# dmuley/sph-code

Measured on AMD Instinct MI355X. Metric: particle-steps/sec + achieved HBM GB/s, 10^6-particle 3D sphere, 1/2/4/8 GPUs, higher is better.
Workload: dtype f64

## Files before the change

### include/sphx.h

```cpp
#ifndef SPHX_H
#define SPHX_H

#include <stddef.h>
#include <stdint.h>

#ifdef __cplusplus
extern "C" {
#endif

#define SPHX_OK            0
#define SPHX_E_ARG        -1
#define SPHX_E_HIP        -2
#define SPHX_E_NOMEM      -3
#define SPHX_E_STATE      -4

#define SPHX_MAX_K        64
#define SPHX_MAX_SPECIES  32

typedef struct sphx_ctx sphx_ctx;

typedef struct sphx_constants {
    double k_B;
    double amu;
    double m_h;
    double m_0;
    double dt_0;
    double max_age;
    double pos_clamp;
} sphx_constants;

typedef struct sphx_stats {
    double ms_grid;
    double ms_search;
    double ms_prep;
    double ms_density;
    double ms_pi;
    double ms_visc;
    double ms_integrate;
    double ms_total;
    int64_t n;
    int64_t steps;
    int64_t candidates;
    int64_t retries;
    int64_t cells;
    int64_t refresh_steps;
    int64_t rebuild_steps;
    double  cell_size;
    double  ms_gravity;
    int64_t fallback_queries;
    double  ms_species;
    int64_t short_rows;
    int64_t detail_steps;
    int64_t far_queries;
    int64_t outlier_levels;
    int64_t bad_accel;
    int64_t bad_energy;
    int64_t bad_state;
    int64_t bad_h;
    int64_t search_steps;
} sphx_stats;

int         sphx_create(sphx_ctx** out, int device);
void        sphx_destroy(sphx_ctx* ctx);
const char* sphx_last_error(const sphx_ctx* ctx);
int         sphx_version(void);
const char* sphx_build_info(void);
const char* sphx_tunables(const sphx_ctx* ctx);
int sphx_selftest_scan(sphx_ctx* ctx, int n, unsigned seed, long long* mismatches, int* single_launch);
int sphx_selftest_mfma_cull(sphx_ctx* ctx, double E, int blocks, unsigned seed, double* max_err_over_E2,
                            double* wrong_signs, double* kappa);
int         sphx_host_alloc(void** out, size_t bytes);
int         sphx_host_free(void* p);
int         sphx_set_constants(sphx_ctx* ctx, const sphx_constants* c);
int         sphx_get_constants(const sphx_ctx* ctx, sphx_constants* c);
int         sphx_set_tuning(sphx_ctx* ctx, double rscale, double cell_factor);
int         sphx_set_timing_detail(sphx_ctx* ctx, int on);
int         sphx_set_incremental(sphx_ctx* ctx, int verlet, double rscale_build);

int sphx_neighbors(sphx_ctx* ctx, int64_t n, int k, const double* points, double dist,
                   double eps, int64_t* idx, double* dist_out, int64_t* nontriv, double* h);

int sphx_hydro_update(sphx_ctx* ctx, int64_t n, int k, int s, const int64_t* neighbor,
                      const double* points, const double* mass, const double* sizes,
                      const double* f_un, const double* particle_type, const double* T,
                      const double* mu_array, const double* gamma_array,
                      const double* velocities, int visc_mode,
                      double* hydro_accel, double* visc_accel, double* visc_heat,
                      double* rho, double* nden, double* f_un_nb, double* rho_dust);

int sphx_density(sphx_ctx* ctx, int64_t n, int k, const double* points, const double* mass,
                 const double* particle_type, const int64_t* neighbor, double d, double* out);
int sphx_dust_density(sphx_ctx* ctx, int64_t n, int k, const double* points, const double* mass,
                      const int64_t* neighbor, const double* particle_type, const double* sizes,
                      double* out);
int sphx_num_dens(sphx_ctx* ctx, int64_t n, int k, const double* mass, const double* points,
                  const double* mu_array, const int64_t* neighbor, double d, double* out);
int sphx_del_pressure(sphx_ctx* ctx, int64_t n, int k, const double* points, const double* mass,
                      const double* particle_type, const int64_t* neighbor,
                      const double* E_internal, const double* gamma_array, double d,
                      double* out );
int sphx_artificial_viscosity(sphx_ctx* ctx, int64_t n, int k, const int64_t* neighbor,
                              const double* points, const double* particle_type,
                              const double* sizes, const double* mass, const double* densities,
                              const double* velocities, const double* T,
                              const double* gamma_array, const double* mu_array, double d,
                              double* visc_accel , double* visc_heat );
int sphx_crossing_time(sphx_ctx* ctx, int64_t n, int k, const int64_t* neighbor,
                       const double* velocities, const double* sizes,
                       const double* particle_type, double* out );
int sphx_net_impulse(sphx_ctx* ctx, int64_t n, int k, const double* points, const double* mass,
                     const double* sizes, const double* velocities, const double* particle_type,
                     const int64_t* neighbor, const double* mean_grain_mass,
                     const double* mean_cross, double* accel_onto ,
                     double* accel_reaction );

int sphx_gravity_direct(sphx_ctx* ctx, int64_t n, const double* mass, const double* points,
                        const double* sizes, double softening, double G, double* accel);

int sphx_gravity_tree(sphx_ctx* ctx, int64_t n, const double* mass, const double* points,
                      const double* sizes, double softening, double G, int ws, int k_cells,
                      double* accel);

int sphx_agb_yields(sphx_ctx* ctx, int64_t n, const double* masses, const double* metallicities,
                    int nspl, const int32_t* ntx, const int32_t* nty, const double* tx,
                    const double* ty, const double* coeffs, const int32_t* mapto, double divisor,
                    int nspecies, const double* mu_specie, const double* composition,
                    double solar_mass, double* dust_out ,
                    double* gas_out );

int sphx_dt_rule(sphx_ctx* ctx, int64_t n, const double* ct, const int32_t* first, double* dt);
int sphx_clamp_arrays(sphx_ctx* ctx, int64_t n, double* points, double* velocities);
int sphx_leapfrog(sphx_ctx* ctx, int64_t n, double* points, double* velocities, double* total_accel,
                  const double* old_accel, double* E_internal, double* T, const double* mass,
                  const double* mu, const double* gamma, const double* ptype, const double* grav_accel,
                  const double* delp, const double* densities, const double* dust_densities,
                  const double* drag_on_gas, const double* drag_reaction, const double* av_accel,
                  const double* av_heat, double dt);

int sphx_state_upload(sphx_ctx* ctx, int64_t n, int s, const double* pos, const double* vel,
                      const double* mass, const double* ptype, const double* f_un,
                      const double* T, const double* mu, const double* gamma,
                      const double* E_internal, const double* accel_old);
int sphx_state_set_drag(sphx_ctx* ctx, const double* mean_grain_mass, const double* mean_cross);
int sphx_state_set_agb(sphx_ctx* ctx, int nspl, const int32_t* ntx, const int32_t* nty, const double* tx,
                       const double* ty, const double* coeffs, const int32_t* mapto, double divisor,
                       const double* mu_specie, double solar_mass);
int sphx_state_download_species(sphx_ctx* ctx, double* F, double* Z, double* agb_dust);
int sphx_state_set_loop_forms(sphx_ctx* ctx, int on, double d);
int sphx_set_clip_grad(sphx_ctx* ctx, int on);
int sphx_set_visc_mode(sphx_ctx* ctx, int mode);
int sphx_state_set_gravity(sphx_ctx* ctx, int mode, double G);
int sphx_set_gravity_order(sphx_ctx* ctx, int order);
int sphx_step(sphx_ctx* ctx, int nsteps, int k, double dist, int first, double fixed_dt);
int sphx_state_download(sphx_ctx* ctx, double* pos, double* vel, double* accel,
                        double* E_internal, double* T, double* sizes, double* rho,
                        double* nden, double* visc_heat, double* dt_last);
int sphx_state_download_pressure(sphx_ctx* ctx, double* pressure);
int sphx_arb_fields(sphx_ctx* ctx, int64_t n, const double* points, const double* mass,
                    const double* particle_type, const double* sizes, const double* T, const double* n_part,
                    const double* value, double d, int64_t m, const double* arb_points, double radius,
                    double* density, double* dust_density, double* temperature, double* dust_temperature,
                    double* photoionization, int64_t* count, int64_t* candidates, int64_t ball_id);
int sphx_arb_fields_list(sphx_ctx* ctx, int64_t n, const double* points, const double* mass,
                         const double* particle_type, const double* sizes, const double* T, const double* n_part,
                         const double* value, double d, int64_t m, const double* arb_points,
                         const int64_t* row_start, const int64_t* members, double* density, double* dust_density,
                         double* temperature, double* dust_temperature, double* photoionization, int64_t* count,
                         int64_t* candidates);
int sphx_state_sample(sphx_ctx* ctx, double d, const double* n_part, const double* value, int64_t m,
                      const double* arb_points, double radius, double* density, double* dust_density,
                      double* temperature, double* dust_temperature, double* photoionization, int64_t* count,
                      int64_t* candidates);
int sphx_arb_last_timing(sphx_ctx* ctx, double ms[4]);
int sphx_get_stats(sphx_ctx* ctx, sphx_stats* out);
int sphx_reset_stats(sphx_ctx* ctx);

int sphx_set_stream(sphx_ctx* ctx, void* hip_stream );
int sphx_reset_stream(sphx_ctx* ctx);
int sphx_sync(sphx_ctx* ctx);
int sphx_dev_set_mean_h(sphx_ctx* ctx, double mean_h);
int sphx_dev_search(sphx_ctx* ctx, int64_t n_total, int64_t n_owned, int k, const double* pos,
                    const double* hint, double rscale, double dist, double* h_out);
int sphx_dev_get_order(sphx_ctx* ctx, int64_t n_total, int32_t* out);
int sphx_dev_prep(sphx_ctx* ctx, const double* pos, const double* vel, const double* mass,
                  const double* h, const double* T, const double* mu, const double* gamma,
                  const double* ptype);
int sphx_dev_density(sphx_ctx* ctx, double* rho, double* rho_dust, double* nden, double* hydro_accel);
int sphx_dev_pi(sphx_ctx* ctx, const double* rho_complete, double* Pi, double* Bw, double* ct_out);
int sphx_dev_visc(sphx_ctx* ctx, const double* Bw_complete, const double* mass, double* visc_accel,
                  double* visc_heat);
int sphx_dev_visc_pairwise(sphx_ctx* ctx, const double* rho_complete, const double* mass, double* visc_accel,
                           double* visc_heat, double* ct_out);
int sphx_dev_clamp(sphx_ctx* ctx, int64_t n, double* pos, double* vel);
int sphx_dev_pack_rows(sphx_ctx* ctx, int64_t n, const int64_t* idx, int nf, const double* const* fields,
                       const int32_t* widths, double* rows);
int sphx_dev_regroup(sphx_ctx* ctx, int64_t n_sel, const int64_t* sel, int64_t n_rows, const double* rows,
                     int nf, const double* const* fields_in, const int32_t* widths,
                     double* const* fields_out);
int sphx_dev_need_map(sphx_ctx* ctx, int64_t n, const double* pos, const double* w, const double* g_lo,
                      double g_cs, int G, unsigned char* out);
int sphx_dev_integrate_auto(sphx_ctx* ctx, int64_t n_owned, double* pos, double* vel, double* accel_old,
                            double* E_internal, double* T, const double* mass, const double* mu,
                            const double* gamma, const double* ptype, const double* hydro_accel,
                            const double* visc_accel, const double* visc_heat, const double* red2,
                            int first, double fixed_dt, double* dt_out);
int sphx_dev_loop_prep(sphx_ctx* ctx, const double* pos, const double* vel, const double* mass, const double* T,
                       const double* mu, const double* gamma, const double* ptype, const double* E_internal, double d);
int sphx_dev_loop_pass1(sphx_ctx* ctx, const double* h_complete, double* rho, double* rho_dust, double* nden, double* delp);
int sphx_dev_loop_pass2(sphx_ctx* ctx, const double* rho_complete, double* visc_accel, double* visc_heat, double* ct_out);
int sphx_dev_loop_pass2_interior(sphx_ctx* ctx);
int sphx_dev_set_reach_cap(sphx_ctx* ctx, double cap);
int sphx_dev_select_blobs(sphx_ctx* ctx, int part);
int sphx_dev_blob_split_counts(sphx_ctx* ctx, int32_t counts[3]);
int sphx_dev_integrate_loop(sphx_ctx* ctx, int64_t n_owned, double* pos, double* vel, double* accel_old,
                            double* E_internal, double* T, const double* mass, const double* mu, const double* gamma,
                            const double* ptype, const double* delp, const double* rho, const double* av_accel,
                            const double* av_heat, const double* red2, int first, double fixed_dt, double dt,
                            double* dt_out);
int sphx_dev_drag(sphx_ctx* ctx, const double* mass, const double* ptype, const double* mean_grain_mass,
                  const double* mean_cross, double* drag_on, double* drag_reaction);
int sphx_dev_set_drag_terms(sphx_ctx* ctx, const double* drag_on, const double* drag_reaction, const double* rho,
                            const double* rho_dust);
int sphx_dev_set_agb(sphx_ctx* ctx, int nspecies, int nspl, const int32_t* ntx, const int32_t* nty, const double* tx,
                     const double* ty, const double* coeffs, const int32_t* mapto, double divisor,
                     const double* mu_specie, double solar_mass);
int sphx_dev_species(sphx_ctx* ctx, int nspecies, const double* f_un, const double* mass, double* F, double* Z,
                     double* agb_dust);
int sphx_dev_reach(sphx_ctx* ctx, int64_t n, const double* h, const double* vel, double halo_scale,
                   double skin_frac, double dt_last, double* w);
int sphx_dev_reach_dt(sphx_ctx* ctx, int64_t n, const double* h, const double* vel, double halo_scale,
                      double skin_frac, const double* dt_dev, double* w);
int sphx_dev_plan_mask(sphx_ctx* ctx, int64_t n, const double* pos, const double* g_lo, double g_cs, int G,
                       int world, int rank, const unsigned char* maps, unsigned char* mask, int64_t* counts);
int sphx_dev_step_scalars(sphx_ctx* ctx, int64_t n_owned, const double* h, const double* w_plan, double D,
                          double hclip, const double* ct, double* out4);
int sphx_dev_integrate(sphx_ctx* ctx, int64_t n_owned, double* pos, double* vel, double* accel_old,
                       double* E_internal, double* T, const double* mass, const double* mu,
                       const double* gamma, const double* ptype, const double* hydro_accel,
                       const double* visc_accel, const double* visc_heat, double dt);

#ifdef __cplusplus
}
#endif
#endif
```

### sph-code_amd/_lib.py

```python
import ctypes as C
import os
import threading
import weakref

import numpy as np

HERE = os.path.dirname(os.path.abspath(__file__))
LIB_PATH = os.environ.get("SPHX_LIB") or os.path.join(HERE, "libsphx.so")

c_double_p = C.POINTER(C.c_double)
c_int64_p = C.POINTER(C.c_int64)


class SphxConstants(C.Structure):
    _fields_ = [(n, C.c_double) for n in ("k_B", "amu", "m_h", "m_0", "dt_0", "max_age", "pos_clamp")]


class SphxStats(C.Structure):
    _fields_ = [(n, C.c_double) for n in ("ms_grid", "ms_search", "ms_prep", "ms_density", "ms_pi",
                                          "ms_visc", "ms_integrate", "ms_total")] + \
               [(n, C.c_int64) for n in ("n", "steps", "candidates", "retries", "cells", "refresh_steps",
                                         "rebuild_steps")] + \
               [("cell_size", C.c_double), ("ms_gravity", C.c_double), ("fallback_queries", C.c_int64),
                ("ms_species", C.c_double), ("short_rows", C.c_int64), ("detail_steps", C.c_int64), ("far_queries", C.c_int64),
                ("outlier_levels", C.c_int64), ("bad_accel", C.c_int64), ("bad_energy", C.c_int64), ("bad_state", C.c_int64),
                ("bad_h", C.c_int64), ("search_steps", C.c_int64)]

    def as_dict(self):
        return {n: getattr(self, n) for n, _ in self._fields_}


SPHX_E_STATE = -4
_P = C.c_void_p
_D = c_double_p
_I = c_int64_p
SIGNATURES = {
    "sphx_create": (C.c_int, [C.POINTER(_P), C.c_int]),
    "sphx_destroy": (None, [_P]),
    "sphx_last_error": (C.c_char_p, [_P]),
    "sphx_version": (C.c_int, []),
    "sphx_build_info": (C.c_char_p, []),
    "sphx_tunables": (C.c_char_p, [_P]),
    "sphx_selftest_scan": (C.c_int, [_P, C.c_int, C.c_uint, C.POINTER(C.c_longlong), C.POINTER(C.c_int)]),
    "sphx_selftest_mfma_cull": (C.c_int, [_P, C.c_double, C.c_int, C.c_uint, _D, _D, _D]),
    "sphx_host_alloc": (C.c_int, [C.POINTER(_P), C.c_size_t]),
    "sphx_host_free": (C.c_int, [_P]),
    "sphx_set_constants": (C.c_int, [_P, C.POINTER(SphxConstants)]),
    "sphx_get_constants": (C.c_int, [_P, C.POINTER(SphxConstants)]),
    "sphx_set_tuning": (C.c_int, [_P, C.c_double, C.c_double]),
    "sphx_set_incremental": (C.c_int, [_P, C.c_int, C.c_double]),
    "sphx_neighbors": (C.c_int, [_P, C.c_int64, C.c_int, _D, C.c_double, C.c_double, _I, _D, _I, _D]),
    "sphx_hydro_update": (C.c_int, [_P, C.c_int64, C.c_int, C.c_int, _I] + [_D] * 9 + [C.c_int] + [_D] * 7),
    "sphx_density": (C.c_int, [_P, C.c_int64, C.c_int, _D, _D, _D, _I, C.c_double, _D]),
    "sphx_dust_density": (C.c_int, [_P, C.c_int64, C.c_int, _D, _D, _I, _D, _D, _D]),
    "sphx_num_dens": (C.c_int, [_P, C.c_int64, C.c_int, _D, _D, _D, _I, C.c_double, _D]),
    "sphx_del_pressure": (C.c_int, [_P, C.c_int64, C.c_int, _D, _D, _D, _I, _D, _D, C.c_double, _D]),
    "sphx_artificial_viscosity": (C.c_int, [_P, C.c_int64, C.c_int, _I] + [_D] * 9 + [C.c_double, _D, _D]),
    "sphx_crossing_time": (C.c_int, [_P, C.c_int64, C.c_int, _I, _D, _D, _D, _D]),
    "sphx_net_impulse": (C.c_int, [_P, C.c_int64, C.c_int, _D, _D, _D, _D, _D, _I, _D, _D, _D, _D]),
    "sphx_agb_yields": (C.c_int, [_P, C.c_int64, _D, _D, C.c_int, C.POINTER(C.c_int32), C.POINTER(C.c_int32), _D, _D, _D,
                                  C.POINTER(C.c_int32), C.c_double, C.c_int, _D, _D, C.c_double, _D, _D]),
    "sphx_dt_rule": (C.c_int, [_P, C.c_int64, _D, C.POINTER(C.c_int32), _D]),
    "sphx_clamp_arrays": (C.c_int, [_P, C.c_int64, _D, _D]),
    "sphx_leapfrog": (C.c_int, [_P, C.c_int64] + [_D] * 18 + [C.c_double]),
    "sphx_state_upload": (C.c_int, [_P, C.c_int64, C.c_int] + [_D] * 10),
    "sphx_state_set_drag": (C.c_int, [_P, _D, _D]),
    "sphx_state_set_agb": (C.c_int, [_P, C.c_int, C.POINTER(C.c_int32), C.POINTER(C.c_int32), _D, _D, _D,
                                     C.POINTER(C.c_int32), C.c_double, _D, C.c_double]),
    "sphx_state_download_species": (C.c_int, [_P, _D, _D, _D]),
    "sphx_state_set_loop_forms": (C.c_int, [_P, C.c_int, C.c_double]),
    "sphx_set_clip_grad": (C.c_int, [_P, C.c_int]),
    "sphx_set_visc_mode": (C.c_int, [_P, C.c_int]),
    "sphx_state_set_gravity": (C.c_int, [_P, C.c_int, C.c_double]),
    "sphx_set_gravity_order": (C.c_int, [_P, C.c_int]),
    "sphx_gravity_direct": (C.c_int, [_P, C.c_int64, _D, _D, _D, C.c_double, C.c_double, _D]),
    "sphx_gravity_tree": (C.c_int, [_P, C.c_int64, _D, _D, _D, C.c_double, C.c_double, C.c_int, C.c_int, _D]),
    "sphx_step": (C.c_int, [_P, C.c_int, C.c_int, C.c_double, C.c_int, C.c_double]),
    "sphx_state_download": (C.c_int, [_P] + [_D] * 10),
    "sphx_state_download_pressure": (C.c_int, [_P, _D]),
    "sphx_arb_fields": (C.c_int, [_P, C.c_int64] + [_D] * 7 + [C.c_double, C.c_int64, _D, C.c_double] + [_D] * 5 + [_I, _I, C.c_int64]),
    "sphx_arb_last_timing": (C.c_int, [_P, _D]),
    "sphx_arb_fields_list": (C.c_int, [_P, C.c_int64] + [_D] * 7 + [C.c_double, C.c_int64, _D, _I, _I] + [_D] * 5 + [_I, _I]),
    "sphx_state_sample": (C.c_int, [_P, C.c_double, _D, _D, C.c_int64, _D, C.c_double] + [_D] * 5 + [_I, _I]),
    "sphx_get_stats": (C.c_int, [_P, C.POINTER(SphxStats)]),
    "sphx_reset_stats": (C.c_int, [_P]),
    "sphx_set_stream": (C.c_int, [_P, C.c_void_p]),
    "sphx_reset_stream": (C.c_int, [_P]),
    "sphx_sync": (C.c_int, [_P]),
    "sphx_dev_set_mean_h": (C.c_int, [_P, C.c_double]),
    "sphx_dev_search": (C.c_int, [_P, C.c_int64, C.c_int64, C.c_int, _P, _P, C.c_double, C.c_double, _P]),
    "sphx_dev_get_order": (C.c_int, [_P, C.c_int64, _P]),
    "sphx_dev_prep": (C.c_int, [_P] + [_P] * 8),
    "sphx_dev_density": (C.c_int, [_P] + [_P] * 4),
    "sphx_dev_pi": (C.c_int, [_P] + [_P] * 4),
    "sphx_dev_visc": (C.c_int, [_P] + [_P] * 4),
    "sphx_dev_visc_pairwise": (C.c_int, [_P] + [_P] * 5),
    "sphx_dev_clamp": (C.c_int, [_P, C.c_int64, _P, _P]),
    "sphx_dev_pack_rows": (C.c_int, [_P, C.c_int64, _P, C.c_int, C.POINTER(C.c_void_p), C.POINTER(C.c_int32), _P]),
    "sphx_dev_regroup": (C.c_int, [_P, C.c_int64, _P, C.c_int64, _P, C.c_int, C.POINTER(C.c_void_p),
                                   C.POINTER(C.c_int32), C.POINTER(C.c_void_p)]),
    "sphx_dev_need_map": (C.c_int, [_P, C.c_int64, _P, _P, C.POINTER(C.c_double), C.c_double, C.c_int, _P]),
    "sphx_dev_integrate_auto": (C.c_int, [_P, C.c_int64] + [_P] * 13 + [C.c_int, C.c_double, _P]),
    "sphx_dev_reach": (C.c_int, [_P, C.c_int64, _P, _P, C.c_double, C.c_double, C.c_double, _P]),
    "sphx_set_timing_detail": (C.c_int, [_P, C.c_int]),
    "sphx_dev_reach_dt": (C.c_int, [_P, C.c_int64, _P, _P, C.c_double, C.c_double, _P, _P]),
    "sphx_dev_plan_mask": (C.c_int, [_P, C.c_int64, _P, C.POINTER(C.c_double), C.c_double, C.c_int, C.c_int, C.c_int, _P, _P, _P]),
    "sphx_dev_step_scalars": (C.c_int, [_P, C.c_int64, _P, _P, C.c_double, C.c_double, _P, _P]),
    "sphx_dev_integrate": (C.c_int, [_P, C.c_int64] + [_P] * 12 + [C.c_double]),
    "sphx_dev_drag": (C.c_int, [_P] + [_P] * 6),
    "sphx_dev_set_drag_terms": (C.c_int, [_P] + [_P] * 4),
    "sphx_dev_set_agb": (C.c_int, [_P, C.c_int, C.c_int, C.POINTER(C.c_int32), C.POINTER(C.c_int32), _D, _D, _D,
                                   C.POINTER(C.c_int32), C.c_double, _D, C.c_double]),
    "sphx_dev_species": (C.c_int, [_P, C.c_int] + [_P] * 5),
    "sphx_dev_loop_prep": (C.c_int, [_P] + [_P] * 8 + [C.c_double]),
    "sphx_dev_loop_pass1": (C.c_int, [_P] + [_P] * 5),
    "sphx_dev_loop_pass2": (C.c_int, [_P] + [_P] * 4),
    "sphx_dev_loop_pass2_interior": (C.c_int, [_P]),
    "sphx_dev_set_reach_cap": (C.c_int, [_P, C.c_double]),
    "sphx_dev_select_blobs": (C.c_int, [_P, C.c_int]),
    "sphx_dev_blob_split_counts": (C.c_int, [_P, _P]),
    "sphx_dev_integrate_loop": (C.c_int, [_P, C.c_int64] + [_P] * 14 + [C.c_int, C.c_double, C.c_double, _P]),
}

_lib = None
_lock = threading.Lock()


def load_library():
    global _lib
    with _lock:
        if _lib is not None:
            return _lib
        if not os.path.exists(LIB_PATH):
            raise RuntimeError(
                "libsphx.so is not built (%s). Run `python -c 'import __graft_entry__ as g; g.build()'` "
                "or `python sph-code_amd/build.py`. There is no CPU fallback." % LIB_PATH)
        lib = C.CDLL(LIB_PATH)
        for name, (res, args) in SIGNATURES.items():
            fn = getattr(lib, name)
            fn.restype = res
            fn.argtypes = args
        _lib = lib
        return lib


def f64(a, shape=None):
    out = np.ascontiguousarray(a, dtype=np.float64)
    if shape is not None and out.shape != shape:
        raise ValueError("expected shape %s, got %s" % (shape, out.shape))
    return out


def i64(a, shape=None):
    out = np.ascontiguousarray(a, dtype=np.int64)
    if shape is not None and out.shape != shape:
        raise ValueError("expected shape %s, got %s" % (shape, out.shape))
    return out


class _PinnedPool:
    MIN_BYTES = 8 << 20
    KEEP_PER_SIZE = 3

    def __init__(self):
        self.free = {}
        self.lock = threading.Lock()

    def empty(self, shape, dtype):
        dtype = np.dtype(dtype)
        nbytes = int(np.prod(shape)) * dtype.itemsize
        if nbytes < self.MIN_BYTES:
            return np.empty(shape, dtype)
        with self.lock:
            lst = self.free.get(nbytes)
            ptr = lst.pop() if lst else None
        if ptr is None:
            lib = load_library()
            p = _P()
            if lib.sphx_host_alloc(C.byref(p), nbytes) != 0 or not p.value:
                return np.empty(shape, dtype)
            ptr = p.value
        buf = (C.c_byte * nbytes).from_address(ptr)
        weakref.finalize(buf, self._release, ptr, nbytes)
        return np.frombuffer(buf, dtype=dtype).reshape(shape)

    def _release(self, ptr, nbytes):
        with self.lock:
            lst = self.free.setdefault(nbytes, [])
            if len(lst) < self.KEEP_PER_SIZE:
                lst.append(ptr)
                return
        try:
            load_library().sphx_host_free(_P(ptr))
        except Exception:
            pass


pinned = _PinnedPool()


def dp(a):
    return None if a is None else a.ctypes.data_as(c_double_p)


def ip(a):
    return None if a is None else a.ctypes.data_as(c_int64_p)


class Context:

    def __init__(self, device=None):
        self.lib = load_library()
        if device is None:
            device = int(os.environ.get("LOCAL_RANK", "0"))
        self.device = device
        h = C.c_void_p()
        rc = self.lib.sphx_create(C.byref(h), device)
        if rc != 0 or not h:
            raise RuntimeError("sphx_create(device=%d) failed with %d: no usable MI355X/HIP device "
                               "(libsphx has no CPU path)" % (device, rc))
        self.h = h

    def close(self):
        if getattr(self, "h", None):
            self.lib.sphx_destroy(self.h)
            self.h = None

    def __del__(self):
        try:
            self.close()
        except Exception:
            pass

    def check(self, rc):
        if rc == 0:
            return
        msg = self.lib.sphx_last_error(self.h)
        msg = msg.decode() if msg else ""
        if rc == -1:
            raise ValueError("libsphx: " + msg)
        raise RuntimeError("libsphx error %d: %s" % (rc, msg))

    def constants(self):
        c = SphxConstants()
        self.check(self.lib.sphx_get_constants(self.h, C.byref(c)))
        return c

    def set_constants(self, **kw):
        c = self.constants()
        for k_, v in kw.items():
            setattr(c, k_, v)
        self.check(self.lib.sphx_set_constants(self.h, C.byref(c)))

    def set_tuning(self, rscale=0.0, cell_factor=0.0):
        self.check(self.lib.sphx_set_tuning(self.h, float(rscale), float(cell_factor)))

    def set_incremental(self, verlet=True, rscale_build=0.0):
        self.check(self.lib.sphx_set_incremental(self.h, 1 if verlet else 0, float(rscale_build)))

    def stats(self):
        s = SphxStats()
        self.check(self.lib.sphx_get_stats(self.h, C.byref(s)))
        return s.as_dict()

    def reset_stats(self):
        self.check(self.lib.sphx_reset_stats(self.h))

    def build_info(self):
        return {"library": self.lib.sphx_build_info().decode(), "tunables": self.lib.sphx_tunables(self.h).decode(),
                "lib_path": LIB_PATH}

    def set_timing_detail(self, on=True):
        self.check(self.lib.sphx_set_timing_detail(self.h, 1 if on else 0))


_default = None


def default_context():
    global _default
    if _default is None:
        _default = Context()
    return _default
```

### sph-code_amd/csrc/sphx_api.hip

```cpp
#include "sphx_internal.h"
#include <stdarg.h>
#include <stdlib.h>
#include <new>

int sphx_set_err(sphx_ctx* ctx, int code, const char* fmt, ...) {
    if (ctx) {
        va_list ap;
        va_start(ap, fmt);
        vsnprintf(ctx->err, sizeof(ctx->err), fmt, ap);
        va_end(ap);
    }
    return code;
}

void sphx_release(sphx_ctx* ctx, DevBuf& b) {
    for (size_t q = 0; q < ctx->allocs.size(); ++q)
        if (ctx->allocs[q] == b.p) { ctx->allocs[q] = ctx->allocs.back(); ctx->allocs.pop_back(); break; }
    if (b.p) (void)hipFree(b.p);
    b.p = nullptr;
    b.cap = 0;
}

int sphx_ensure(sphx_ctx* ctx, DevBuf& b, size_t bytes, hipStream_t in_use_on) {
    if (bytes == 0) bytes = 8;
    if (b.cap >= bytes) return SPHX_OK;
    if (b.p) {
        HIPCHK(hipStreamSynchronize(in_use_on));
        sphx_release(ctx, b);
    }
    size_t want = bytes + bytes / 8 + 256;
    hipError_t e = hipMalloc(&b.p, want);
    if (e != hipSuccess) {
        b.p = nullptr;
        return sphx_set_err(ctx, SPHX_E_NOMEM, "hipMalloc(%zu) failed: %s", want, hipGetErrorString(e));
    }
    b.cap = want;
    ctx->allocs.push_back(b.p);
    return SPHX_OK;
}

static void default_constants(sphx_constants* c) {
    c->k_B = 1.380649e-23;
    c->amu = 1.66053906892e-27;
    c->m_h = 1.0008 * c->amu;
    c->m_0 = 31.622776601683793 * 1.989e30;
    c->dt_0 = 60. * 60. * 24. * 365. * 250000.;
    c->max_age = 3e7 * 60. * 60. * 24. * 365.;
    c->pos_clamp = 1e11 * 149597870700.0;
}

extern "C" int sphx_version(void) { return 100; }

extern "C" const char* sphx_build_info(void) { return "gfx950 experiments=0"; }
extern "C" const char* sphx_tunables(const sphx_ctx* ctx) { return ctx ? ctx->tunables : ""; }

extern "C" int sphx_host_alloc(void** out, size_t bytes) {
    if (!out) return SPHX_E_ARG;
    *out = nullptr;
    if (bytes == 0) bytes = 8;
    if (hipHostMalloc(out, bytes, hipHostMallocDefault) != hipSuccess) {
        (void)hipGetLastError();
        *out = nullptr;
        return SPHX_E_NOMEM;
    }
    return SPHX_OK;
}
extern "C" int sphx_host_free(void* p) {
    if (p && hipHostFree(p) != hipSuccess) return SPHX_E_HIP;
    return SPHX_OK;
}

static hipError_t sphx_stream_create(hipStream_t* st, int side) {
    int least = 0, greatest = 0;
    if (hipDeviceGetStreamPriorityRange(&least, &greatest) != hipSuccess) return hipStreamCreateWithFlags(st, hipStreamNonBlocking);
    return hipStreamCreateWithPriority(st, hipStreamNonBlocking, side ? least : greatest);
}

extern "C" int sphx_create(sphx_ctx** out, int device) {
    if (!out) return SPHX_E_ARG;
    *out = nullptr;
    int count = 0;
    if (hipGetDeviceCount(&count) != hipSuccess || count <= 0 || device < 0 || device >= count) {
        fprintf(stderr, "sphx_create: no usable HIP device %d (found %d). libsphx has no CPU path.\n",
                device, count);
        return SPHX_E_HIP;
    }
    sphx_ctx* ctx = new (std::nothrow) sphx_ctx();
    if (!ctx) return SPHX_E_NOMEM;
    ctx->device = device;
    memset(&ctx->stats, 0, sizeof(ctx->stats));
    memset(&ctx->grid, 0, sizeof(ctx->grid));
    default_constants(&ctx->cst);
    auto env = [&](const char* name) -> const char* {
        const char* e = getenv(name);
        if (e) {
            const size_t used = strlen(ctx->tunables);
            snprintf(ctx->tunables + used, sizeof(ctx->tunables) - used, "%s%s=%s", used ? " " : "", name, e);
        }
        return e;
    };
    if (const char* e = env("SPHX_RSCALE")) { double v = atof(e); if (v >= 1.0) ctx->rscale = v; }
    if (const char* e = env("SPHX_CELL")) { double v = atof(e); if (v > 0.0) ctx->cell_factor = v; }
    if (const char* e = env("SPHX_RSCALE_BUILD")) { double v = atof(e); if (v >= 1.0) ctx->rscale_build = v; }
    if (const char* e = env("SPHX_VERLET")) ctx->use_verlet = atoi(e) != 0;
    if (const char* e = env("SPHX_BLOB")) ctx->use_blob = atoi(e) != 0;
    if (const char* e = env("SPHX_BLOB_CURVE")) ctx->blob_curve = atoi(e);
    if (const char* e = env("SPHX_KNN_GROUP")) ctx->use_group = atoi(e) != 0;
    if (const char* e = env("SPHX_HCLIP")) { double v = atof(e); if (v > 1.0) ctx->h_clip_factor = v; }
    if (const char* e = env("SPHX_TIMING_DETAIL")) ctx->timing_detail = atoi(e) != 0;
    if (const char* e = env("SPHX_MAX_CELLS")) { long long v = atoll(e); if (v > 0) ctx->max_cells = v; }
    if (const char* e = env("SPHX_CELL_FEEDBACK")) ctx->cell_feedback = atoi(e) != 0;
    if (const char* e = env("SPHX_CELL_FB_HI")) ctx->cell_fb_hi = atof(e);
    if (const char* e = env("SPHX_CELL_FB_LO")) ctx->cell_fb_lo = atof(e);
    if (const char* e = env("SPHX_DRAG_LDS")) ctx->drag_lds = atoi(e) != 0;
    if (const char* e = env("SPHX_BLOB_SPLIT")) ctx->blob_split_on = atoi(e) != 0;
    if (const char* e = env("SPHX_SPECIES_FUSED")) ctx->species_fused = atoi(e) != 0;
    if (const char* e = env("SPHX_SPECIES_LDS")) ctx->species_lds = atoi(e) != 0;
    if (const char* e = env("SPHX_HINT_DISTRUST")) ctx->distrust_mode = atoi(e);
    if (const char* e = env("SPHX_OUTLIER_LEVELS")) ctx->olev_mode = atoi(e);
    if (const char* e = env("SPHX_BOX_SIGMAS")) { double v = atof(e); if (v >= 1.0) ctx->box_sigmas = v; }
    if (const char* e = env("SPHX_GRAV_KERNEL")) ctx->grav_per_thread = atoi(e) == 0;
    if (const char* e = env("SPHX_GRAV_ORDER")) { int v = atoi(e); if (v == 1 || v == 2) ctx->grav_order = v; }
    if (const char* e = env("SPHX_GRAV_WS")) { int v = atoi(e); if (v >= 1 && v <= 4) ctx->grav_ws = v; }
    if (const char* e = env("SPHX_LDS")) ctx->use_lds = atoi(e) != 0;
    if (const char* e = env("SPHX_BLOB_SLOTS")) ctx->blob_slots = atoi(e);
    if (const char* e = env("SPHX_BLOB_WGS")) {
        int cus = 256;
        (void)hipDeviceGetAttribute(&cus, hipDeviceAttributeMultiprocessorCount, ctx->device);
        if (atoi(e) > 0) ctx->blob_grid = ((cus * atoi(e) + 7) / 8) * 8;
    }
    bool ok = hipSetDevice(device) == hipSuccess &&
              sphx_stream_create(&ctx->stream, 0) == hipSuccess &&
              hipHostMalloc(&ctx->pinned, 16384, hipHostMallocDefault) == hipSuccess;
    ctx->own_stream = ctx->stream;
    for (int i = 0; ok && i < 10; ++i) ok = hipEventCreate(&ctx->ev[i]) == hipSuccess;
    for (int r = 0; ok && r < 3; ++r)
        for (int i = 0; ok && i < 10; ++i) ok = hipEventCreate(&ctx->evring[r][i]) == hipSuccess;
    for (int r = 0; ok && r < 2; ++r)
        ok = hipEventCreateWithFlags(&ctx->lag_bev[r], hipEventDisableTiming) == hipSuccess &&
             hipEventCreateWithFlags(&ctx->lag_hev[r], hipEventDisableTiming) == hipSuccess;
    if (ok) ok = sphx_stream_create(&ctx->side_stream, 1) == hipSuccess &&
                 hipEventCreateWithFlags(&ctx->ev_join, hipEventDisableTiming) == hipSuccess &&
                 hipEventCreateWithFlags(&ctx->ev_perm, hipEventDisableTiming) == hipSuccess;
    if (ok) ok = sphx_ensure(ctx, ctx->scal, SC_NSLOTS * 8) == SPHX_OK &&
                 hipMemsetAsync(ctx->scal.p, 0, SC_NSLOTS * 8, ctx->stream) == hipSuccess &&
                 sphx_ensure(ctx, ctx->badc, (size_t)BADC_BUCKETS * BADC_STRIDE * sizeof(u64)) == SPHX_OK &&
                 hipMemsetAsync(ctx->badc.p, 0, (size_t)BADC_BUCKETS * BADC_STRIDE * sizeof(u64), ctx->stream) == hipSuccess;
    if (!ok) {
        fprintf(stderr, "sphx_create: HIP initialisation failed on device %d\n", device);
        delete ctx;
        return SPHX_E_HIP;
    }
    *out = ctx;
    return SPHX_OK;
}

extern "C" void sphx_destroy(sphx_ctx* ctx) {
    if (!ctx) return;
    (void)hipSetDevice(ctx->device);
    if (ctx->stream) (void)hipStreamSynchronize(ctx->stream);
    for (void* p : ctx->allocs) (void)hipFree(p);
    for (int i = 0; i < 10; ++i)
        if (ctx->ev[i]) (void)hipEventDestroy(ctx->ev[i]);
    for (int i = 0; i < 5; ++i)
        if (ctx->arb_ev[i]) (void)hipEventDestroy(ctx->arb_ev[i]);
    for (int r = 0; r < 3; ++r)
        for (int i = 0; i < 10; ++i)
            if (ctx->evring[r][i]) (void)hipEventDestroy(ctx->evring[r][i]);
    for (int r = 0; r < 2; ++r) {
        if (ctx->lag_bev[r]) (void)hipEventDestroy(ctx->lag_bev[r]);
        if (ctx->lag_hev[r]) (void)hipEventDestroy(ctx->lag_hev[r]);
    }
    if (ctx->pinned) (void)hipHostFree(ctx->pinned);
    if (ctx->olev_ev) (void)hipEventDestroy(ctx->olev_ev);
    if (ctx->ev_join) (void)hipEventDestroy(ctx->ev_join);
    if (ctx->ev_perm) (void)hipEventDestroy(ctx->ev_perm);
    if (ctx->side_stream) (void)hipStreamDestroy(ctx->side_stream);
    if (ctx->own_stream) (void)hipStreamDestroy(ctx->own_stream);
    delete ctx;
}

extern "C" const char* sphx_last_error(const sphx_ctx* ctx) { return ctx ? ctx->err : "null context"; }

extern "C" int sphx_set_constants(sphx_ctx* ctx, const sphx_constants* c) {
    if (!ctx || !c) return SPHX_E_ARG;
    ctx->cst = *c;
    return SPHX_OK;
}
extern "C" int sphx_set_tuning(sphx_ctx* ctx, double rscale, double cell_factor) {
    if (!ctx) return SPHX_E_ARG;
    if (rscale > 0.0) {
        if (rscale < 1.0) return sphx_set_err(ctx, SPHX_E_ARG, "rscale %g < 1", rscale);
        ctx->rscale = rscale;
    }
    if (cell_factor > 0.0) ctx->cell_factor = cell_factor;
    return SPHX_OK;
}
extern "C" int sphx_set_incremental(sphx_ctx* ctx, int verlet, double rscale_build) {
    if (!ctx) return SPHX_E_ARG;
    ctx->use_verlet = verlet != 0;
    if (!ctx->use_verlet) ctx->list_valid = false;
    if (rscale_build > 0.0) {
        if (rscale_build < 1.0) return sphx_set_err(ctx, SPHX_E_ARG, "rscale_build %g < 1", rscale_build);
        ctx->rscale_build = rscale_build;
    }
    return SPHX_OK;
}
extern "C" int sphx_get_constants(const sphx_ctx* ctx, sphx_constants* c) {
    if (!ctx || !c) return SPHX_E_ARG;
    *c = ctx->cst;
    return SPHX_OK;
}

static int upload(sphx_ctx* ctx, DevBuf& b, const void* host, size_t bytes) {
    SPHX_TRY(sphx_ensure(ctx, b, bytes));
    HIPCHK(hipMemcpyAsync(b.p, host, bytes, hipMemcpyHostToDevice, ctx->stream));
    return SPHX_OK;
}
static int download(sphx_ctx* ctx, void* host, const void* dev, size_t bytes) {
    if (!host) return SPHX_OK;
    HIPCHK(hipMemcpyAsync(host, dev, bytes, hipMemcpyDeviceToHost, ctx->stream));
    return SPHX_OK;
}

extern "C" int sphx_neighbors(sphx_ctx* ctx, int64_t n, int k, const double* points, double dist,
                              double eps, int64_t* idx, double* dist_out, int64_t* nontriv,
                              double* h) {
    (void)eps;
    if (!ctx) return SPHX_E_ARG;
    NEED(points);
    if (n < 1) return sphx_set_err(ctx, SPHX_E_ARG, "n=%lld < 1", (long long)n);
    if (k < 1 || k > SPHX_MAX_K) return sphx_set_err(ctx, SPHX_E_ARG, "N_NEIGH=%d not in 1..%d", k, SPHX_MAX_K);
    HIPCHK(hipSetDevice(ctx->device));
    ctx->map_perm = nullptr;
    ctx->qorder = nullptr;
    const size_t nb = (size_t)n * sizeof(double);
    SPHX_TRY(upload(ctx, ctx->in_a, points, 3 * nb));
    SPHX_TRY(sphx_ensure(ctx, ctx->in_b, nb));
    SPHX_TRY(sphx_ensure(ctx, ctx->in_c, nb));
    SPHX_TRY(sphx_ensure(ctx, ctx->in_d, nb));
    SPHX_TRY(sphx_ensure(ctx, ctx->in_e, nb));
    SPHX_TRY(sphx_ensure(ctx, ctx->in_f, nb));
    SPHX_TRY(sphx_ensure(ctx, ctx->in_g, nb));
    double *x = ctx->in_b.as<double>(), *y = ctx->in_c.as<double>(), *z = ctx->in_d.as<double>();
    double *xs = ctx->in_e.as<double>(), *ys = ctx->in_f.as<double>(), *zs = ctx->in_g.as<double>();
    SPHX_TRY(sphx_aos_to_soa3(ctx, n, ctx->in_a.as<double>(), x, y, z));
    ctx->clip_valid = false;
    SPHX_TRY(sphx_build_grid(ctx, n, k, x, y, z, 0.0));
    SPHX_TRY(sphx_gather3(ctx, n, ctx->perm.as<int>(), x, y, z, xs, ys, zs));
    SPHX_TRY(sphx_ensure(ctx, ctx->idx64, (size_t)n * k * sizeof(int64_t)));
    SPHX_TRY(sphx_ensure(ctx, ctx->dist_out, (size_t)n * k * sizeof(double)));
    SPHX_TRY(sphx_ensure(ctx, ctx->nontriv, (size_t)n * sizeof(int64_t)));
    SPHX_TRY(sphx_ensure(ctx, ctx->h_api, nb));
    KnnOut o;
    o.nbr = nullptr; o.h_sorted = nullptr;
    o.idx64 = ctx->idx64.as<int64_t>(); o.dist = ctx->dist_out.as<double>();
    o.nontriv = ctx->nontriv.as<int64_t>(); o.h_by_id = ctx->h_api.as<double>();
    KnnIn in;
    in.xs = xs; in.ys = ys; in.zs = zs;
    in.id = ctx->perm.as<int>();
    in.rbound = dist;
    SPHX_TRY(sphx_knn(ctx, n, k, in, o));
    SPHX_TRY(download(ctx, idx, o.idx64, (size_t)n * k * sizeof(int64_t)));
    SPHX_TRY(download(ctx, dist_out, o.dist, (size_t)n * k * sizeof(double)));
    SPHX_TRY(download(ctx, nontriv, o.nontriv, (size_t)n * sizeof(int64_t)));
    SPHX_TRY(download(ctx, h, o.h_by_id, nb));
    HIPCHK(hipStreamSynchronize(ctx->stream));
    return SPHX_OK;
}

extern "C" int sphx_hydro_update(sphx_ctx* ctx, int64_t n, int k, int s, const int64_t* neighbor,
                                 const double* points, const double* mass, const double* sizes,
                                 const double* f_un, const double* particle_type, const double* T,
                                 const double* mu_array, const double* gamma_array,
                                 const double* velocities, int visc_mode, double* hydro_accel,
                                 double* visc_accel, double* visc_heat, double* rho, double* nden,
                                 double* f_un_nb, double* rho_dust) {
    if (!ctx) return SPHX_E_ARG;
    NEED(points); NEED(mass); NEED(sizes); NEED(particle_type); NEED(T);
    NEED(mu_array); NEED(gamma_array); NEED(velocities);
    if (n < 1 || n > 0x7FFFFFF0ll) return sphx_set_err(ctx, SPHX_E_ARG, "n=%lld out of range", (long long)n);
    if (k < 1 || k > 4096) return sphx_set_err(ctx, SPHX_E_ARG, "k=%d out of range", k);
    if (visc_mode != 0 && visc_mode != 1)
// ... 651 lines not shown
```

### sph-code_amd/csrc/sphx_blob.h

```cpp
#pragma once
#include "sphx_internal.h"
#include "sphx_pair.h"

#ifndef BLOB_P
#define BLOB_P 128
#endif
#define BLOB_T (2 * BLOB_P)
#define LPP SPHX_SUM_PARTS
#define PASS_T (BLOB_P * LPP)
#ifndef BLOB_S
#define BLOB_S 960
#endif
#ifndef DEDUP_PRIO
#define DEDUP_PRIO 2
#endif
#ifndef BLOB_STAGE_PRIO
#define BLOB_STAGE_PRIO 1
#endif
#ifndef PASS_MINW
#define PASS_MINW 4
#endif
#define BLOB_PROBES 96
#define SLOT_NONE 0xFFFFu
#define SLOT_OVER 0xFFFEu
#define DD_BATCH 8

typedef unsigned short u16;

__device__ __forceinline__ unsigned slot_hash(int j) {
    return (unsigned)(((u64)((unsigned)j * 2654435761u) * (u64)BLOB_S) >> 32);
}

__device__ __forceinline__ Q4 lload4(const double2* img, int s, int c2) {
    const double2 lo = img[(2 * c2) * BLOB_S + s];
    const double2 hi = img[(2 * c2 + 1) * BLOB_S + s];
    return Q4{lo.x, lo.y, hi.x, hi.y};
}
__device__ __forceinline__ double sqrt_mid(double x) {
    const double y = __builtin_amdgcn_rsq(x);
    double g = x * y;
    double h = 0.5 * y;
    const double r = __builtin_fma(-h, g, 0.5);
    g = __builtin_fma(g, r, g);
    h = __builtin_fma(h, r, h);
    const double d0 = __builtin_fma(-g, g, x);
    g = __builtin_fma(d0, h, g);
    const double d1 = __builtin_fma(-g, g, x);
    g = __builtin_fma(d1, h, g);
    return x > 0.0 ? g : 0.0;
}
struct SqrtMid { __device__ __forceinline__ double operator()(double x) const { return sqrt_mid(x); } };

__device__ __forceinline__ double pair_swap(double v) {
    const long long b = __double_as_longlong(v);
    const int lo = __builtin_amdgcn_update_dpp(0, (int)b, 0xB1, 0xF, 0xF, true);
    const int hi = __builtin_amdgcn_update_dpp(0, (int)(b >> 32), 0xB1, 0xF, 0xF, true);
    return __longlong_as_double(((long long)hi << 32) | (unsigned)lo);
}
__device__ __forceinline__ double pair_swap2(double v) {
    const long long b = __double_as_longlong(v);
    const int lo = __builtin_amdgcn_update_dpp(0, (int)b, 0x4E, 0xF, 0xF, true);
    const int hi = __builtin_amdgcn_update_dpp(0, (int)(b >> 32), 0x4E, 0xF, 0xF, true);
    return __longlong_as_double(((long long)hi << 32) | (unsigned)lo);
}
__device__ __forceinline__ double group_total(double acc) {
    acc = acc + pair_swap(acc);
    if (LPP == 4) acc = acc + pair_swap2(acc);
    return acc;
}
__device__ __forceinline__ double group_max(double v) {
    v = fmax(v, pair_swap(v));
    if (LPP == 4) v = fmax(v, pair_swap2(v));
    return v;
}

#define NSTAGE ((BLOB_S + PASS_T - 1) / PASS_T)
#define NB (8 / LPP)
#define KPAD(k) ((((k) + 7) / 8) * 8)
#define IMG_BYTES(per_slot, k) ((size_t)BLOB_S * (per_slot) + (size_t)KPAD(k) * BLOB_P * sizeof(u16))

template <int NSIDE, class Rec>
__device__ __forceinline__ void stage(double2* img, double* side, u16* tile, const Rec* __restrict__ rec,
                                      const double* __restrict__ g0, int g0_stride,
                                      const double* __restrict__ g1, int g1_stride,
                                      const int* __restrict__ uq, const u16* __restrict__ slot16, int npad,
                                      int k, int b) {
    __builtin_amdgcn_s_setprio(BLOB_STAGE_PRIO);
    int ju[NSTAGE];
#pragma unroll
    for (int r = 0; r < NSTAGE; ++r) {
        const int s = threadIdx.x + r * PASS_T;
        ju[r] = (s < BLOB_S) ? uq[s] : -1;
    }
    const int pieces = KPAD(k) * (BLOB_P / 8);
    for (int q = threadIdx.x; q < pieces; q += PASS_T) {
        const int kk = q / (BLOB_P / 8), c = q % (BLOB_P / 8);
        uint4 v = make_uint4(0xFFFFFFFFu, 0xFFFFFFFFu, 0xFFFFFFFFu, 0xFFFFFFFFu);
        if (kk < k) v = *reinterpret_cast<const uint4*>(slot16 + (size_t)kk * npad + (size_t)b * BLOB_P + c * 8);
        *reinterpret_cast<uint4*>(tile + kk * BLOB_P + c * 8) = v;
    }
    double2 c[NSTAGE][4];
    double e0[NSTAGE], e1[NSTAGE];
#pragma unroll
    for (int r = 0; r < NSTAGE; ++r) {
        const int j = ju[r] < 0 ? 0 : ju[r];
        const double2* g = reinterpret_cast<const double2*>(&rec[j]);
        c[r][0] = g[0]; c[r][1] = g[1]; c[r][2] = g[2]; c[r][3] = g[3];
        e0[r] = (NSIDE > 0) ? g0[(size_t)j * g0_stride] : 0.0;
        e1[r] = (NSIDE > 1) ? g1[(size_t)j * g1_stride] : 0.0;
    }
#pragma unroll
    for (int r = 0; r < NSTAGE; ++r) {
        const int s = threadIdx.x + r * PASS_T;
        if (ju[r] >= 0) {
            if (NSIDE == 2) c[r][3].y = e0[r];
            img[0 * BLOB_S + s] = c[r][0]; img[1 * BLOB_S + s] = c[r][1];
            img[2 * BLOB_S + s] = c[r][2]; img[3 * BLOB_S + s] = c[r][3];
            if (NSIDE == 1) side[s] = e0[r];
            if (NSIDE == 2) side[s] = e1[r];
        }
    }
    __builtin_amdgcn_s_setprio(0);
}

__device__ __forceinline__ void load_slots(unsigned (&sl)[NB], const u16* tile, int m0, int half, int t) {
#pragma unroll
    for (int u = 0; u < NB; ++u) sl[u] = tile[(LPP * (m0 + u) + half) * BLOB_P + t];
}
__device__ __forceinline__ bool all_staged(const unsigned (&sl)[NB]) {
    unsigned worst = sl[0];
#pragma unroll
    for (int u = 1; u < NB; ++u) worst = worst > sl[u] ? worst : sl[u];
    return __ballot(worst >= SLOT_OVER) == 0ull;
}


struct BlobSel { const int* list; const int* cnt; int mode; };
__device__ __forceinline__ int blob_sel_count(const BlobSel& s, int nblk) {
    if (!s.list) return nblk;
    return (s.mode == 1) ? s.cnt[0] : (s.mode == 2) ? s.cnt[1] : s.cnt[0] + s.cnt[1];
}
__device__ __forceinline__ int blob_sel_at(const BlobSel& s, int bi, int count) {
    const int q = xcd_block(bi, count);
    return s.list ? s.list[q + (s.mode == 2 ? s.cnt[0] : 0)] : q;
}
BlobSel sphx_blob_sel(sphx_ctx* ctx, int part);

int sphx_blob_grid(sphx_ctx* ctx, int nblk);
int sphx_lds_opt_in(sphx_ctx* ctx, const void* kernel, size_t bytes);
```

### sph-code_amd/csrc/sphx_blob.hip

```cpp
#include "sphx_blob.h"
#include "sphx_wave.h"
#pragma clang fp contract(off)
#include <float.h>
#include <stdlib.h>
#include <stdio.h>

#define DD_TAB 2048
#define DD_PROBES 64
__device__ __forceinline__ unsigned dd_hash(int j) { return ((unsigned)j * 2654435761u) >> 21; }

__global__ __launch_bounds__(BLOB_T) void blob_dedup_kernel(int n, int npad, int k, int slots,
                                                            const int* __restrict__ nbr, u16* slot16,
                                                            int* uniq, const int* __restrict__ qorder,
                                                            const int* __restrict__ omap, int n_active,
                                                            unsigned char* bclass) {
    __builtin_amdgcn_s_setprio(DEDUP_PRIO);
    extern __shared__ u16 dd_tile[];
    __shared__ int key[DD_TAB];
    __shared__ u16 slot_of[DD_TAB];
    __shared__ int wave_tot[BLOB_T / 64];
    const int b = xcd_block(blockIdx.x, gridDim.x);
    const int t = threadIdx.x >> 1, half = threadIdx.x & 1;
    const int p = b * BLOB_P + t;
    for (int q = threadIdx.x; q < DD_TAB; q += BLOB_T) key[q] = -1;
// ... 11 lines not shown
            int jb[DD_BATCH];
#pragma unroll
            for (int u = 0; u < DD_BATCH; ++u) {
                jb[u] = jn[u];
                const int kk = 2 * (m0 + DD_BATCH + u) + half;
                jn[u] = (kk < k && live) ? nbr[(size_t)kk * npad + p] : -1;
            }
            unsigned hb[DD_BATCH];
            int eb[DD_BATCH];
#pragma unroll
            for (int u = 0; u < DD_BATCH; ++u) {
                hb[u] = dd_hash(jb[u] < 0 ? 0 : jb[u]);
                eb[u] = key[hb[u]];
            }
#pragma unroll
            for (int u = 0; u < DD_BATCH; ++u)
                if (jb[u] >= 0 && eb[u] == -1) {
                    const int old = atomicCAS(&key[hb[u]], -1, jb[u]);
                    eb[u] = (old == -1) ? jb[u] : old;
                }
#pragma unroll
            for (int u = 0; u < DD_BATCH; ++u) {
                const int kk = 2 * (m0 + u) + half;
                if (kk >= k) continue;
                const int j = jb[u];
                unsigned s = SLOT_NONE;
                if (j >= 0) {
                    unsigned h = hb[u];
                    s = SLOT_OVER;
                    if (eb[u] == j) {
                        s = h;
                    } else {
                        for (int probe = 1; probe < DD_PROBES; ++probe) {
                            h = (h + 1) & (DD_TAB - 1);
                            int e = key[h];
                            if (e == -1) {
                                e = atomicCAS(&key[h], -1, j);
                                if (e == -1) e = j;
                            }
                            if (e == j) { s = h; break; }
                        }
                    }
                }
                dd_tile[kk * BLOB_P + t] = (u16)s;
            }
        }
    }
    __syncthreads();
    constexpr int EPT = DD_TAB / BLOB_T;
    const int e0 = threadIdx.x * EPT;
    int cnt = 0;
#pragma unroll
    for (int q = 0; q < EPT; ++q) cnt += key[e0 + q] != -1;
    const int incl = wave_scan_incl(cnt);
    const int lane = threadIdx.x & 63, wv = threadIdx.x >> 6;
    if (lane == 63) wave_tot[wv] = incl;
    __syncthreads();
    int base = incl - cnt, total = 0;
#pragma unroll
    for (int w = 0; w < BLOB_T / 64; ++w) {
        const int tw = wave_tot[w];
        if (w < wv) base += tw;
        total += tw;
    }
    int* uq = uniq + (size_t)b * BLOB_S;
    int needs_ghost = 0;
#pragma unroll
    for (int q = 0; q < EPT; ++q) {
        const int j = key[e0 + q];
        if (j != -1) {
            slot_of[e0 + q] = (u16)(base < slots ? base : SLOT_OVER);
            if (base < slots) uq[base] = j;
            ++base;
            if (bclass && omap[j] >= n_active) needs_ghost = 1;
        }
    }
    for (int q = (total < slots ? total : slots) + threadIdx.x; q < BLOB_S; q += BLOB_T) uq[q] = -1;
    __syncthreads();
    const int pieces = k * (BLOB_P / 8);
    for (int q = threadIdx.x; q < pieces; q += BLOB_T) {
        u16* src = dd_tile + q * 8;
        const int kk = q / (BLOB_P / 8), c = q % (BLOB_P / 8);
        unsigned v[8];
#pragma unroll
        for (int u = 0; u < 8; ++u) {
            const unsigned e = src[u];
            v[u] = e < DD_TAB ? (unsigned)slot_of[e] : e;
            if (v[u] == SLOT_OVER) needs_ghost = 1;
        }
        if ((size_t)b * BLOB_P + c * 8 < (size_t)npad)
            *reinterpret_cast<uint4*>(slot16 + (size_t)kk * npad + (size_t)b * BLOB_P + c * 8) =
                make_uint4(v[0] | (v[1] << 16), v[2] | (v[3] << 16), v[4] | (v[5] << 16), v[6] | (v[7] << 16));
    }
    if (bclass) {
        const int owned_q = (half == 0 && p < n && omap[qorder[p]] < n_active) ? 1 : 0;
        const int any_owned = __syncthreads_or(owned_q);
        const int any_ghost = __syncthreads_or(needs_ghost);
        if (threadIdx.x == 0) bclass[b] = (unsigned char)(!any_owned ? 2 : (any_ghost ? 1 : 0));
    }
}

#define SPLIT_T 1024
__global__ __launch_bounds__(SPLIT_T) void blob_split_kernel(int nblk, const unsigned char* __restrict__ bclass, int* list,
                                                             int* cnt) {
    __shared__ int wsum[2][SPLIT_T / 64];
    const int per = (nblk + SPLIT_T - 1) / SPLIT_T;
    const int b0 = threadIdx.x * per, b1 = (b0 + per < nblk) ? b0 + per : nblk;
    int c0 = 0, c1 = 0;
    for (int b = b0; b < b1; ++b) { const int c = bclass[b]; c0 += c == 0; c1 += c == 1; }
    const int i0 = wave_scan_incl(c0), i1 = wave_scan_incl(c1);
    const int lane = threadIdx.x & 63, wv = threadIdx.x >> 6;
    if (lane == 63) { wsum[0][wv] = i0; wsum[1][wv] = i1; }
    __syncthreads();
    int o0 = i0 - c0, o1 = i1 - c1, t0 = 0, t1 = 0;
    for (int w = 0; w < SPLIT_T / 64; ++w) {
        if (w < wv) { o0 += wsum[0][w]; o1 += wsum[1][w]; }
        t0 += wsum[0][w]; t1 += wsum[1][w];
    }
    for (int b = b0; b < b1; ++b) {
        const int c = bclass[b];
        if (c == 0) list[o0++] = b;
        else if (c == 1) list[t0 + o1++] = b;
    }
    if (threadIdx.x == 0) { cnt[0] = t0; cnt[1] = t1; cnt[2] = nblk - t0 - t1; }
}

int sphx_blob_translate(sphx_ctx* ctx, int64_t n, int k) {
    const int64_t npad = sphx_pad64(n);
    const int nblk = (int)((npad + BLOB_P - 1) / BLOB_P);
    SPHX_TRY(sphx_ensure(ctx, ctx->slot16, (size_t)k * npad * sizeof(u16) + 512));
    SPHX_TRY(sphx_ensure(ctx, ctx->uniq, (size_t)nblk * BLOB_S * sizeof(int)));
    int slots = ctx->blob_slots;
    if (slots < 1) slots = 1;
    if (slots > BLOB_S) slots = BLOB_S;
    const bool split = ctx->map_perm != nullptr && ctx->blob_split_on;
    unsigned char* bclass = nullptr;
    ctx->blob_split_valid = false;
    if (split) {
        SPHX_TRY(sphx_ensure(ctx, ctx->blob_class, (size_t)nblk));
        SPHX_TRY(sphx_ensure(ctx, ctx->blob_split, ((size_t)nblk + 4) * sizeof(int)));
        bclass = ctx->blob_class.as<unsigned char>();
    }
    hipLaunchKernelGGL(blob_dedup_kernel, dim3(nblk), dim3(BLOB_T), (size_t)k * BLOB_P * sizeof(u16), ctx->stream, (int)n, (int)npad, k, slots,
                       ctx->nbr.as<int>(), ctx->slot16.as<u16>(), ctx->uniq.as<int>(), ctx->qorder, ctx->map_perm,
                       ctx->map_nactive, bclass);
    if (split) {
        int* list = ctx->blob_split.as<int>();
        hipLaunchKernelGGL(blob_split_kernel, dim3(1), dim3(SPLIT_T), 0, ctx->stream, nblk, bclass, list, list + (size_t)nblk);
        ctx->blob_split_valid = true;
        ctx->blob_split_nblk = nblk;
    }
    HIPCHK(hipGetLastError());
    ctx->blob_lists = true;
    return SPHX_OK;
}

template <bool FAST, bool CLIP>
__device__ __forceinline__ void density_batch(DensAcc& a, double (&wout)[NB], const unsigned (&sl)[NB], const double2* img,
                                              const RecA* __restrict__ rec, const int* __restrict__ nbr,
                                              size_t col0, size_t colstep, double xr, double yr, double zr,
                                              double hi2, double ci, double Ai) {
    Q4 q0b[NB], q1b[NB];
#pragma unroll
    for (int u = 0; u < NB; ++u) {
        if (FAST || sl[u] < SLOT_OVER) { q0b[u] = lload4(img, (int)sl[u], 0); q1b[u] = lload4(img, (int)sl[u], 1); }
        else if (sl[u] == SLOT_OVER) {
            const double* q = reinterpret_cast<const double*>(&rec[nbr[col0 + u * colstep]]);
            q0b[u] = gload4(q); q1b[u] = gload4(q + 4);
        } else { q0b[u] = Q4{xr, yr, zr, 0.0}; q1b[u] = Q4{0.0, 0.0, 0.0, 0.0}; }
    }
    if (FAST) __builtin_amdgcn_sched_barrier(0);
#pragma unroll
    for (int u = 0; u < NB; ++u) {
        wout[u] = 0.0;
        if (!FAST && sl[u] == SLOT_NONE) continue;
        wout[u] = density_term<SqrtMid>(a, q0b[u], q1b[u], xr, yr, zr, hi2, ci, Ai, CLIP);
    }
}

__global__ __launch_bounds__(PASS_T, PASS_MINW) void blob_density_kernel(int n, int npad, int k, int nblk,
                                                              const int* __restrict__ nbr,
                                                              const u16* __restrict__ slot16,
                                                              const int* __restrict__ uniq,
                                                              const int* __restrict__ qorder, int clip,
                                                              const int* __restrict__ omap, int n_active,
                                                              const RecA* __restrict__ rec, double* rho_s,
                                                              double* rho, double* rhod, double* nden, double* G,
                                                              double* ha, BlobSel sel) {
    extern __shared__ double2 img[];
    u16* tile = reinterpret_cast<u16*>(img + 4 * BLOB_S);
    const int t = threadIdx.x / LPP, half = threadIdx.x & (LPP - 1);
    const int nsel = blob_sel_count(sel, nblk);
    for (int bi = blockIdx.x; bi < nsel; bi += gridDim.x) {
        const int b = blob_sel_at(sel, bi, nsel);
        const int p = b * BLOB_P + t;
        const int i = (p < n) ? qorder[p] : 0;
        stage<0>(img, nullptr, tile, rec, nullptr, 0, nullptr, 0, uniq + (size_t)b * BLOB_S, slot16, npad, k, b);
        const double* self = reinterpret_cast<const double*>(&rec[i]);
        const Q4 s0 = gload4(self), s1 = gload4(self + 4);
        const int o = (p < n) ? (omap ? omap[i] : i) : 0x7FFFFFFF;
        __syncthreads();
        if (o < n_active) {
            double xr = s0.a, yr = s0.b, zr = s0.c;
            {
                const unsigned sl0 = tile[t];
                if (sl0 < SLOT_OVER) { const Q4 r = lload4(img, (int)sl0, 0); xr = r.a; yr = r.b; zr = r.c; }
                else if (sl0 == SLOT_OVER) { const int j0 = nbr[p]; xr = rec[j0].x; yr = rec[j0].y; zr = rec[j0].z; }
            }
            const double hi2 = s0.d, ci = -6.0 * s1.a, Ai = s1.c;
            DensAcc a{0.0, 0.0, 0.0, 0.0, 0.0, 0.0};
            const int nm = KPAD(k) / LPP;
            unsigned sl[NB];
            load_slots(sl, tile, 0, half, t);
            for (int m0 = 0; m0 < nm; m0 += NB) {
                unsigned cur[NB];
#pragma unroll
                for (int u = 0; u < NB; ++u) cur[u] = sl[u];
                if (m0 + NB < nm) load_slots(sl, tile, m0 + NB, half, t);
                const size_t col0 = (size_t)(LPP * m0 + half) * npad + p;
                const bool fast = all_staged(cur);
                double wo[NB];
                if (fast && !clip) density_batch<true, false>(a, wo, cur, img, rec, nbr, col0, LPP * (size_t)npad, xr, yr, zr, hi2, ci, Ai);
                else if (fast) density_batch<true, true>(a, wo, cur, img, rec, nbr, col0, LPP * (size_t)npad, xr, yr, zr, hi2, ci, Ai);
                else if (!clip) density_batch<false, false>(a, wo, cur, img, rec, nbr, col0, LPP * (size_t)npad, xr, yr, zr, hi2, ci, Ai);
                else density_batch<false, true>(a, wo, cur, img, rec, nbr, col0, LPP * (size_t)npad, xr, yr, zr, hi2, ci, Ai);
            }
            const double s_rho = group_total(a.rho), s_rd = group_total(a.rd), s_n = group_total(a.n);
            const double gx = group_total(a.gx), gy = group_total(a.gy), gz = group_total(a.gz);
            if (!half) {
                rho[o] = s_rho; rhod[o] = s_rd; nden[o] = s_n;
                rho_s[i] = s_rho;
                if (G) { G[3 * (size_t)o + 0] = -gx; G[3 * (size_t)o + 1] = -gy; G[3 * (size_t)o + 2] = -gz; }
                ha[3 * (size_t)o + 0] = -gx / s_rho;
                ha[3 * (size_t)o + 1] = -gy / s_rho;
                ha[3 * (size_t)o + 2] = -gz / s_rho;
            }
        }
        __syncthreads();
    }
}

template <bool FAST>
__device__ __forceinline__ void pi_batch(double& s_pi, double& maxrel, const unsigned (&sl)[NB], const double2* img,
                                         const double* lrho, const RecB* __restrict__ recb,
                                         const double* __restrict__ rho_s, const int* __restrict__ nbr, size_t col0,
                                         size_t colstep, const Q4& r0, const Q4& rv, double rho_i, double cs_i) {
    Q4 q0b[NB], qvb[NB];
    double rhob[NB];
#pragma unroll
    for (int u = 0; u < NB; ++u) {
        if (FAST || sl[u] < SLOT_OVER) {
            q0b[u] = lload4(img, (int)sl[u], 0); qvb[u] = lload4(img, (int)sl[u], 1);
            rhob[u] = lrho[sl[u]];
        } else if (sl[u] == SLOT_OVER) {
            const int jj = nbr[col0 + u * colstep];
            const double* qb = reinterpret_cast<const double*>(&recb[jj]);
            q0b[u] = gload4(qb); qvb[u] = gload4(qb + 4);
            rhob[u] = rho_s[jj];
        } else { q0b[u] = r0; qvb[u] = rv; rhob[u] = rho_i; }
    }
    if (FAST) __builtin_amdgcn_sched_barrier(0);
#pragma unroll
    for (int u = 0; u < NB; ++u) {
        if (!FAST && sl[u] == SLOT_NONE) continue;
        const PiPair t = pi_term<SqrtMid>(q0b[u], qvb[u], rhob[u], r0, rv, rho_i, cs_i);
        s_pi += t.pi;
        maxrel = fmax(maxrel, t.rel);
    }
}

__global__ __launch_bounds__(PASS_T, PASS_MINW) void blob_pi_kernel(int n, int npad, int k, int nblk,
                                                         const int* __restrict__ nbr,
                                                         const u16* __restrict__ slot16,
                                                         const int* __restrict__ uniq,
                                                         const int* __restrict__ qorder,
                                                         const int* __restrict__ omap, int n_active,
                                                         const RecB* __restrict__ recb,
                                                         const double* __restrict__ rho_s,
                                                         const RecSelf* __restrict__ selfr, RecBC* bc, double* Pi,
                                                         double* BwOut, u64* ct_bits, BlobSel sel) {
    extern __shared__ double2 img[];
    double* lrho = reinterpret_cast<double*>(img + 4 * BLOB_S);
    u16* tile = reinterpret_cast<u16*>(lrho + BLOB_S);
    const int t = threadIdx.x / LPP, half = threadIdx.x & (LPP - 1);
    u64 my_ct = SPHX_CT_NONE;
    const int nsel = blob_sel_count(sel, nblk);
    for (int bi = blockIdx.x; bi < nsel; bi += gridDim.x) {
        const int b = blob_sel_at(sel, bi, nsel);
        const int p = b * BLOB_P + t;
        const int i = (p < n) ? qorder[p] : 0;
        stage<1>(img, lrho, tile, recb, rho_s, 1, nullptr, 0, uniq + (size_t)b * BLOB_S, slot16, npad, k, b);
        const RecSelf sf = selfr[i];
        const double rho_i = rho_s[i];
        const double* selfq = reinterpret_cast<const double*>(&recb[i]);
        const Q4 self0 = gload4(selfq), selfv = gload4(selfq + 4);
        const int o = (p < n) ? (omap ? omap[i] : i) : 0x7FFFFFFF;
        __syncthreads();
        if (o < n_active) {
            Q4 r0 = self0, rv = selfv;
            {
                const unsigned sl0 = tile[t];
                if (sl0 < SLOT_OVER) { r0 = lload4(img, (int)sl0, 0); rv = lload4(img, (int)sl0, 1); }
                else if (sl0 == SLOT_OVER) {
                    const double* rq = reinterpret_cast<const double*>(&recb[nbr[p]]);
                    r0 = gload4(rq); rv = gload4(rq + 4);
                }
            }
            const double cs_i = sf.csi, ms_i = sf.mg, h_i = sf.h;
            double s_pi = 0.0, maxrel = 0.0;
            const int nm = KPAD(k) / LPP;
            unsigned sl[NB];
            load_slots(sl, tile, 0, half, t);
            for (int m0 = 0; m0 < nm; m0 += NB) {
                unsigned cur[NB];
#pragma unroll
                for (int u = 0; u < NB; ++u) cur[u] = sl[u];
                if (m0 + NB < nm) load_slots(sl, tile, m0 + NB, half, t);
                const size_t col0 = (size_t)(LPP * m0 + half) * npad + p;
                if (all_staged(cur))
                    pi_batch<true>(s_pi, maxrel, cur, img, lrho, recb, rho_s, nbr, col0, LPP * (size_t)npad, r0, rv, rho_i, cs_i);
                else
                    pi_batch<false>(s_pi, maxrel, cur, img, lrho, recb, rho_s, nbr, col0, LPP * (size_t)npad, r0, rv, rho_i, cs_i);
            }
            s_pi = group_total(s_pi);
            maxrel = group_max(maxrel);
            if (!half) {
                Pi[o] = s_pi;
                const double bw = fmax(ms_i, 0.0) * s_pi;
                bc[i].Bw = bw;
                if (BwOut) BwOut[o] = bw;
                if (ms_i > 0.0) {
                    const u64 cb = ct_vote_bits(h_i, maxrel);
                    my_ct = cb < my_ct ? cb : my_ct;
                }
            }
        }
        __syncthreads();
    }
    block_min_vote<PASS_T>(my_ct, ct_bits);
}

template <bool FAST, bool CLIP>
__device__ __forceinline__ void visc_batch(ViscAcc& a, const unsigned (&sl)[NB], const double2* img,
                                           const double* lc1, const RecB* __restrict__ recb,
                                           const RecBC* __restrict__ bc, const int* __restrict__ nbr, size_t col0,
                                           size_t colstep, const Q4& r0, const Q4& rv, double hi2, double ci,
                                           double Bi) {
    Q4 q0b[NB], qvb[NB];
    double c1b[NB];
#pragma unroll
    for (int u = 0; u < NB; ++u) {
        if (FAST || sl[u] < SLOT_OVER) {
            q0b[u] = lload4(img, (int)sl[u], 0); qvb[u] = lload4(img, (int)sl[u], 1);
            c1b[u] = lc1[sl[u]];
        } else if (sl[u] == SLOT_OVER) {
            const int jj = nbr[col0 + u * colstep];
            const double* qb = reinterpret_cast<const double*>(&recb[jj]);
            q0b[u] = gload4(qb); qvb[u] = gload4(qb + 4);
            const double2 tt = *reinterpret_cast<const double2*>(&bc[jj]);
            qvb[u].d = tt.x; c1b[u] = tt.y;
        } else { q0b[u] = r0; qvb[u] = rv; c1b[u] = 0.0; }
    }
    if (FAST) __builtin_amdgcn_sched_barrier(0);
#pragma unroll
    for (int u = 0; u < NB; ++u) {
        if (!FAST && sl[u] == SLOT_NONE) continue;
        visc_term<SqrtMid>(a, q0b[u], qvb[u], qvb[u].d, c1b[u], r0, rv, hi2, ci, Bi, CLIP);
    }
}

__global__ __launch_bounds__(PASS_T, PASS_MINW) void blob_visc_kernel(int n, int npad, int k, int nblk,
                                                           const int* __restrict__ nbr,
                                                           const u16* __restrict__ slot16,
                                                           const int* __restrict__ uniq,
                                                           const int* __restrict__ qorder, int clip,
                                                           const int* __restrict__ omap, int n_active,
                                                           const RecB* __restrict__ recb,
                                                           const RecBC* __restrict__ bc,
                                                           const double* __restrict__ m, double* va, double* vh,
                                                           BlobSel sel) {
    extern __shared__ double2 img[];
    double* lc1 = reinterpret_cast<double*>(img + 4 * BLOB_S);
    u16* tile = reinterpret_cast<u16*>(lc1 + BLOB_S);
    const int t = threadIdx.x / LPP, half = threadIdx.x & (LPP - 1);
    const double* bcd = reinterpret_cast<const double*>(bc);
    const int nsel = blob_sel_count(sel, nblk);
    for (int bi = blockIdx.x; bi < nsel; bi += gridDim.x) {
        const int b = blob_sel_at(sel, bi, nsel);
        const int p = b * BLOB_P + t;
        const int i = (p < n) ? qorder[p] : 0;
        stage<2>(img, lc1, tile, recb, bcd, 2, bcd + 1, 2, uniq + (size_t)b * BLOB_S, slot16, npad, k, b);
        const double2 bci = *reinterpret_cast<const double2*>(&bc[i]);
        const double* selfq = reinterpret_cast<const double*>(&recb[i]);
        const Q4 self0 = gload4(selfq), selfv = gload4(selfq + 4);
        const int o = (p < n) ? (omap ? omap[i] : i) : 0x7FFFFFFF;
        const double mi = (o < n_active) ? m[o] : 0.0;
        __syncthreads();
        if (o < n_active) {
            Q4 r0 = self0, rv = selfv;
            {
                const unsigned sl0 = tile[t];
                if (sl0 < SLOT_OVER) { r0 = lload4(img, (int)sl0, 0); rv = lload4(img, (int)sl0, 1); }
                else if (sl0 == SLOT_OVER) {
                    const double* rq = reinterpret_cast<const double*>(&recb[nbr[p]]);
                    r0 = gload4(rq); rv = gload4(rq + 4);
                }
            }
            const double hi2 = self0.d, ci = -6.0 * bci.y, Bi = bci.x;
            ViscAcc a{0.0, 0.0, 0.0, 0.0};
            const int nm = KPAD(k) / LPP;
            unsigned sl[NB];
            load_slots(sl, tile, 0, half, t);
            for (int m0 = 0; m0 < nm; m0 += NB) {
                unsigned cur[NB];
#pragma unroll
                for (int u = 0; u < NB; ++u) cur[u] = sl[u];
                if (m0 + NB < nm) load_slots(sl, tile, m0 + NB, half, t);
                const size_t col0 = (size_t)(LPP * m0 + half) * npad + p;
                const bool fast = all_staged(cur);
                if (fast && !clip) visc_batch<true, false>(a, cur, img, lc1, recb, bc, nbr, col0, LPP * (size_t)npad, r0, rv, hi2, ci, Bi);
                else if (fast) visc_batch<true, true>(a, cur, img, lc1, recb, bc, nbr, col0, LPP * (size_t)npad, r0, rv, hi2, ci, Bi);
                else if (!clip) visc_batch<false, false>(a, cur, img, lc1, recb, bc, nbr, col0, LPP * (size_t)npad, r0, rv, hi2, ci, Bi);
                else visc_batch<false, true>(a, cur, img, lc1, recb, bc, nbr, col0, LPP * (size_t)npad, r0, rv, hi2, ci, Bi);
            }
            const double ax = group_total(a.x), ay = group_total(a.y), az = group_total(a.z), heat = group_total(a.h);
            if (!half) {
                va[3 * (size_t)o + 0] = -ax; va[3 * (size_t)o + 1] = -ay; va[3 * (size_t)o + 2] = -az;
                vh[o] = heat * mi / 2.0;
            }
        }
        __syncthreads();
    }
}

template <bool FAST, bool CLIP>
__device__ __forceinline__ void visc_pw_batch(ViscAcc& a, double& maxrel, const unsigned (&sl)[NB], const double2* img,
                                              const double* lrho, const RecB* __restrict__ recb,
                                              const double* __restrict__ rho_s, const RecBC* __restrict__ bc,
                                              const int* __restrict__ nbr, size_t col0, size_t colstep, const Q4& r0,
                                              const Q4& rv, double rho_i, double cs_i, double hi2, double ci) {
    Q4 q0b[NB], qvb[NB];
    double rhob[NB], mcb[NB];
#pragma unroll
    for (int u = 0; u < NB; ++u) {
        if (FAST || sl[u] < SLOT_OVER) {
            q0b[u] = lload4(img, (int)sl[u], 0); qvb[u] = lload4(img, (int)sl[u], 1);
            rhob[u] = lrho[sl[u]];
            mcb[u] = bc[nbr[col0 + u * colstep]].Bw;
        } else if (sl[u] == SLOT_OVER) {
            const int jj = nbr[col0 + u * colstep];
            const double* qb = reinterpret_cast<const double*>(&recb[jj]);
            q0b[u] = gload4(qb); qvb[u] = gload4(qb + 4);
            rhob[u] = rho_s[jj]; mcb[u] = bc[jj].Bw;
        } else { q0b[u] = r0; qvb[u] = rv; rhob[u] = rho_i; mcb[u] = 0.0; }
    }
    if (FAST) __builtin_amdgcn_sched_barrier(0);
#pragma unroll
    for (int u = 0; u < NB; ++u) {
        if (!FAST && sl[u] == SLOT_NONE) continue;
        maxrel = fmax(maxrel, visc_pw_term<SqrtMid>(a, q0b[u], qvb[u], rhob[u], mcb[u], r0, rv, rho_i, cs_i, hi2, ci, CLIP));
    }
}

__global__ __launch_bounds__(PASS_T, PASS_MINW) void blob_visc_pw_kernel(int n, int npad, int k, int nblk,
                                                              const int* __restrict__ nbr,
                                                              const u16* __restrict__ slot16,
                                                              const int* __restrict__ uniq,
                                                              const int* __restrict__ qorder, int clip,
                                                              const int* __restrict__ omap, int n_active,
                                                              const RecB* __restrict__ recb,
                                                              const double* __restrict__ rho_s,
                                                              const RecBC* __restrict__ bc,
                                                              const RecSelf* __restrict__ selfr,
                                                              const double* __restrict__ m, double* va, double* vh,
                                                              u64* ct_bits, BlobSel sel) {
    extern __shared__ double2 img[];
    double* lrho = reinterpret_cast<double*>(img + 4 * BLOB_S);
    u16* tile = reinterpret_cast<u16*>(lrho + BLOB_S);
    const int t = threadIdx.x / LPP, half = threadIdx.x & (LPP - 1);
    u64 my_ct = SPHX_CT_NONE;
    const int nsel = blob_sel_count(sel, nblk);
    for (int bi = blockIdx.x; bi < nsel; bi += gridDim.x) {
        const int b = blob_sel_at(sel, bi, nsel);
        const int p = b * BLOB_P + t;
        const int i = (p < n) ? qorder[p] : 0;
        stage<1>(img, lrho, tile, recb, rho_s, 1, nullptr, 0, uniq + (size_t)b * BLOB_S, slot16, npad, k, b);
        const RecSelf sf = selfr[i];
        const double rho_i = rho_s[i], mci = bc[i].Bw;
        const double* selfq = reinterpret_cast<const double*>(&recb[i]);
        const Q4 self0 = gload4(selfq), selfv = gload4(selfq + 4);
        const int o = (p < n) ? (omap ? omap[i] : i) : 0x7FFFFFFF;
        const double mi = (o < n_active) ? m[o] : 0.0;
        __syncthreads();
        if (o < n_active) {
            Q4 r0 = self0, rv = selfv;
            {
                const unsigned sl0 = tile[t];
                if (sl0 < SLOT_OVER) { r0 = lload4(img, (int)sl0, 0); rv = lload4(img, (int)sl0, 1); }
                else if (sl0 == SLOT_OVER) {
                    const double* rq = reinterpret_cast<const double*>(&recb[nbr[p]]);
                    r0 = gload4(rq); rv = gload4(rq + 4);
                }
            }
            const double cs_i = sf.csi, h_i = sf.h, hi2 = self0.d, ci = -6.0 * mci;
            ViscAcc a{0.0, 0.0, 0.0, 0.0};
            double maxrel = 0.0;
            const int nm = KPAD(k) / LPP;
            unsigned sl[NB];
            load_slots(sl, tile, 0, half, t);
            for (int m0 = 0; m0 < nm; m0 += NB) {
                unsigned cur[NB];
#pragma unroll
                for (int u = 0; u < NB; ++u) cur[u] = sl[u];
                if (m0 + NB < nm) load_slots(sl, tile, m0 + NB, half, t);
                const size_t col0 = (size_t)(LPP * m0 + half) * npad + p;
                const bool fast = all_staged(cur);
                if (fast && !clip) visc_pw_batch<true, false>(a, maxrel, cur, img, lrho, recb, rho_s, bc, nbr, col0, LPP * (size_t)npad, r0, rv, rho_i, cs_i, hi2, ci);
                else if (fast) visc_pw_batch<true, true>(a, maxrel, cur, img, lrho, recb, rho_s, bc, nbr, col0, LPP * (size_t)npad, r0, rv, rho_i, cs_i, hi2, ci);
                else if (!clip) visc_pw_batch<false, false>(a, maxrel, cur, img, lrho, recb, rho_s, bc, nbr, col0, LPP * (size_t)npad, r0, rv, rho_i, cs_i, hi2, ci);
                else visc_pw_batch<false, true>(a, maxrel, cur, img, lrho, recb, rho_s, bc, nbr, col0, LPP * (size_t)npad, r0, rv, rho_i, cs_i, hi2, ci);
            }
            const double ax = group_total(a.x), ay = group_total(a.y), az = group_total(a.z), heat = group_total(a.h);
            maxrel = group_max(maxrel);
            if (!half) {
                va[3 * (size_t)o + 0] = -ax; va[3 * (size_t)o + 1] = -ay; va[3 * (size_t)o + 2] = -az;
                vh[o] = heat * mi / 2.0;
                if (sf.mg > 0.0) {
                    const u64 cb = ct_vote_bits(h_i, maxrel);
                    my_ct = cb < my_ct ? cb : my_ct;
                }
            }
        }
        __syncthreads();
    }
    block_min_vote<PASS_T>(my_ct, ct_bits);
}

template <int SPEC_MAXM>
__device__ __forceinline__ void species_sweeps(const double (&w)[SPEC_MAXM], double2* img, const u16* tile,
                                               const int* __restrict__ uq, const int* __restrict__ nbr, int n, int npad,
                                               int nm, int p, int i, int t, int half, bool live, int S,
                                               const double* __restrict__ fun, const int* __restrict__ row_of,
                                               const double* __restrict__ m, const AgbTable& agb, int agb_on, double* F,
                                               double* Zout, double* agb_out) {
    double tot[16];
#pragma unroll
    for (int hh = 0; hh < 2; ++hh) {
        __syncthreads();
        {
            int ju[NSTAGE];
#pragma unroll
            for (int r = 0; r < NSTAGE; ++r) {
                const int s = threadIdx.x + r * PASS_T;
                ju[r] = (s < BLOB_S) ? uq[s] : -1;
            }
            double2 c[NSTAGE][4];
#pragma unroll
            for (int r = 0; r < NSTAGE; ++r) {
                const int jr = ju[r] < 0 ? 0 : ju[r];
                const double2* g = reinterpret_cast<const double2*>(fun + (size_t)(row_of ? row_of[jr] : jr) * 16) + 4 * hh;
                c[r][0] = g[0]; c[r][1] = g[1]; c[r][2] = g[2]; c[r][3] = g[3];
            }
#pragma unroll
            for (int r = 0; r < NSTAGE; ++r) {
                const int s = threadIdx.x + r * PASS_T;
                if (ju[r] >= 0) {
                    img[0 * BLOB_S + s] = c[r][0]; img[1 * BLOB_S + s] = c[r][1];
                    img[2 * BLOB_S + s] = c[r][2]; img[3 * BLOB_S + s] = c[r][3];
                }
            }
        }
        __syncthreads();
        double acc[8];
#pragma unroll
        for (int q = 0; q < 8; ++q) acc[q] = 0.0;
#pragma unroll
        for (int mm = 0; mm < SPEC_MAXM; ++mm) {
            if (mm < nm) {
                const unsigned sl = tile[(LPP * mm + half) * BLOB_P + t];
                if (sl != SLOT_NONE && live) {
                    Q4 f0, f1;
                    if (sl < SLOT_OVER) { f0 = lload4(img, (int)sl, 0); f1 = lload4(img, (int)sl, 1); }
                    else {
                        const int jo = nbr[(size_t)(LPP * mm + half) * npad + p];
                        const double* q = fun + (size_t)(row_of ? row_of[jo] : jo) * 16 + 8 * hh;
                        f0 = gload4(q); f1 = gload4(q + 4);
                    }
                    const double wm = w[mm];
                    acc[0] += wm * f0.a; acc[1] += wm * f0.b; acc[2] += wm * f0.c; acc[3] += wm * f0.d;
                    acc[4] += wm * f1.a; acc[5] += wm * f1.b; acc[6] += wm * f1.c; acc[7] += wm * f1.d;
                }
            }
        }
#pragma unroll
        for (int q = 0; q < 8; ++q) tot[8 * hh + q] = group_total(acc[q]);
    }
    if (live && !half) {
#pragma unroll
        for (int q = 0; q < 16; ++q)
            if (q < S) F[(size_t)q * n + i] = tot[q];
    }
    if (live && agb_on) {
        const double Z = species_metallicity(agb, tot, S);
        if (!half) Zout[i] = Z;
        const double Mi = m[i];
        double* row = agb_out + (size_t)i * S;
        for (int q = half; q < S; q += LPP)
            if (!((agb.covered >> q) & 1u)) row[q] = 0.0;
        for (int o = half; o < agb.nspl; o += LPP) {
            double val;
            const int target = agb_one_spline(agb, o, Mi, Z, val);
            if (target >= 0) row[target] = val;
        }
    }
}

template <int SPEC_MAXM>
__global__ __launch_bounds__(PASS_T, PASS_MINW) void blob_density_species_kernel(int n, int npad, int k, int nblk,
        const int* __restrict__ nbr, const u16* __restrict__ slot16, const int* __restrict__ uniq,
        const int* __restrict__ qorder, int clip, const RecA* __restrict__ rec, double* rho_s, double* rho, double* rhod,
        double* nden, double* G, double* ha,
        int S, const double* __restrict__ fun, const int* __restrict__ row_of, const double* __restrict__ m, AgbTable agb,
        int agb_on, double* F, double* Zout, double* agb_out) {
    extern __shared__ double2 img[];
    u16* tile = reinterpret_cast<u16*>(img + 4 * BLOB_S);
    const int t = threadIdx.x / LPP, half = threadIdx.x & (LPP - 1);
    const int nm = KPAD(k) / LPP;
    for (int bi = blockIdx.x; bi < nblk; bi += gridDim.x) {
        const int b = xcd_block(bi, nblk);
        const int p = b * BLOB_P + t;
        const bool live = p < n;
        const int i = live ? qorder[p] : 0;
        const int* uq = uniq + (size_t)b * BLOB_S;
        stage<0>(img, nullptr, tile, rec, nullptr, 0, nullptr, 0, uq, slot16, npad, k, b);
        const double* self = reinterpret_cast<const double*>(&rec[i]);
        const Q4 s0 = gload4(self), s1 = gload4(self + 4);
        __syncthreads();
        double w[SPEC_MAXM];
#pragma unroll
        for (int mm = 0; mm < SPEC_MAXM; ++mm) w[mm] = 0.0;
        if (live) {
            double xr = s0.a, yr = s0.b, zr = s0.c;
            {
                const unsigned sl0 = tile[t];
                if (sl0 < SLOT_OVER) { const Q4 r = lload4(img, (int)sl0, 0); xr = r.a; yr = r.b; zr = r.c; }
                else if (sl0 == SLOT_OVER) { const int j0 = nbr[p]; xr = rec[j0].x; yr = rec[j0].y; zr = rec[j0].z; }
            }
            const double hi2 = s0.d, ci = -6.0 * s1.a, Ai = s1.c;
            DensAcc a{0.0, 0.0, 0.0, 0.0, 0.0, 0.0};
#pragma unroll
            for (int m0 = 0; m0 < SPEC_MAXM; m0 += NB) {
                if (m0 < nm) {
                    unsigned cur[NB];
                    load_slots(cur, tile, m0, half, t);
                    const size_t col0 = (size_t)(LPP * m0 + half) * npad + p;
                    const bool fast = all_staged(cur);
                    double wo[NB];
                    if (fast && !clip) density_batch<true, false>(a, wo, cur, img, rec, nbr, col0, LPP * (size_t)npad, xr, yr, zr, hi2, ci, Ai);
                    else if (fast) density_batch<true, true>(a, wo, cur, img, rec, nbr, col0, LPP * (size_t)npad, xr, yr, zr, hi2, ci, Ai);
                    else if (!clip) density_batch<false, false>(a, wo, cur, img, rec, nbr, col0, LPP * (size_t)npad, xr, yr, zr, hi2, ci, Ai);
                    else density_batch<false, true>(a, wo, cur, img, rec, nbr, col0, LPP * (size_t)npad, xr, yr, zr, hi2, ci, Ai);
#pragma unroll
                    for (int u = 0; u < NB; ++u) if (m0 + u < SPEC_MAXM) w[m0 + u] = wo[u];
                }
            }
            const double s_rho = group_total(a.rho), s_rd = group_total(a.rd), s_n = group_total(a.n);
            const double gx = group_total(a.gx), gy = group_total(a.gy), gz = group_total(a.gz);
            if (!half) {
                rho[i] = s_rho; rhod[i] = s_rd; nden[i] = s_n;
                rho_s[i] = s_rho;
                if (G) { G[3 * (size_t)i + 0] = -gx; G[3 * (size_t)i + 1] = -gy; G[3 * (size_t)i + 2] = -gz; }
                ha[3 * (size_t)i + 0] = -gx / s_rho;
                ha[3 * (size_t)i + 1] = -gy / s_rho;
                ha[3 * (size_t)i + 2] = -gz / s_rho;
            }
        }
        species_sweeps(w, img, tile, uq, nbr, n, npad, nm, p, i, t, half, live, S, fun, row_of, m, agb, agb_on, F, Zout, agb_out);
        __syncthreads();
    }
}


template <int SPEC_MAXM>
__global__ __launch_bounds__(PASS_T, PASS_MINW) void blob_species_kernel(int n, int npad, int k, int nblk,
                                                              const int* __restrict__ nbr,
                                                              const u16* __restrict__ slot16,
                                                              const int* __restrict__ uniq,
                                                              const int* __restrict__ qorder, int S,
                                                              const RecA* __restrict__ rec,
                                                              const double* __restrict__ fun,
                                                              const int* __restrict__ row_of,
                                                              const double* __restrict__ m, AgbTable agb, int agb_on,
                                                              double* F, double* Zout, double* agb_out) {
    extern __shared__ double2 img[];
    u16* tile = reinterpret_cast<u16*>(img + 4 * BLOB_S);
    const int t = threadIdx.x / LPP, half = threadIdx.x & (LPP - 1);
    const int nm = KPAD(k) / LPP;
    for (int bi = blockIdx.x; bi < nblk; bi += gridDim.x) {
        const int b = xcd_block(bi, nblk);
        const int p = b * BLOB_P + t;
        const bool live = p < n;
        const int i = live ? qorder[p] : 0;
        const int* uq = uniq + (size_t)b * BLOB_S;
        stage<0>(img, nullptr, tile, rec, nullptr, 0, nullptr, 0, uq, slot16, npad, k, b);
        __syncthreads();
        double w[SPEC_MAXM];
        {
            double xr, yr, zr;
            {
                const int j0 = live ? nbr[p] : 0;
                const unsigned sl0 = tile[t];
                if (sl0 < SLOT_OVER) { const Q4 r = lload4(img, (int)sl0, 0); xr = r.a; yr = r.b; zr = r.c; }
                else { const int jj = j0 < 0 ? i : j0; xr = rec[jj].x; yr = rec[jj].y; zr = rec[jj].z; }
            }
#pragma unroll
            for (int mm = 0; mm < SPEC_MAXM; ++mm) {
                w[mm] = 0.0;
                if (mm < nm) {
                    const unsigned sl = tile[(LPP * mm + half) * BLOB_P + t];
                    if (sl != SLOT_NONE && live) {
                        Q4 q0, q1;
                        if (sl < SLOT_OVER) { q0 = lload4(img, (int)sl, 0); q1 = lload4(img, (int)sl, 1); }
                        else {
                            const double* q = reinterpret_cast<const double*>(&rec[nbr[(size_t)(LPP * mm + half) * npad + p]]);
                            q0 = gload4(q); q1 = gload4(q + 4);
                        }
                        w[mm] = species_weight<SqrtMid>(q0, q1.a, q1.d, xr, yr, zr);
                    }
                }
            }
        }
        species_sweeps(w, img, tile, uq, nbr, n, npad, nm, p, i, t, half, live, S, fun, row_of, m, agb, agb_on, F, Zout, agb_out);
        __syncthreads();
    }
}

#define DRAG_XLDS (BLOB_S * (2 * sizeof(int) + 1))
template <bool FILL>
__global__ __launch_bounds__(PASS_T, PASS_MINW) void blob_drag_kernel(int n, int npad, int k, int nblk,
                                                           const int* __restrict__ nbr,
                                                           const u16* __restrict__ slot16,
                                                           const int* __restrict__ uniq,
                                                           const int* __restrict__ qorder,
                                                           const RecB* __restrict__ recb,
                                                           const double* __restrict__ m,
                                                           const double* __restrict__ ptype,
                                                           const double* __restrict__ mgm,
                                                           const double* __restrict__ mcs,
                                                           const int* __restrict__ id, double* onto, DragScatter sc) {
    extern __shared__ double2 img[];
    u16* tile = reinterpret_cast<u16*>(img + (FILL ? 4 * BLOB_S : 0));
    int* cntL = reinterpret_cast<int*>(tile + KPAD(k) * BLOB_P);
    int* baseL = cntL + BLOB_S;
    unsigned char* dust = reinterpret_cast<unsigned char*>(baseL + BLOB_S);
    const int t = threadIdx.x / LPP, part = threadIdx.x & (LPP - 1);
    const int nm = KPAD(k) / LPP;
    for (int bi = blockIdx.x; bi < nblk; bi += gridDim.x) {
        const int b = xcd_block(bi, nblk);
        const int p = b * BLOB_P + t;
        const bool live = p < n;
        const int i = live ? qorder[p] : 0;
        const int* uq = uniq + (size_t)b * BLOB_S;
        if (FILL) {
            stage<0>(img, nullptr, tile, recb, nullptr, 0, nullptr, 0, uq, slot16, npad, k, b);
        } else {
            const int pieces = KPAD(k) * (BLOB_P / 8);
            for (int q = threadIdx.x; q < pieces; q += PASS_T) {
                const int kk = q / (BLOB_P / 8), c = q % (BLOB_P / 8);
                uint4 v = make_uint4(0xFFFFFFFFu, 0xFFFFFFFFu, 0xFFFFFFFFu, 0xFFFFFFFFu);
                if (kk < k) v = *reinterpret_cast<const uint4*>(slot16 + (size_t)kk * npad + (size_t)b * BLOB_P + c * 8);
                *reinterpret_cast<uint4*>(tile + kk * BLOB_P + c * 8) = v;
            }
        }
        for (int s = threadIdx.x; s < BLOB_S; s += PASS_T) {
            const int j = uq[s];
            dust[s] = (j >= 0 && ptype[j] == 2.0) ? 1 : 0;
            cntL[s] = 0;
        }
        __syncthreads();
        if (live) {
            for (int m0 = 0; m0 < nm; ++m0) {
                const int kk = LPP * m0 + part;
                const unsigned sl = tile[kk * BLOB_P + t];
                if (sl < SLOT_OVER) {
                    if (dust[sl] && uq[sl] != i) atomicAdd(&cntL[sl], 1);
                } else if (sl == SLOT_OVER && !FILL) {
                    const int j = nbr[(size_t)kk * npad + p];
                    if (j != i && ptype[j] == 2.0) atomicAdd(&sc.cnt[j], 1);
                }
            }
        }
        __syncthreads();
        if (!FILL) {
            for (int s = threadIdx.x; s < BLOB_S; s += PASS_T)
                if (cntL[s]) atomicAdd(&sc.cnt[uq[s]], cntL[s]);
            __syncthreads();
            continue;
        }
        for (int s = threadIdx.x; s < BLOB_S; s += PASS_T) {
            const int c = cntL[s];
            if (c) {
                const int j = uq[s];
                baseL[s] = sc.start[j] + atomicSub(&sc.cnt[j], c) - c;
                cntL[s] = 0;
            }
        }
        const double* rq = reinterpret_cast<const double*>(&recb[i]);
        const Q4 r0 = gload4(rq), rv = gload4(rq + 4);
        __syncthreads();
        double ox = 0.0, oy = 0.0, oz = 0.0;
        if (live) {
            unsigned dm = 0;
            for (int m0 = 0; m0 < nm; ++m0) {
                const int kk = LPP * m0 + part;
                const unsigned sl = tile[kk * BLOB_P + t];
                bool d = false;
                if (sl < SLOT_OVER) d = dust[sl] != 0;
                else if (sl == SLOT_OVER) d = ptype[nbr[(size_t)kk * npad + p]] == 2.0;
                dm |= (d ? 1u : 0u) << m0;
            }
            while (dm) {
                const int m0 = __builtin_ctz(dm);
                dm &= dm - 1;
                const int kk = LPP * m0 + part;
                const unsigned sl = tile[kk * BLOB_P + t];
                int j;
                Q4 q0, qv;
                if (sl < SLOT_OVER) {
                    j = uq[sl];
                    q0 = lload4(img, (int)sl, 0); qv = lload4(img, (int)sl, 1);
                } else {
                    j = nbr[(size_t)kk * npad + p];
                    const double* qb = reinterpret_cast<const double*>(&recb[j]);
                    q0 = gload4(qb); qv = gload4(qb + 4);
                }
                const Vec3 f = drag_term(ox, oy, oz, q0, qv, r0, rv, j, m, mgm, mcs);
                if (j != i) {
                    const int slot = (sl < SLOT_OVER) ? baseL[sl] + atomicAdd(&cntL[sl], 1)
                                                      : sc.start[j] + atomicSub(&sc.cnt[j], 1) - 1;
                    sphx_drag_put(sc, slot, ((u64)(unsigned)id[i] << 8) | (u64)kk, -f.x, -f.y, -f.z);
                }
            }
        }
        const double tx = group_total(ox), ty = group_total(oy), tz = group_total(oz);
        if (live && part == 0) { onto[3 * (size_t)i] = tx; onto[3 * (size_t)i + 1] = ty; onto[3 * (size_t)i + 2] = tz; }
        __syncthreads();
    }
}

BlobSel sphx_blob_sel(sphx_ctx* ctx, int part) {
    if (!ctx->blob_split_valid) return BlobSel{nullptr, nullptr, 0};
    const int* list = ctx->blob_split.as<int>();
    return BlobSel{list, list + (size_t)ctx->blob_split_nblk, part == 0 ? 3 : part};
}

int sphx_blob_grid(sphx_ctx* ctx, int nblk) {
    if (ctx->blob_grid <= 0) {
        int cus = 256;
        (void)hipDeviceGetAttribute(&cus, hipDeviceAttributeMultiprocessorCount, ctx->device);
        ctx->blob_grid = ((cus * 2 + 7) / 8) * 8;
    }
    return nblk < ctx->blob_grid ? nblk : ctx->blob_grid;
}

int sphx_lds_opt_in(sphx_ctx* ctx, const void* kernel, size_t bytes) {
    for (int q = 0; q < ctx->n_lds_raised; ++q)
        if (ctx->lds_raised[q] == kernel) return SPHX_OK;
    if (ctx->n_lds_raised == SPHX_LDS_KERNELS)
        return sphx_set_err(ctx, SPHX_E_HIP, "sphx_lds_opt_in: more than %d kernels", SPHX_LDS_KERNELS);
    HIPCHK(hipFuncSetAttribute(kernel, hipFuncAttributeMaxDynamicSharedMemorySize, (int)bytes));
    ctx->lds_raised[ctx->n_lds_raised++] = kernel;
    return SPHX_OK;
}

template <class Kern, class... Rest>
static int blob_launch(sphx_ctx* ctx, Kern kern, int per_slot, size_t extra, int64_t n, int k, Rest... rest) {
    const int64_t npad = sphx_pad64(n);
    const int nblk = (int)((npad + BLOB_P - 1) / BLOB_P);
    SPHX_TRY(sphx_lds_opt_in(ctx, reinterpret_cast<const void*>(kern), IMG_BYTES(per_slot, SPHX_MAX_K) + extra));
    hipLaunchKernelGGL(kern, dim3(sphx_blob_grid(ctx, nblk)), dim3(PASS_T), IMG_BYTES(per_slot, k) + extra, ctx->stream, (int)n,
                       (int)npad, k, nblk, ctx->nbr.as<int>(), ctx->slot16.as<u16>(), ctx->uniq.as<int>(), ctx->qorder, rest...);
    HIPCHK(hipGetLastError());
    return SPHX_OK;
}
static int blob_n_active(const sphx_ctx* ctx, int64_t n) { return ctx->map_perm ? ctx->map_nactive : (int)n; }

int sphx_blob_density(sphx_ctx* ctx, int64_t n, int k, bool lean) {
    return blob_launch(ctx, blob_density_kernel, 64, 0, n, k, ctx->clip_grad, ctx->map_perm, blob_n_active(ctx, n),
                       ctx->rec1.as<RecA>(), ctx->rho_s.as<double>(), ctx->rho.as<double>(), ctx->rhod.as<double>(),
                       ctx->nden.as<double>(), lean ? nullptr : ctx->G.as<double>(), ctx->ha.as<double>(),
                       sphx_blob_sel(ctx, ctx->pass_part));
}

int sphx_blob_pi(sphx_ctx* ctx, int64_t n, int k, u64* ct_bits) {
    return blob_launch(ctx, blob_pi_kernel, 72, 0, n, k, ctx->map_perm, blob_n_active(ctx, n), ctx->recv.as<RecB>(),
                       ctx->rho_s.as<double>(), ctx->self_s.as<RecSelf>(), ctx->bc_s.as<RecBC>(), ctx->Pi.as<double>(),
                       ctx->map_perm ? ctx->Bw.as<double>() : nullptr, ct_bits, sphx_blob_sel(ctx, ctx->pass_part));
}

int sphx_blob_visc(sphx_ctx* ctx, int64_t n, int k, const double* m) {
    return blob_launch(ctx, blob_visc_kernel, 72, 0, n, k, ctx->clip_grad, ctx->map_perm, blob_n_active(ctx, n),
                       ctx->recv.as<RecB>(), ctx->bc_s.as<RecBC>(), m, ctx->va.as<double>(), ctx->vh.as<double>(),
                       sphx_blob_sel(ctx, ctx->pass_part));
}

int sphx_blob_visc_pw(sphx_ctx* ctx, int64_t n, int k, const double* m, u64* ct_bits) {
    return blob_launch(ctx, blob_visc_pw_kernel, 72, 0, n, k, ctx->clip_grad, ctx->map_perm, blob_n_active(ctx, n),
                       ctx->recv.as<RecB>(), ctx->rho_s.as<double>(), ctx->bc_s.as<RecBC>(), ctx->self_s.as<RecSelf>(), m,
                       ctx->va.as<double>(), ctx->vh.as<double>(), ct_bits, sphx_blob_sel(ctx, ctx->pass_part));
}

int sphx_blob_density_species(sphx_ctx* ctx, int64_t n, int k, bool lean, int S, const double* fun, const int* row_of,
                              const double* m_sorted, double* F, double* Z, double* agb, int agb_on) {
    const auto kern = (KPAD(k) / LPP <= 10) ? blob_density_species_kernel<10> : blob_density_species_kernel<16>;
    return blob_launch(ctx, kern, 64, 0, n, k, ctx->clip_grad, ctx->rec1.as<RecA>(), ctx->rho_s.as<double>(), ctx->rho.as<double>(),
                       ctx->rhod.as<double>(), ctx->nden.as<double>(), lean ? nullptr : ctx->G.as<double>(),
                       ctx->ha.as<double>(), S, fun, row_of, m_sorted, ctx->agb, agb_on, F, Z, agb);
}

int sphx_blob_species(sphx_ctx* ctx, int64_t n, int k, int S, const double* fun, const int* row_of, const double* m_sorted, double* F,
                      double* Z, double* agb, int agb_on) {
    const auto kern = (KPAD(k) / LPP <= 10) ? blob_species_kernel<10> : blob_species_kernel<16>;
    return blob_launch(ctx, kern, 64, 0, n, k, S, ctx->rec1.as<RecA>(), fun, row_of, m_sorted, ctx->agb, agb_on, F, Z, agb);
}

int sphx_blob_drag(sphx_ctx* ctx, int64_t n, int k, bool count_only, const double* m, const double* ptype, const double* mgm,
                   const double* mcs, const int* id, double* onto, const DragScatter& sc) {
    if (count_only)
        return blob_launch(ctx, blob_drag_kernel<false>, 0, DRAG_XLDS, n, k, nullptr, m, ptype, mgm, mcs, id, onto, sc);
    return blob_launch(ctx, blob_drag_kernel<true>, 64, DRAG_XLDS, n, k, ctx->recv.as<RecB>(), m, ptype, mgm, mcs, id, onto, sc);
}
```

### sph-code_amd/csrc/sphx_internal.h

```cpp
#pragma once
#include <hip/hip_runtime.h>
#include <stdint.h>
#include <stdio.h>
#include <string.h>
#include <math.h>
#include <float.h>
#include <vector>
#include "../../include/sphx.h"
#include "sphx_agb.h"

#define SPHX_WAVE 64
#define SPHX_W6_C 1.5666814710608448

typedef unsigned long long u64;
typedef unsigned int u32;

struct DevBuf {
    void* p = nullptr;
    size_t cap = 0;
    template <class T> T* as() const { return (T*)p; }
};

struct __attribute__((aligned(64))) RecA {
    double x, y, z;
    double h2;
    double c1;
    double ms;
    double A;
    double Nw;
};
struct __attribute__((aligned(64))) RecB {
    double x, y, z, h2;
    double vx, vy, vz;
    double cs;
};
struct __attribute__((aligned(16))) RecBC {
    double Bw;
    double c1;
};
struct __attribute__((aligned(32))) RecSelf {
    double csi;
    double h;
    double mg;
    double pad;
};

struct GridParams {
    double xmin, ymin, zmin;
    double cell, inv_cell;
    int nx, ny, nz;
    int ncells;
    float fnx1, fny1, fnz1;
};

#define OLEV_N 32
#define OLEV_MAX 20
#define OLEV_MIN_RC 8.0f
struct OutLevels {
    int L;
    double cx, cy, cz;
    double hmax;
    const int* start;
    const int* list;
};
__device__ __forceinline__ bool sphx_outside_box(const GridParams& g, double x, double y, double z) {
    const double tx = (x - g.xmin) * g.inv_cell, ty = (y - g.ymin) * g.inv_cell, tz = (z - g.zmin) * g.inv_cell;
    return tx < 0.0 || tx >= (double)g.nx || ty < 0.0 || ty >= (double)g.ny || tz < 0.0 || tz >= (double)g.nz;
}

struct BlobBits { int bx, by, bz; int hilbert; };
__device__ __forceinline__ unsigned hilbert_rank(unsigned x, unsigned y, unsigned z, int b) {
    unsigned X[3] = {x, y, z};
    const unsigned M = 1u << (b - 1);
    for (unsigned Q = M; Q > 1; Q >>= 1) {
        const unsigned P = Q - 1;
#pragma unroll
        for (int i = 0; i < 3; ++i) {
            if (X[i] & Q) X[0] ^= P;
            else { const unsigned t = (X[0] ^ X[i]) & P; X[0] ^= t; X[i] ^= t; }
        }
    }
    X[1] ^= X[0]; X[2] ^= X[1];
    unsigned t = 0;
    for (unsigned Q = M; Q > 1; Q >>= 1)
        if (X[2] & Q) t ^= Q - 1;
    X[0] ^= t; X[1] ^= t; X[2] ^= t;
    unsigned out = 0;
    for (int q = 0; q < b; ++q) {
        out |= ((X[2] >> q) & 1u) << (3 * q);
        out |= ((X[1] >> q) & 1u) << (3 * q + 1);
        out |= ((X[0] >> q) & 1u) << (3 * q + 2);
    }
    return out;
}
__device__ __forceinline__ unsigned blob_rank(int cx, int cy, int cz, BlobBits b) {
    if (b.hilbert) return hilbert_rank((unsigned)cx, (unsigned)cy, (unsigned)cz, b.hilbert);
    unsigned out = 0;
    int pos = 0;
    for (int q = 0; q < 11; ++q) {
        if (q < b.bx) out |= (unsigned)((cx >> q) & 1) << pos++;
        if (q < b.by) out |= (unsigned)((cy >> q) & 1) << pos++;
        if (q < b.bz) out |= (unsigned)((cz >> q) & 1) << pos++;
    }
    return out;
}

struct StateArrays {
    DevBuf x, y, z, vx, vy, vz, ax, ay, az;
    DevBuf m, T, mu, gam, E, hprev;
    DevBuf ptype;
    DevBuf id;
    DevBuf fun;
    DevBuf mgm, mcs;
};

#define SPHX_LDS_KERNELS 16

struct sphx_ctx {
    int device = 0;
    hipStream_t stream = nullptr;
    hipStream_t own_stream = nullptr;
    hipStream_t side_stream = nullptr;
    sphx_constants cst;
    char tunables[1024] = {0};
    double rscale = 1.08, cell_factor = 0.55;
    double rscale_build = 1.3;
    bool use_verlet = false;
    bool use_blob = true;
    int blob_curve = 0;
    bool use_group = true;
    bool use_lds = true;
    bool drag_lds = true;
    bool blob_split_on = true;
    bool species_lds = true;
    bool species_fused = true;
    int blob_grid = 0;
    int blob_slots = 1 << 20;
    int olev_mode = 2;
    int distrust_mode = 0;
    bool cell_feedback = true;
    double cell_fb_hi = 0.30, cell_fb_lo = 0.10;
    int64_t max_cells = 0;
    double box_sigmas = 3.0;
    double h_clip_factor = 8.0;
    double reach_cap = 0.0;
    bool timing_detail = false;
    int clip_grad = 0;
    int visc_mode = 0;
    bool drag = false;
    int loop_forms = 0;
    double loop_d = 0.0;
    int gravity = 0;
    double grav_G = 0.0;
    int grav_order = 2;
    bool grav_per_thread = false;
    int grav_ws = 1;
    bool agb_on = false;
    AgbTable agb;
    double dev_hmean = 0.0;

    char err[512] = {0};
    sphx_stats stats;
    int64_t n = 0, npad = 0;
    int k = 0, s = 0;
    int sp = 0;
    bool has_state = false;
    int64_t step_count = 0;
    double dt_last = 0.0;
    bool tprev_valid = false;
    bool ct_primed = false;
    bool recs_pw = false;
    bool nbr_api_valid = false;
    int64_t nbr_api_n = 0;
    int nbr_api_k = 0;
    bool list_valid = false;
    int64_t list_n = 0;
    int list_k = 0;
    const int* map_perm = nullptr;
    int map_nactive = 0;
    const int* qorder = nullptr;
    bool blob_lists = false;
    bool blob_split_valid = false;
    int blob_split_nblk = 0;
    int pass_part = 0;
    bool loop2_interior_done = false;
    bool dev_ev_pending = false;
    const double *dev_drag_on = nullptr, *dev_drag_re = nullptr, *dev_drag_rho = nullptr, *dev_drag_rhod = nullptr;
    GridParams grid;
    const double* tbox = nullptr;
    double tbox_h[6] = {0, 0, 0, 0, 0, 0};
    double clip_lo[3] = {0, 0, 0}, clip_hi[3] = {0, 0, 0};
    bool clip_valid = false;
    double h_clip = 0.0;
    double cell_scale = 1.0;
    bool cells_unsorted = false;
    bool blob_scatter_pending = false;
    BlobBits blob_scatter_bits;
    const int* blob_scatter_mstart = nullptr;
    bool bbox_ticket_zeroed = false;
    const void* cell_fill_zeroed = nullptr;
    const void* mcount_zeroed = nullptr;
    int mcount_zeroed_M = 0;
    const void* fcount_zeroed = nullptr;
    int64_t fcount_zeroed_n = 0;
    const void* ds_cnt_zeroed = nullptr;
    const void* olev_fill_zeroed = nullptr;
    unsigned lbs_epoch[2] = {0u, 0u};
    const void* lds_raised[SPHX_LDS_KERNELS] = {nullptr};
    int n_lds_raised = 0;
    OutLevels olev;
    bool olev_ev_valid = false;
    u64 farq_seen = 0;
    int64_t farq_last = 0;
    int64_t list_len_last = 0;
    bool knn_lag_valid = false;
    u64 knn_lag[10] = {0, 0, 0, 0, 0, 0, 0, 0, 0, 0};
    u64 densep_seen = 0;
    int64_t densep_last = 0;
    u64 crowded_seen = 0;
    int64_t crowded_last = 0;
    bool distrust = false;
    u64 badhint_seen = 0;
    bool ev_detail[3] = {false, false, false};
    int ev_has07[3] = {0, 0, 0};
    unsigned ev_pending = 0;
    hipEvent_t lag_balias[2] = {nullptr, nullptr}, lag_halias[2] = {nullptr, nullptr};
    bool lag_bvalid[2] = {false, false}, lag_hvalid[2] = {false, false};
    int64_t lag_bn[2] = {0, 0};
    int lag_bslot = 0, lag_hslot = 0;

    std::vector<void*> allocs;
    DevBuf rec1, recv;
    DevBuf rho_s, bc_s, self_s;
    DevBuf drag_on, drag_re;
    DevBuf need_pyr;
    DevBuf fun_id;
    DevBuf crowded;
    DevBuf loop_side;
    DevBuf ds_cnt, ds_start, ds_ent;
    DevBuf lrec_a, lrec_v;
    DevBuf grav, grav_sort, grav_tmp;
    DevBuf grav_pyr, grav_cell;
    DevBuf grav_quad;
    DevBuf list64, dref, pos0, pos4;
    DevBuf nbr;
    DevBuf porder, mcount, mstart;
    DevBuf agb_knots, Zmet, agb_dust;
    DevBuf fail_list;
    DevBuf olev_start, olev_fill, olev_list, olev_key;
    DevBuf lbs_state[2];
    DevBuf cell_rank;
    DevBuf tie_list;
    DevBuf slot16, uniq;
    DevBuf blob_class, blob_split;
    DevBuf rho, rhod, nden, G, Pi, Bw, va, vh, ha, F;
    DevBuf scal;
    DevBuf cell_of, cell_start, cell_fill, perm, inv, scan_tmp, bbox_tmp;
    DevBuf in_a, in_b, in_c, in_d, in_e, in_f, in_g, in_h, in_i, in_j, out_a, out_b, out_c;
    DevBuf idx64, dist_out, nontriv, h_api;
    DevBuf arb_rec, arb_wrec, arb_flag, arb_cmax, arb_q, arb_key, arb_tmp, arb_acc, arb_out, arb_red;
    DevBuf arb_pos, arb_cs, arb_perm;
    int64_t arb_ball_id = 0, arb_ball_n = 0, arb_ball_m = 0;
    GridParams arb_g;
    double arb_tb[6] = {0, 0, 0, 0, 0, 0};
    double arb_ms[4] = {0, 0, 0, 0};
    hipEvent_t arb_ev[5] = {nullptr, nullptr, nullptr, nullptr, nullptr};
    StateArrays st, alt;
    DevBuf badc;
    DevBuf scal_tmp;
    DevBuf hsum_tmp;
    hipEvent_t ev_join = nullptr;
    hipEvent_t ev_perm = nullptr;
    hipEvent_t olev_ev = nullptr;
    hipEvent_t ev[10] = {nullptr};
    hipEvent_t evring[3][10] = {{nullptr}};
    hipEvent_t lag_bev[2] = {nullptr, nullptr}, lag_hev[2] = {nullptr, nullptr};
    void* pinned = nullptr;
};

int sphx_set_err(sphx_ctx* ctx, int code, const char* fmt, ...);
int sphx_ensure(sphx_ctx* ctx, DevBuf& b, size_t bytes, hipStream_t in_use_on);
static inline int sphx_ensure(sphx_ctx* ctx, DevBuf& b, size_t bytes) { return sphx_ensure(ctx, b, bytes, ctx->stream); }
void sphx_release(sphx_ctx* ctx, DevBuf& b);

#define HIPCHK(expr)                                                                         \
    do {                                                                                     \
        hipError_t e_ = (expr);                                                              \
        if (e_ != hipSuccess)                                                                \
            return sphx_set_err(ctx, SPHX_E_HIP, "%s:%d %s -> %s", __FILE__, __LINE__,       \
                                #expr, hipGetErrorString(e_));                               \
    } while (0)
#define NEED(p)                                                                              \
    do {                                                                                     \
        if (!(p)) return sphx_set_err(ctx, SPHX_E_ARG, "%s: argument %s is NULL", __func__, #p); \
    } while (0)
#define SPHX_TRY(expr)                                                                       \
    do {                                                                                     \
        int r_ = (expr);                                                                     \
        if (r_ != SPHX_OK) return r_;                                                        \
    } while (0)

static inline int64_t sphx_pad64(int64_t n) { return (n + 63) & ~int64_t(63); }

__device__ __forceinline__ int xcd_block(int b, int nb) {
    const int q = nb >> 3, r = nb & 7, x = b & 7, s = b >> 3;
    return x * q + (x < r ? x : r) + s;
}

#ifndef SPHX_SUM_PARTS
#define SPHX_SUM_PARTS 4
#endif

#define LAG_OFF 1024

__device__ __forceinline__ double sphx_nan_to_num(double v) {
    if (v != v) return 0.0;
    if (v > DBL_MAX) return DBL_MAX;
    if (v < -DBL_MAX) return -DBL_MAX;
    return v;
}

#define SPHX_CT_NONE 0x7FF0000000000000ull
int sphx_prime_ct(sphx_ctx* ctx, u64* ct_bits);

enum {
    SC_CT_BITS = 0,
    SC_DT = 1,
    SC_CAND = 2,
    SC_RETRY = 3,
    SC_HSUM = 4,
    SC_DISP2 = 5,
    SC_NFAIL = 6,
    SC_HCNT = 7,
    SC_GRAV_EPS = 8,
    SC_NFAILQ = 9,
    SC_SHORT = 10,
    SC_FARQ = 11,
    SC_BADHINT = 12,
    SC_CROWDED = 13,
    SC_DENSEP = 14,
    SC_KGDBG = 16,
    SC_NSLOTS = 24
};

enum {
    BAD_ACCEL = 0,
    BAD_ENERGY = 1,
    BAD_STATE = 2,
    BAD_H = 3,
    BADC_BUCKETS = 64, BADC_STRIDE = 16
};
int sphx_badc_read(sphx_ctx* ctx);

int sphx_bbox(sphx_ctx* ctx, int64_t n, const double* x, const double* y, const double* z,
              double out_minmax[13], bool use_clip);
int sphx_median(sphx_ctx* ctx, int64_t n, const double* v, double* out_dev);
int sphx_gravity_launch(sphx_ctx* ctx, int64_t n, const double* x, const double* y, const double* z, int ps,
                        const double* m, const double* eps_dev, double eps, double G, const int* omap,
                        double* acc);
int sphx_gravity_tree_launch(sphx_ctx* ctx, int64_t n, const double* x, const double* y, const double* z,
                             const double* m, int ws, const double* eps_dev, double eps, double G, const int* omap,
                             double* acc);
int sphx_dev_collect(sphx_ctx* ctx);
int sphx_loop_step_sums(sphx_ctx* ctx, int64_t n, int k, double d);
int sphx_build_blob_order(sphx_ctx* ctx, int64_t n, bool defer_scatter = false);
static inline double sphx_cell_feedback(sphx_ctx* ctx, int64_t n) {
    if (ctx->cell_feedback && n > 0) {
        const double dense = (double)ctx->densep_last / (double)n;
        if (dense > ctx->cell_fb_hi) ctx->cell_scale = ctx->cell_scale * 0.97 > 0.35 ? ctx->cell_scale * 0.97 : 0.35;
        else if (dense < ctx->cell_fb_lo) ctx->cell_scale = ctx->cell_scale * 1.01 < 1.0 ? ctx->cell_scale * 1.01 : 1.0;
    }
    return ctx->cell_scale;
}
int sphx_blob_translate(sphx_ctx* ctx, int64_t n, int k);
int sphx_blob_density_species(sphx_ctx* ctx, int64_t n, int k, bool lean, int S, const double* fun, const int* row_of,
                              const double* m_sorted, double* F, double* Z, double* agb, int agb_on);
int sphx_blob_density(sphx_ctx* ctx, int64_t n, int k, bool lean);
int sphx_blob_pi(sphx_ctx* ctx, int64_t n, int k, u64* ct_bits);
int sphx_blob_visc(sphx_ctx* ctx, int64_t n, int k, const double* m);
int sphx_blob_visc_pw(sphx_ctx* ctx, int64_t n, int k, const double* m, u64* ct_bits);
int sphx_blob_species(sphx_ctx* ctx, int64_t n, int k, int S, const double* fun, const int* row_of, const double* m_sorted, double* F,
                      double* Z, double* agb, int agb_on);
struct GridBuildOpts {
    bool lagged = false;
    hipEvent_t alias_ev = nullptr;
    bool sort_cells_later = false;
    double* clamp_vel[3] = {nullptr, nullptr, nullptr};
};
int sphx_build_grid(sphx_ctx* ctx, int64_t n, int k, const double* x, const double* y, const double* z, double cell_hint,
                    const GridBuildOpts& opts = GridBuildOpts());
int sphx_excl_scan_int(sphx_ctx* ctx, const int* in, int* out, int n);
struct alignas(32) DragEntry { u64 key; double x, y, z; };
struct DragScatter { int* cnt; const int* start; DragEntry* ent; };
__device__ __forceinline__ void sphx_drag_put(const DragScatter& sc, int slot, u64 key, double x, double y, double z) {
    double2* q = reinterpret_cast<double2*>(sc.ent + slot);
    q[0] = make_double2(__longlong_as_double((long long)key), x);
    q[1] = make_double2(y, z);
}
int sphx_drag_scatter_plan(sphx_ctx* ctx, int64_t n, int k, const int* nbr, const double* ptype, const int* qorder, DragScatter* out,
                           bool blob = false);
int sphx_drag_scatter_reduce(sphx_ctx* ctx, int64_t n, const DragScatter& d, double* react);
int sphx_blob_drag(sphx_ctx* ctx, int64_t n, int k, bool count_only, const double* m, const double* ptype, const double* mgm,
                   const double* mcs, const int* id, double* onto, const DragScatter& sc);
int sphx_build_outlier_levels(sphx_ctx* ctx, int64_t n, const double* xs, const double* ys, const double* zs);
struct KnnIn {
    const double *xs, *ys, *zs;
// ... 57 lines not shown
```

### sph-code_amd/csrc/sphx_loopforms.hip

```cpp
#include "sphx_internal.h"
#include "sphx_pair.h"
#pragma clang fp contract(off)
#include <float.h>

#define PI64 201.06192982974676

__device__ __forceinline__ double pow9(double d) {
    double d2 = d * d, d4 = d2 * d2;
    return d4 * d4 * d;
}
__device__ __forceinline__ double weigh2(double r2, double m, double d, double m0, double d9) {
    const double a = m0 / m;
    const double q = pow(m / m0, 2.0 / 3.0) * (d * d) - r2;
    return m * 315.0 * (a * a * a) * (q * q * q) / (PI64 * d9);
}
__device__ __forceinline__ double weigh2_dust(double r2, double m, double ds) {
    const double q = ds * ds - r2;
    return m * 315.0 * (q * q * q) / (PI64 * pow9(ds));
}
__device__ __forceinline__ double grad_coef(double r2, double m, double d, double m0, double d9, double tk) {
    const double a = m0 / m;
    const double q = pow(m / m0, 2.0 / 3.0) * (d * d) - r2;
    double c = -315.0 * 6.0 * (a * a * a) / (PI64 * d9) * (q * q) * ((tk == 0.0) ? 1.0 : 0.0);
    return (q > 0.0) ? c : 0.0;
// ... 337 lines not shown
    RecP2 v;
    v.x = r.x; v.y = r.y; v.z = r.z;
    const double cs = sphx_nan_to_num(sqrt(a.gam[i] * a.kB * a.T[i] / (a.mu[i] * a.amu)));
    v.css = gas ? cs : -(cs + 1.0);
    v.vx = a.vx[i]; v.vy = a.vy[i]; v.vz = a.vz[i];
    v.rho = 0.0;
    a.p2[i] = v;
}

struct L1Acc { double rho, rd, n, gx, gy, gz; };
__device__ __forceinline__ void loop1_term(L1Acc& a, const Q4& q0, const Q4& q1, double gam_j, double dm, double dh,
                                           double xi, double yi, double zi, double Ei, bool gas_i, double d9) {
    const double dx = q0.a - xi, dy = q0.b - yi, dz = q0.c - zi;
    const double r2 = dx * dx + dy * dy + dz * dz;
    const double q = q0.d - r2;
    const double w = q1.a * (q * q * q) / (PI64 * d9);
    const bool gas_j = q1.c > 0.0;
    const double vr = w * (gas_j ? 1.0 : 0.0);
    if (vr > 0.0) a.rho += vr;
    const double vn = w / fabs(q1.c);
    if (vn > 0.0) a.n += vn;
    if (dm >= 0.0) {
        const double vd = weigh2_dust(r2, dm, dh);
        if (vd > 0.0) a.rd += vd;
    }
    if (gas_i) {
        double c = q1.b * (q * q) * (gas_j ? 1.0 : 0.0);
        c = (q > 0.0) ? c : 0.0;
        const double f = (q1.d + Ei) / gam_j;
        a.gx += 0.5 * sphx_nan_to_num(c * dx) * f;
        a.gy += 0.5 * sphx_nan_to_num(c * dy) * f;
        a.gz += 0.5 * sphx_nan_to_num(c * dz) * f;
    }
}
struct L2Acc { double ax, ay, az, heat; };
__device__ __forceinline__ double loop2_term(L2Acc& a, const Q4& q0, const Q4& qv, double m_j, const Q4& s0,
                                             const Q4& sv, double rho_i, double m_i, double hq_i, double g1_i) {
    const double dvx = qv.a - sv.a, dvy = qv.b - sv.b, dvz = qv.c - sv.c;
    const double rel = dvx * dvx + dvy * dvy + dvz * dvz;
    if (q0.d < 0.0) return rel;
    const double dx = q0.a - s0.a, dy = q0.b - s0.b, dz = q0.c - s0.c;
    const double r2 = dx * dx + dy * dy + dz * dz;
    double w = (dvx * dx + dvy * dy + dvz * dz) / sqrt_mid(r2);
    w = (w > 0.0) ? 0.0 : w;
    w = sphx_nan_to_num(w);
    const double vsig = q0.d + s0.d - 3.0 * w;
    const double rho_ij = (qv.d + rho_i) / 2.0;
    const double PI = -0.5 * vsig * w / rho_ij;
    const double q = hq_i - r2;
    double c = g1_i * (q * q) * 1.0;
    c = (q > 0.0) ? c : 0.0;
    const double gwx = sphx_nan_to_num(c * dx), gwy = sphx_nan_to_num(c * dy), gwz = sphx_nan_to_num(c * dz);
    const double mb = (m_j + m_i) / 2.0;
    a.ax += mb * PI * gwx; a.ay += mb * PI * gwy; a.az += mb * PI * gwz;
    a.heat += 0.5 * mb * PI * (dvx * gwx + dvy * gwy + dvz * gwz);
    return rel;
}

#define LNB 4
__global__ __launch_bounds__(256) void loop_pass1_kernel(int n, int npad, int k, double d9,
                                                         const int* __restrict__ nbr,
                                                         const RecP1* __restrict__ p1,
                                                         const double* __restrict__ gam,
                                                         const double* __restrict__ pt, const double* __restrict__ m,
                                                         const double* __restrict__ h,
                                                         const int* __restrict__ qorder, double* rho, double* rhod,
                                                         double* nden, double* G, RecP2* p2) {
    const int p = xcd_block(blockIdx.x, gridDim.x) * blockDim.x + threadIdx.x;
    if (p >= n) return;
    const int i = qorder ? qorder[p] : p;
    const double* sp = reinterpret_cast<const double*>(&p1[i]);
    const Q4 s0 = gload4(sp), s1 = gload4(sp + 4);
    const bool gas_i = s1.c > 0.0;
    L1Acc acc[SPHX_SUM_PARTS] = {};
    for (int kk0 = 0; kk0 < k; kk0 += LNB) {
        int jb[LNB];
        Q4 q0b[LNB], q1b[LNB];
        double gb[LNB];
#pragma unroll
        for (int u = 0; u < LNB; ++u) jb[u] = (kk0 + u < k) ? nbr[(size_t)(kk0 + u) * npad + p] : -1;
#pragma unroll
        for (int u = 0; u < LNB; ++u) {
            const int jj = jb[u] < 0 ? i : jb[u];
            const double* q = reinterpret_cast<const double*>(&p1[jj]);
            q0b[u] = gload4(q); q1b[u] = gload4(q + 4);
            gb[u] = gam[jj];
        }
#pragma unroll
        for (int u = 0; u < LNB; ++u) {
            if (jb[u] < 0) continue;
            double dm = -1.0, dh = 0.0;
            if (!(q1b[u].c > 0.0) && pt[jb[u]] == 2.0) { dm = m[jb[u]]; dh = h[jb[u]]; }
            loop1_term(acc[u & (SPHX_SUM_PARTS - 1)], q0b[u], q1b[u], gb[u], dm, dh, s0.a, s0.b, s0.c, s1.d, gas_i, d9);
        }
    }
    const double s_rho = parts_total(acc, &L1Acc::rho);
    rho[i] = s_rho; rhod[i] = parts_total(acc, &L1Acc::rd); nden[i] = parts_total(acc, &L1Acc::n);
    G[3 * (size_t)i] = parts_total(acc, &L1Acc::gx); G[3 * (size_t)i + 1] = parts_total(acc, &L1Acc::gy);
    G[3 * (size_t)i + 2] = parts_total(acc, &L1Acc::gz);
    p2[i].rho = s_rho;
}

__global__ __launch_bounds__(256) void loop_pass2_kernel(int n, int npad, int k, const int* __restrict__ nbr,
                                                         const RecP1* __restrict__ p1,
                                                         const RecP2* __restrict__ p2,
                                                         const double* __restrict__ m, const double* __restrict__ h,
                                                         const int* __restrict__ qorder, double* va, double* vh,
                                                         u64* ct_bits) {
    const int p = xcd_block(blockIdx.x, gridDim.x) * blockDim.x + threadIdx.x;
    u64 mine = SPHX_CT_NONE;
    if (p < n) {
        const int i = qorder ? qorder[p] : p;
        const double* sp = reinterpret_cast<const double*>(&p2[i]);
        const Q4 s0 = gload4(sp), sv = gload4(sp + 4);
        double ax = 0.0, ay = 0.0, az = 0.0, heat = 0.0;
        if (s0.d >= 0.0) {
            const double hq_i = p1[i].hq, g1_i = p1[i].g1, m_i = m[i];
            L2Acc acc[SPHX_SUM_PARTS] = {};
            double mx = 0.0;
            for (int kk0 = 0; kk0 < k; kk0 += LNB) {
                int jb[LNB];
                Q4 q0b[LNB], qvb[LNB];
                double mb[LNB];
#pragma unroll
                for (int u = 0; u < LNB; ++u) jb[u] = (kk0 + u < k) ? nbr[(size_t)(kk0 + u) * npad + p] : -1;
#pragma unroll
                for (int u = 0; u < LNB; ++u) {
                    const int jj = jb[u] < 0 ? i : jb[u];
                    const double* q = reinterpret_cast<const double*>(&p2[jj]);
                    q0b[u] = gload4(q); qvb[u] = gload4(q + 4);
                    mb[u] = m[jj];
                }
#pragma unroll
                for (int u = 0; u < LNB; ++u) {
                    if (jb[u] < 0) continue;
                    mx = fmax(mx, loop2_term(acc[u & (SPHX_SUM_PARTS - 1)], q0b[u], qvb[u], mb[u], s0, sv, sv.d, m_i, hq_i,
                                             g1_i));
                }
            }
            ax = parts_total(acc, &L2Acc::ax); ay = parts_total(acc, &L2Acc::ay); az = parts_total(acc, &L2Acc::az);
            heat = parts_total(acc, &L2Acc::heat);
            mine = ct_vote_bits(h[i], mx);
        }
        va[3 * (size_t)i] = ax; va[3 * (size_t)i + 1] = ay; va[3 * (size_t)i + 2] = az;
        vh[i] = heat;
    }
    block_min_vote<256>(mine, ct_bits);
}

__global__ __launch_bounds__(PASS_T, PASS_MINW) void blob_loop1_kernel(int n, int npad, int k, int nblk, double d9,
                                                                          const int* __restrict__ nbr,
                                                                          const u16* __restrict__ slot16,
                                                                          const int* __restrict__ uniq,
                                                                          const int* __restrict__ qorder,
                                                                          const RecP1* __restrict__ p1,
                                                                          const double* __restrict__ side, double* rho,
                                                                          double* rhod, double* nden, double* G,
                                                                          RecP2* p2, BlobSel sel) {
    extern __shared__ double2 img[];
    double* lgam = reinterpret_cast<double*>(img + 4 * BLOB_S);
    u16* tile = reinterpret_cast<u16*>(lgam + BLOB_S);
    const int t = threadIdx.x / LPP, part = threadIdx.x & (LPP - 1);
    const int nsel = blob_sel_count(sel, nblk);
    for (int bi = blockIdx.x; bi < nsel; bi += gridDim.x) {
        const int b = blob_sel_at(sel, bi, nsel);
        const int p = b * BLOB_P + t;
        const int i = (p < n) ? qorder[p] : 0;
        stage<1>(img, lgam, tile, p1, side, 1, nullptr, 0, uniq + (size_t)b * BLOB_S, slot16, npad, k, b);
        const double* sp = reinterpret_cast<const double*>(&p1[i]);
        const Q4 s0 = gload4(sp), s1 = gload4(sp + 4);
        __syncthreads();
        if (p < n) {
            const bool gas_i = s1.c > 0.0;
            L1Acc a{0.0, 0.0, 0.0, 0.0, 0.0, 0.0};
            const int nm = KPAD(k) / LPP;
            for (int m0 = 0; m0 < nm; m0 += NB) {
                unsigned sl[NB];
                load_slots(sl, tile, m0, part, t);
                Q4 q0b[NB], q1b[NB];
                double gb[NB];
                int jb[NB];
                if (all_staged(sl)) {
#pragma unroll
                    for (int u = 0; u < NB; ++u) {
                        q0b[u] = lload4(img, (int)sl[u], 0); q1b[u] = lload4(img, (int)sl[u], 1); gb[u] = lgam[sl[u]];
                        jb[u] = -1;
                    }
                } else {
#pragma unroll
                    for (int u = 0; u < NB; ++u) {
                        jb[u] = -1;
                        if (sl[u] < SLOT_OVER) {
                            q0b[u] = lload4(img, (int)sl[u], 0); q1b[u] = lload4(img, (int)sl[u], 1); gb[u] = lgam[sl[u]];
                        } else if (sl[u] == SLOT_OVER) {
                            jb[u] = nbr[(size_t)(LPP * (m0 + u) + part) * npad + p];
                            const double* q = reinterpret_cast<const double*>(&p1[jb[u]]);
                            q0b[u] = gload4(q); q1b[u] = gload4(q + 4); gb[u] = side[jb[u]];
                        } else { q0b[u] = s0; q1b[u] = s1; gb[u] = 1.0; }
                    }
                }
#pragma unroll
                for (int u = 0; u < NB; ++u) {
                    if (sl[u] == SLOT_NONE) continue;
                    double dm = -1.0, dh = 0.0;
                    if (!(q1b[u].c > 0.0) && gb[u] >= 0.0) { dm = gb[u]; dh = q1b[u].b; }
                    loop1_term(a, q0b[u], q1b[u], gb[u], dm, dh, s0.a, s0.b, s0.c, s1.d, gas_i, d9);
                }
            }
            const double s_rho = group_total(a.rho), s_rd = group_total(a.rd), s_n = group_total(a.n);
            const double gx = group_total(a.gx), gy = group_total(a.gy), gz = group_total(a.gz);
            if (part == 0) {
                rho[i] = s_rho; rhod[i] = s_rd; nden[i] = s_n;
                G[3 * (size_t)i] = gx; G[3 * (size_t)i + 1] = gy; G[3 * (size_t)i + 2] = gz;
                p2[i].rho = s_rho;
            }
        }
        __syncthreads();
    }
}

__global__ __launch_bounds__(PASS_T, PASS_MINW) void blob_loop2_kernel(int n, int npad, int k, int nblk,
                                                                          const int* __restrict__ nbr,
                                                                          const u16* __restrict__ slot16,
                                                                          const int* __restrict__ uniq,
                                                                          const int* __restrict__ qorder,
                                                                          const RecP1* __restrict__ p1,
                                                                          const RecP2* __restrict__ p2,
                                                                          const double* __restrict__ m,
                                                                          const double* __restrict__ h, double* va,
                                                                          double* vh, u64* ct_bits, BlobSel sel) {
    extern __shared__ double2 img[];
    double* lm = reinterpret_cast<double*>(img + 4 * BLOB_S);
    u16* tile = reinterpret_cast<u16*>(lm + BLOB_S);
    const int t = threadIdx.x / LPP, part = threadIdx.x & (LPP - 1);
    u64 mine = SPHX_CT_NONE;
    const int nsel = blob_sel_count(sel, nblk);
    for (int bi = blockIdx.x; bi < nsel; bi += gridDim.x) {
        const int b = blob_sel_at(sel, bi, nsel);
        const int p = b * BLOB_P + t;
        const int i = (p < n) ? qorder[p] : 0;
        stage<1>(img, lm, tile, p2, m, 1, nullptr, 0, uniq + (size_t)b * BLOB_S, slot16, npad, k, b);
        const double* sp = reinterpret_cast<const double*>(&p2[i]);
        const Q4 s0 = gload4(sp), sv = gload4(sp + 4);
        const double hq_i = p1[i].hq, g1_i = p1[i].g1, m_i = m[i], h_i = h[i];
        __syncthreads();
        if (p < n) {
            L2Acc a{0.0, 0.0, 0.0, 0.0};
            double mx = 0.0;
            if (s0.d >= 0.0) {
                const int nm = KPAD(k) / LPP;
                for (int m0 = 0; m0 < nm; m0 += NB) {
                    unsigned sl[NB];
                    load_slots(sl, tile, m0, part, t);
                    Q4 q0b[NB], qvb[NB];
                    double mb[NB];
                    if (all_staged(sl)) {
#pragma unroll
                        for (int u = 0; u < NB; ++u) {
                            q0b[u] = lload4(img, (int)sl[u], 0); qvb[u] = lload4(img, (int)sl[u], 1); mb[u] = lm[sl[u]];
                        }
                    } else {
#pragma unroll
                        for (int u = 0; u < NB; ++u) {
                            if (sl[u] < SLOT_OVER) {
                                q0b[u] = lload4(img, (int)sl[u], 0); qvb[u] = lload4(img, (int)sl[u], 1); mb[u] = lm[sl[u]];
                            } else if (sl[u] == SLOT_OVER) {
                                const int j = nbr[(size_t)(LPP * (m0 + u) + part) * npad + p];
                                const double* q = reinterpret_cast<const double*>(&p2[j]);
                                q0b[u] = gload4(q); qvb[u] = gload4(q + 4); mb[u] = m[j];
                            } else { q0b[u] = s0; qvb[u] = sv; mb[u] = m_i; }
                        }
                    }
#pragma unroll
                    for (int u = 0; u < NB; ++u) {
                        if (sl[u] == SLOT_NONE) continue;
                        mx = fmax(mx, loop2_term(a, q0b[u], qvb[u], mb[u], s0, sv, sv.d, m_i, hq_i, g1_i));
                    }
                }
            }
            const double ax = group_total(a.ax), ay = group_total(a.ay), az = group_total(a.az), heat = group_total(a.heat);
            mx = group_max(mx);
            if (part == 0) {
                va[3 * (size_t)i] = ax; va[3 * (size_t)i + 1] = ay; va[3 * (size_t)i + 2] = az;
                vh[i] = heat;
                if (s0.d >= 0.0) {
                    const u64 cb = ct_vote_bits(h_i, mx);
                    mine = cb < mine ? cb : mine;
                }
            }
        }
        __syncthreads();
    }
    block_min_vote<PASS_T>(mine, ct_bits);
}

static int loop_prep_launch(sphx_ctx* ctx, int64_t n, double d, StateArrays& st) {
    const size_t nb = (size_t)n * sizeof(double);
    DevBuf* outs[] = {&ctx->rho, &ctx->rhod, &ctx->nden, &ctx->vh};
    for (DevBuf* b : outs) SPHX_TRY(sphx_ensure(ctx, *b, nb));
    SPHX_TRY(sphx_ensure(ctx, ctx->G, 3 * nb));
    SPHX_TRY(sphx_ensure(ctx, ctx->va, 3 * nb));
    SPHX_TRY(sphx_ensure(ctx, ctx->lrec_a, (size_t)n * sizeof(RecP1)));
    SPHX_TRY(sphx_ensure(ctx, ctx->lrec_v, (size_t)n * sizeof(RecP2)));
    LoopPrepArgs p;
    p.n = (int)n;
    p.x = st.x.as<double>(); p.y = st.y.as<double>(); p.z = st.z.as<double>();
    p.vx = st.vx.as<double>(); p.vy = st.vy.as<double>(); p.vz = st.vz.as<double>();
    p.m = st.m.as<double>(); p.pt = st.ptype.as<double>();
    p.mu = st.mu.as<double>(); p.gam = st.gam.as<double>(); p.E = st.E.as<double>(); p.T = st.T.as<double>();
    p.d = d; p.m0 = ctx->cst.m_0; p.m_h = ctx->cst.m_h; p.kB = ctx->cst.k_B; p.amu = ctx->cst.amu;
    p.p1 = ctx->lrec_a.as<RecP1>(); p.p2 = ctx->lrec_v.as<RecP2>();
    hipLaunchKernelGGL(loop_prep_kernel, dim3((unsigned)((n + 255) / 256)), dim3(256), 0, ctx->stream, p);
    HIPCHK(hipGetLastError());
    return SPHX_OK;
}
__global__ __launch_bounds__(256) void loop_dust_side_kernel(int n, const double* __restrict__ pt, const double* __restrict__ m,
                                                             const double* __restrict__ h, const double* __restrict__ gam,
                                                             RecP1* p1, double* side) {
    const int i = blockIdx.x * blockDim.x + threadIdx.x;
    if (i >= n) return;
    const double t = pt[i];
    if (t == 0.0) { side[i] = gam[i]; return; }
    if (t == 2.0) { side[i] = m[i]; p1[i].g1 = h[i]; }
    else side[i] = -1.0;
}
static int loop_pass1_launch(sphx_ctx* ctx, int64_t n, int k, double d, StateArrays& st, const double* h) {
    const double d2 = d * d, d4 = d2 * d2, d9 = d4 * d4 * d;
    const int npad = (int)sphx_pad64(n);
    RecP1* p1 = ctx->lrec_a.as<RecP1>(); RecP2* p2 = ctx->lrec_v.as<RecP2>();
    if (ctx->qorder && ctx->blob_lists) {
        SPHX_TRY(sphx_lds_opt_in(ctx, reinterpret_cast<const void*>(blob_loop1_kernel), IMG_BYTES(72, SPHX_MAX_K)));
        const int nblk = (npad + BLOB_P - 1) / BLOB_P;
        const int g = sphx_blob_grid(ctx, nblk);
        SPHX_TRY(sphx_ensure(ctx, ctx->loop_side, (size_t)n * sizeof(double)));
        hipLaunchKernelGGL(loop_dust_side_kernel, dim3((unsigned)((n + 255) / 256)), dim3(256), 0, ctx->stream, (int)n,
                           st.ptype.as<double>(), st.m.as<double>(), h, st.gam.as<double>(), p1, ctx->loop_side.as<double>());
        hipLaunchKernelGGL(blob_loop1_kernel, dim3(g), dim3(PASS_T), IMG_BYTES(72, k), ctx->stream, (int)n, npad, k, nblk,
                           d9, ctx->nbr.as<int>(), ctx->slot16.as<u16>(), ctx->uniq.as<int>(), ctx->qorder, p1,
                           ctx->loop_side.as<double>(),
                           ctx->rho.as<double>(), ctx->rhod.as<double>(), ctx->nden.as<double>(), ctx->G.as<double>(), p2,
                           sphx_blob_sel(ctx, 0));
    } else {
        hipLaunchKernelGGL(loop_pass1_kernel, dim3((unsigned)((n + 255) / 256)), dim3(256), 0, ctx->stream, (int)n, npad, k, d9,
                           ctx->nbr.as<int>(), p1, st.gam.as<double>(), st.ptype.as<double>(), st.m.as<double>(),
                           h, ctx->qorder, ctx->rho.as<double>(), ctx->rhod.as<double>(),
                           ctx->nden.as<double>(), ctx->G.as<double>(), p2);
    }
    HIPCHK(hipGetLastError());
    return SPHX_OK;
}
static int loop_pass2_launch(sphx_ctx* ctx, int64_t n, int k, StateArrays& st, const double* h, u64* ct, int part = 0) {
    const int npad = (int)sphx_pad64(n);
    RecP1* p1 = ctx->lrec_a.as<RecP1>(); RecP2* p2 = ctx->lrec_v.as<RecP2>();
    if (ctx->qorder && ctx->blob_lists) {
        SPHX_TRY(sphx_lds_opt_in(ctx, reinterpret_cast<const void*>(blob_loop2_kernel), IMG_BYTES(72, SPHX_MAX_K)));
        const int nblk = (npad + BLOB_P - 1) / BLOB_P;
        const int g = sphx_blob_grid(ctx, nblk);
        hipLaunchKernelGGL(blob_loop2_kernel, dim3(g), dim3(PASS_T), IMG_BYTES(72, k), ctx->stream, (int)n, npad, k, nblk,
                           ctx->nbr.as<int>(), ctx->slot16.as<u16>(), ctx->uniq.as<int>(), ctx->qorder, p1, p2,
                           st.m.as<double>(), h, ctx->va.as<double>(), ctx->vh.as<double>(), ct, sphx_blob_sel(ctx, part));
    } else {
        hipLaunchKernelGGL(loop_pass2_kernel, dim3((unsigned)((n + 255) / 256)), dim3(256), 0, ctx->stream, (int)n, npad, k,
                           ctx->nbr.as<int>(), p1, p2, st.m.as<double>(), h, ctx->qorder, ctx->va.as<double>(),
                           ctx->vh.as<double>(), ct);
    }
    HIPCHK(hipGetLastError());
    return SPHX_OK;
}

int sphx_loop_step_sums(sphx_ctx* ctx, int64_t n, int k, double d) {
    StateArrays& st = ctx->st;
    SPHX_TRY(loop_prep_launch(ctx, n, d, st));
    u64* ct = ctx->scal.as<u64>() + SC_CT_BITS;
    if (!ctx->ct_primed) SPHX_TRY(sphx_prime_ct(ctx, ct));
    ctx->ct_primed = false;
    SPHX_TRY(loop_pass1_launch(ctx, n, k, d, st, st.hprev.as<double>()));
    SPHX_TRY(loop_pass2_launch(ctx, n, k, st, st.hprev.as<double>(), ct));
    return SPHX_OK;
}

struct DevGatherArgs {
    int n;
    const int* perm;
    const double *pos, *vel, *m, *T, *mu, *gam, *pt, *E;
    double *x, *y, *z, *vx, *vy, *vz, *sm, *sT, *smu, *sgam, *spt, *sE;
};
__global__ __launch_bounds__(256) void dev_gather_state_kernel(DevGatherArgs a) {
    const int s = blockIdx.x * blockDim.x + threadIdx.x;
    if (s >= a.n) return;
    const size_t c = (size_t)a.perm[s];
    a.x[s] = a.pos[3 * c]; a.y[s] = a.pos[3 * c + 1]; a.z[s] = a.pos[3 * c + 2];
    a.vx[s] = a.vel[3 * c]; a.vy[s] = a.vel[3 * c + 1]; a.vz[s] = a.vel[3 * c + 2];
    a.sm[s] = a.m[c]; a.sT[s] = a.T[c]; a.smu[s] = a.mu[c]; a.sgam[s] = a.gam[c]; a.spt[s] = a.pt[c]; a.sE[s] = a.E[c];
}
__global__ __launch_bounds__(256) void dev_to_sorted_kernel(int n, const int* perm, int n_active, int owned_only,
                                                            const double* src, double* dst) {
    const int s = blockIdx.x * blockDim.x + threadIdx.x;
    if (s >= n) return;
    const int c = perm[s];
    dst[s] = (owned_only && c >= n_active) ? 0.0 : src[c];
}
__global__ __launch_bounds__(256) void dev_rho_to_records_kernel(int n, const int* perm, const double* rho, RecP2* p2) {
    const int s = blockIdx.x * blockDim.x + threadIdx.x;
    if (s < n) p2[s].rho = rho[perm[s]];
}
__global__ __launch_bounds__(256) void dev_to_caller_kernel(int n, const int* perm, int n_active, int w,
                                                            const double* src, double* dst) {
    const int s = blockIdx.x * blockDim.x + threadIdx.x;
    if (s >= n) return;
    const int c = perm[s];
    if (c >= n_active) return;
    for (int q = 0; q < w; ++q) dst[(size_t)c * w + q] = src[(size_t)s * w + q];
}

extern "C" int sphx_dev_loop_prep(sphx_ctx* ctx, const double* pos, const double* vel, const double* mass,
                                  const double* T, const double* mu, const double* gamma, const double* ptype,
                                  const double* E_internal, double d) {
    if (!ctx) return SPHX_E_ARG;
    NEED(pos); NEED(vel); NEED(mass); NEED(T); NEED(mu); NEED(gamma); NEED(ptype); NEED(E_internal);
    if (!ctx->map_perm) return sphx_set_err(ctx, SPHX_E_STATE, "sphx_dev_loop_prep before sphx_dev_search");
    if (!(d > 0.0)) return sphx_set_err(ctx, SPHX_E_ARG, "sphx_dev_loop_prep: d must be positive");
    HIPCHK(hipSetDevice(ctx->device));
    const int64_t n = ctx->n;
    StateArrays& st = ctx->alt;
    DevBuf* bufs[] = {&st.x, &st.y, &st.z, &st.vx, &st.vy, &st.vz, &st.m, &st.T, &st.mu, &st.gam, &st.ptype, &st.E,
                      &st.hprev, &st.ax};
    for (DevBuf* b : bufs) SPHX_TRY(sphx_ensure(ctx, *b, (size_t)n * sizeof(double)));
    DevGatherArgs g;
    g.n = (int)n; g.perm = ctx->map_perm;
    g.pos = pos; g.vel = vel; g.m = mass; g.T = T; g.mu = mu; g.gam = gamma; g.pt = ptype; g.E = E_internal;
    g.x = st.x.as<double>(); g.y = st.y.as<double>(); g.z = st.z.as<double>();
    g.vx = st.vx.as<double>(); g.vy = st.vy.as<double>(); g.vz = st.vz.as<double>();
    g.sm = st.m.as<double>(); g.sT = st.T.as<double>(); g.smu = st.mu.as<double>(); g.sgam = st.gam.as<double>();
    g.spt = st.ptype.as<double>(); g.sE = st.E.as<double>();
    hipLaunchKernelGGL(dev_gather_state_kernel, dim3((unsigned)((n + 255) / 256)), dim3(256), 0, ctx->stream, g);
    HIPCHK(hipGetLastError());
    ctx->loop_d = d;
    return loop_prep_launch(ctx, n, d, st);
}

extern "C" int sphx_dev_loop_pass1(sphx_ctx* ctx, const double* h_complete, double* rho, double* rho_dust, double* nden,
                                   double* delp) {
    if (!ctx) return SPHX_E_ARG;
    NEED(h_complete);
    if (!ctx->map_perm || !(ctx->loop_d > 0.0)) return sphx_set_err(ctx, SPHX_E_STATE, "sphx_dev_loop_pass1 before sphx_dev_loop_prep");
    HIPCHK(hipSetDevice(ctx->device));
    const int64_t n = ctx->n;
    const unsigned grid = (unsigned)((n + 255) / 256);
    StateArrays& st = ctx->alt;
    hipLaunchKernelGGL(dev_to_sorted_kernel, dim3(grid), dim3(256), 0, ctx->stream, (int)n, ctx->map_perm, ctx->map_nactive, 0,
                       h_complete, st.hprev.as<double>());
    hipLaunchKernelGGL(dev_to_sorted_kernel, dim3(grid), dim3(256), 0, ctx->stream, (int)n, ctx->map_perm, ctx->map_nactive, 1,
                       h_complete, st.ax.as<double>());
    SPHX_TRY(loop_pass1_launch(ctx, n, ctx->k, ctx->loop_d, st, st.hprev.as<double>()));
    struct O { double* dst; const double* src; int w; } outs[] = {{rho, ctx->rho.as<double>(), 1}, {rho_dust, ctx->rhod.as<double>(), 1},
                                                                   {nden, ctx->nden.as<double>(), 1}, {delp, ctx->G.as<double>(), 3}};
    for (O& o : outs)
        if (o.dst)
            hipLaunchKernelGGL(dev_to_caller_kernel, dim3(grid), dim3(256), 0, ctx->stream, (int)n, ctx->map_perm,
                               ctx->map_nactive, o.w, o.src, o.dst);
    HIPCHK(hipGetLastError());
    return SPHX_OK;
}

extern "C" int sphx_dev_loop_pass2_interior(sphx_ctx* ctx) {
    if (!ctx) return SPHX_E_ARG;
    if (!ctx->map_perm || !(ctx->loop_d > 0.0))
        return sphx_set_err(ctx, SPHX_E_STATE, "sphx_dev_loop_pass2_interior before sphx_dev_loop_pass1");
    ctx->loop2_interior_done = false;
    if (!(ctx->qorder && ctx->blob_lists && ctx->blob_split_valid)) return 0;
    HIPCHK(hipSetDevice(ctx->device));
    u64* ct = ctx->scal.as<u64>() + SC_CT_BITS;
    SPHX_TRY(sphx_prime_ct(ctx, ct));
    ctx->ct_primed = false;
    SPHX_TRY(loop_pass2_launch(ctx, ctx->n, ctx->k, ctx->alt, ctx->alt.ax.as<double>(), ct, 1));
    ctx->loop2_interior_done = true;
    return 1;
}

extern "C" int sphx_dev_loop_pass2(sphx_ctx* ctx, const double* rho_complete, double* visc_accel, double* visc_heat,
                                   double* ct_out) {
    if (!ctx) return SPHX_E_ARG;
    NEED(rho_complete);
    if (!ctx->map_perm || !(ctx->loop_d > 0.0)) return sphx_set_err(ctx, SPHX_E_STATE, "sphx_dev_loop_pass2 before sphx_dev_loop_prep");
    HIPCHK(hipSetDevice(ctx->device));
    const int64_t n = ctx->n;
    const unsigned grid = (unsigned)((n + 255) / 256);
    StateArrays& st = ctx->alt;
    hipLaunchKernelGGL(dev_rho_to_records_kernel, dim3(grid), dim3(256), 0, ctx->stream, (int)n, ctx->map_perm, rho_complete,
                       ctx->lrec_v.as<RecP2>());
    u64* ct = ctx->scal.as<u64>() + SC_CT_BITS;
    const bool rest_only = ctx->loop2_interior_done;
    ctx->loop2_interior_done = false;
    if (!rest_only) SPHX_TRY(sphx_prime_ct(ctx, ct));
    ctx->ct_primed = false;
    SPHX_TRY(loop_pass2_launch(ctx, n, ctx->k, st, st.ax.as<double>(), ct, rest_only ? 2 : 0));
    if (visc_accel)
        hipLaunchKernelGGL(dev_to_caller_kernel, dim3(grid), dim3(256), 0, ctx->stream, (int)n, ctx->map_perm, ctx->map_nactive,
                           3, ctx->va.as<double>(), visc_accel);
    if (visc_heat)
        hipLaunchKernelGGL(dev_to_caller_kernel, dim3(grid), dim3(256), 0, ctx->stream, (int)n, ctx->map_perm, ctx->map_nactive,
                           1, ctx->vh.as<double>(), visc_heat);
    HIPCHK(hipGetLastError());
    if (ct_out)
        HIPCHK(hipMemcpyAsync(ct_out, ct, 8, hipMemcpyDeviceToDevice, ctx->stream));
    return SPHX_OK;
}
```

Before: 817.1 million.

## Drop LDS slot tile, load slot indices into registers, add per-pass stage caps

The blob passes stop staging the per-block u16 slot tile into LDS. Each thread now reads its neighbor slot indices straight from global memory, either into packed registers (density) or via a one-batch-ahead prefetch (loop passes). Staged-image capacity becomes a template and runtime parameter per pass (DENS_S/PI_S/VISC_S and a pass-slots cap), and workgroups-per-CU become per-kernel launch-bound knobs. The aim is to cut LDS footprint and raise occupancy, at the cost of more registers and global slot loads. A debug API for reporting distinct counts per block is also added.

```diff
diff --git a/include/sphx.h b/include/sphx.h
--- a/include/sphx.h
+++ b/include/sphx.h
@@ -174,6 +174,7 @@
 int sphx_arb_last_timing(sphx_ctx* ctx, double ms[4]);
 int sphx_get_stats(sphx_ctx* ctx, sphx_stats* out);
 int sphx_reset_stats(sphx_ctx* ctx);
+int sphx_blob_distinct_counts(sphx_ctx* ctx, int64_t cap, int32_t* counts, int64_t* nblk);
 
 int sphx_set_stream(sphx_ctx* ctx, void* hip_stream );
 int sphx_reset_stream(sphx_ctx* ctx);
diff --git a/sph-code_amd/_lib.py b/sph-code_amd/_lib.py
--- a/sph-code_amd/_lib.py
+++ b/sph-code_amd/_lib.py
@@ -84,6 +84,7 @@
     "sphx_state_sample": (C.c_int, [_P, C.c_double, _D, _D, C.c_int64, _D, C.c_double] + [_D] * 5 + [_I, _I]),
     "sphx_get_stats": (C.c_int, [_P, C.POINTER(SphxStats)]),
     "sphx_reset_stats": (C.c_int, [_P]),
+    "sphx_blob_distinct_counts": (C.c_int, [_P, C.c_int64, C.POINTER(C.c_int32), _I]),
     "sphx_set_stream": (C.c_int, [_P, C.c_void_p]),
     "sphx_reset_stream": (C.c_int, [_P]),
     "sphx_sync": (C.c_int, [_P]),
@@ -266,6 +267,14 @@
     def reset_stats(self):
         self.check(self.lib.sphx_reset_stats(self.h))
 
+    def blob_distinct_counts(self):
+        nblk = C.c_int64(0)
+        self.check(self.lib.sphx_blob_distinct_counts(self.h, 0, None, C.byref(nblk)))
+        out = np.zeros(nblk.value, np.int32)
+        self.check(self.lib.sphx_blob_distinct_counts(self.h, out.size, out.ctypes.data_as(C.POINTER(C.c_int32)),
+                                                      C.byref(nblk)))
+        return out
+
     def build_info(self):
         return {"library": self.lib.sphx_build_info().decode(), "tunables": self.lib.sphx_tunables(self.h).decode(),
                 "lib_path": LIB_PATH}
diff --git a/sph-code_amd/csrc/sphx_api.hip b/sph-code_amd/csrc/sphx_api.hip
--- a/sph-code_amd/csrc/sphx_api.hip
+++ b/sph-code_amd/csrc/sphx_api.hip
@@ -124,11 +124,8 @@
     if (const char* e = env("SPHX_GRAV_WS")) { int v = atoi(e); if (v >= 1 && v <= 4) ctx->grav_ws = v; }
     if (const char* e = env("SPHX_LDS")) ctx->use_lds = atoi(e) != 0;
     if (const char* e = env("SPHX_BLOB_SLOTS")) ctx->blob_slots = atoi(e);
-    if (const char* e = env("SPHX_BLOB_WGS")) {
-        int cus = 256;
-        (void)hipDeviceGetAttribute(&cus, hipDeviceAttributeMultiprocessorCount, ctx->device);
-        if (atoi(e) > 0) ctx->blob_grid = ((cus * atoi(e) + 7) / 8) * 8;
-    }
+    if (const char* e = env("SPHX_BLOB_PASS_SLOTS")) ctx->blob_pass_slots = atoi(e);
+    if (const char* e = env("SPHX_BLOB_WGS")) { if (atoi(e) > 0) ctx->blob_wgs = atoi(e); }
     bool ok = hipSetDevice(device) == hipSuccess &&
               sphx_stream_create(&ctx->stream, 0) == hipSuccess &&
               hipHostMalloc(&ctx->pinned, 16384, hipHostMallocDefault) == hipSuccess;
diff --git a/sph-code_amd/csrc/sphx_blob.h b/sph-code_amd/csrc/sphx_blob.h
--- a/sph-code_amd/csrc/sphx_blob.h
+++ b/sph-code_amd/csrc/sphx_blob.h
@@ -17,9 +17,26 @@
 #ifndef BLOB_STAGE_PRIO
 #define BLOB_STAGE_PRIO 1
 #endif
-#ifndef PASS_MINW
-#define PASS_MINW 4
-#endif
+#ifndef DENS_S
+#define DENS_S BLOB_S
+#endif
+#ifndef PI_S
+#define PI_S BLOB_S
+#endif
+#ifndef VISC_S
+#define VISC_S BLOB_S
+#endif
+#ifndef DENS_WGS
+#define DENS_WGS 2
+#endif
+#ifndef PI_WGS
+#define PI_WGS 2
+#endif
+#ifndef VISC_WGS
+#define VISC_WGS 2
+#endif
+#define PASS_MINW_OF(wgs) ((wgs) * PASS_T / 256)
+#define PASS_MINW PASS_MINW_OF(2)
 #define BLOB_PROBES 96
 #define SLOT_NONE 0xFFFFu
 #define SLOT_OVER 0xFFFEu
@@ -31,9 +48,10 @@
     return (unsigned)(((u64)((unsigned)j * 2654435761u) * (u64)BLOB_S) >> 32);
 }
 
+template <int CAP = BLOB_S>
 __device__ __forceinline__ Q4 lload4(const double2* img, int s, int c2) {
-    const double2 lo = img[(2 * c2) * BLOB_S + s];
-    const double2 hi = img[(2 * c2 + 1) * BLOB_S + s];
+    const double2 lo = img[(2 * c2) * CAP + s];
+    const double2 hi = img[(2 * c2 + 1) * CAP + s];
     return Q4{lo.x, lo.y, hi.x, hi.y};
 }
 __device__ __forceinline__ double sqrt_mid(double x) {
@@ -74,24 +92,97 @@
     return v;
 }
 
-#define NSTAGE ((BLOB_S + PASS_T - 1) / PASS_T)
+#define NSTAGE_OF(cap) (((cap) + PASS_T - 1) / PASS_T)
+#define NSTAGE NSTAGE_OF(BLOB_S)
 #define NB (8 / LPP)
 #define KPAD(k) ((((k) + 7) / 8) * 8)
-#define IMG_BYTES(per_slot, k) ((size_t)BLOB_S * (per_slot) + (size_t)KPAD(k) * BLOB_P * sizeof(u16))
-
-template <int NSIDE, class Rec>
-__device__ __forceinline__ void stage(double2* img, double* side, u16* tile, const Rec* __restrict__ rec,
+#define IMG_BYTES(cap, per_slot) ((size_t)(cap) * (per_slot))
+#define TILE_BYTES(k) ((size_t)KPAD(k) * BLOB_P * sizeof(u16))
+
+template <int NSIDE, int CAP, class Rec>
+__device__ __forceinline__ void stage(double2* img, double* side, const Rec* __restrict__ rec,
                                       const double* __restrict__ g0, int g0_stride,
                                       const double* __restrict__ g1, int g1_stride,
-                                      const int* __restrict__ uq, const u16* __restrict__ slot16, int npad,
-                                      int k, int b) {
+                                      const int* __restrict__ uq, int cap) {
     __builtin_amdgcn_s_setprio(BLOB_STAGE_PRIO);
-    int ju[NSTAGE];
-#pragma unroll
-    for (int r = 0; r < NSTAGE; ++r) {
+    constexpr int NS = NSTAGE_OF(CAP);
+    int ju[NS];
+#pragma unroll
+    for (int r = 0; r < NS; ++r) {
         const int s = threadIdx.x + r * PASS_T;
-        ju[r] = (s < BLOB_S) ? uq[s] : -1;
-    }
+        ju[r] = (s < cap) ? uq[s] : -1;
+    }
+    double2 c[NS][4];
+    double e0[NS], e1[NS];
+#pragma unroll
+    for (int r = 0; r < NS; ++r) {
+        const int j = ju[r] < 0 ? 0 : ju[r];
+        const double2* g = reinterpret_cast<const double2*>(&rec[j]);
+        c[r][0] = g[0]; c[r][1] = g[1]; c[r][2] = g[2]; c[r][3] = g[3];
+        e0[r] = (NSIDE > 0) ? g0[(size_t)j * g0_stride] : 0.0;
+        e1[r] = (NSIDE > 1) ? g1[(size_t)j * g1_stride] : 0.0;
+    }
+#pragma unroll
+    for (int r = 0; r < NS; ++r) {
+        const int s = threadIdx.x + r * PASS_T;
+        if (ju[r] >= 0) {
+            if (NSIDE == 2) c[r][3].y = e0[r];
+            img[0 * CAP + s] = c[r][0]; img[1 * CAP + s] = c[r][1];
+            img[2 * CAP + s] = c[r][2]; img[3 * CAP + s] = c[r][3];
+            if (NSIDE == 1) side[s] = e0[r];
+            if (NSIDE == 2) side[s] = e1[r];
+        }
+    }
+    __builtin_amdgcn_s_setprio(0);
+}
+
+#define MAXB (SPHX_MAX_K / 8)
+#define PKW (NB / 2)
+struct SlotRegs { unsigned pk[MAXB][PKW]; };
+__device__ __forceinline__ void load_slot_regs(SlotRegs& r, unsigned& ref, const u16* __restrict__ slot16, int npad, int k,
+                                               int p, int half, bool live) {
+    const unsigned lane = (unsigned)half * (unsigned)npad + (unsigned)p;
+    ref = live ? (unsigned)slot16[(unsigned)p] : SLOT_NONE;
+#pragma unroll
+    for (int bt = 0; bt < MAXB; ++bt) {
+#pragma unroll
+        for (int w = 0; w < PKW; ++w) {
+            const int r0 = LPP * (NB * bt + 2 * w), r1 = r0 + LPP;
+            const u16* row0 = slot16 + (size_t)r0 * npad;
+            const u16* row1 = slot16 + (size_t)r1 * npad;
+            unsigned lo = SLOT_NONE, hi = SLOT_NONE;
+            if (live && r0 + half < k) lo = row0[lane];
+            if (live && r1 + half < k) hi = row1[lane];
+            r.pk[bt][w] = lo | (hi << 16);
+        }
+    }
+}
+__device__ __forceinline__ void next_slots(unsigned (&sl)[NB], SlotRegs& r) {
+#pragma unroll
+    for (int w = 0; w < PKW; ++w) { sl[2 * w] = r.pk[0][w] & 0xFFFFu; sl[2 * w + 1] = r.pk[0][w] >> 16; }
+#pragma unroll
+    for (int bt = 0; bt + 1 < MAXB; ++bt) {
+#pragma unroll
+        for (int w = 0; w < PKW; ++w) r.pk[bt][w] = r.pk[bt + 1][w];
+    }
+}
+__device__ __forceinline__ unsigned slot_lane(int npad, int p, int half) { return (unsigned)half * (unsigned)npad + (unsigned)p; }
+__device__ __forceinline__ void load_batch_slots(unsigned (&sl)[NB], const u16* __restrict__ slot16, int npad, int k, int m0,
+                                                 unsigned lane, int half, bool live) {
+#pragma unroll
+    for (int u = 0; u < NB; ++u) {
+        const int r = LPP * (m0 + u);
+        sl[u] = (live && r + half < k) ? (unsigned)(slot16 + (size_t)r * npad)[lane] : SLOT_NONE;
+    }
+}
+__device__ __forceinline__ bool all_staged(const unsigned (&sl)[NB], unsigned cap) {
+    unsigned worst = sl[0];
+#pragma unroll
+    for (int u = 1; u < NB; ++u) worst = worst > sl[u] ? worst : sl[u];
+    return __ballot(worst >= cap) == 0ull;
+}
+
+__device__ __forceinline__ void stage_tile(u16* tile, const u16* __restrict__ slot16, int npad, int k, int b) {
     const int pieces = KPAD(k) * (BLOB_P / 8);
     for (int q = threadIdx.x; q < pieces; q += PASS_T) {
         const int kk = q / (BLOB_P / 8), c = q % (BLOB_P / 8);
@@ -99,39 +190,10 @@
         if (kk < k) v = *reinterpret_cast<const uint4*>(slot16 + (size_t)kk * npad + (size_t)b * BLOB_P + c * 8);
         *reinterpret_cast<uint4*>(tile + kk * BLOB_P + c * 8) = v;
     }
-    double2 c[NSTAGE][4];
-    double e0[NSTAGE], e1[NSTAGE];
-#pragma unroll
-    for (int r = 0; r < NSTAGE; ++r) {
-        const int j = ju[r] < 0 ? 0 : ju[r];
-        const double2* g = reinterpret_cast<const double2*>(&rec[j]);
-        c[r][0] = g[0]; c[r][1] = g[1]; c[r][2] = g[2]; c[r][3] = g[3];
-        e0[r] = (NSIDE > 0) ? g0[(size_t)j * g0_stride] : 0.0;
-        e1[r] = (NSIDE > 1) ? g1[(size_t)j * g1_stride] : 0.0;
-    }
-#pragma unroll
-    for (int r = 0; r < NSTAGE; ++r) {
-        const int s = threadIdx.x + r * PASS_T;
-        if (ju[r] >= 0) {
-            if (NSIDE == 2) c[r][3].y = e0[r];
-            img[0 * BLOB_S + s] = c[r][0]; img[1 * BLOB_S + s] = c[r][1];
-            img[2 * BLOB_S + s] = c[r][2]; img[3 * BLOB_S + s] = c[r][3];
-            if (NSIDE == 1) side[s] = e0[r];
-            if (NSIDE == 2) side[s] = e1[r];
-        }
-    }
-    __builtin_amdgcn_s_setprio(0);
-}
-
+}
 __device__ __forceinline__ void load_slots(unsigned (&sl)[NB], const u16* tile, int m0, int half, int t) {
 #pragma unroll
     for (int u = 0; u < NB; ++u) sl[u] = tile[(LPP * (m0 + u) + half) * BLOB_P + t];
-}
-__device__ __forceinline__ bool all_staged(const unsigned (&sl)[NB]) {
-    unsigned worst = sl[0];
-#pragma unroll
-    for (int u = 1; u < NB; ++u) worst = worst > sl[u] ? worst : sl[u];
-    return __ballot(worst >= SLOT_OVER) == 0ull;
 }
 
 
@@ -146,5 +208,9 @@
 }
 BlobSel sphx_blob_sel(sphx_ctx* ctx, int part);
 
-int sphx_blob_grid(sphx_ctx* ctx, int nblk);
+int sphx_blob_grid(sphx_ctx* ctx, int nblk, int wgs);
+static inline int sphx_pass_slots(const sphx_ctx* ctx, int cap) {
+    const int q = ctx->blob_pass_slots < 1 ? 1 : ctx->blob_pass_slots;
+    return q < cap ? q : cap;
+}
 int sphx_lds_opt_in(sphx_ctx* ctx, const void* kernel, size_t bytes);
diff --git a/sph-code_amd/csrc/sphx_blob.hip b/sph-code_amd/csrc/sphx_blob.hip
--- a/sph-code_amd/csrc/sphx_blob.hip
+++ b/sph-code_amd/csrc/sphx_blob.hip
@@ -187,19 +187,43 @@
     }
     HIPCHK(hipGetLastError());
     ctx->blob_lists = true;
+    ctx->blob_nblk = nblk;
     return SPHX_OK;
 }
 
-template <bool FAST, bool CLIP>
-__device__ __forceinline__ void density_batch(DensAcc& a, double (&wout)[NB], const unsigned (&sl)[NB], const double2* img,
+extern "C" int sphx_blob_distinct_counts(sphx_ctx* ctx, int64_t cap, int32_t* counts, int64_t* nblk_out) {
+    if (!ctx || !nblk_out || (cap > 0 && !counts)) return SPHX_E_ARG;
+    if (!ctx->blob_lists || ctx->blob_nblk < 1)
+        return sphx_set_err(ctx, SPHX_E_STATE, "sphx_blob_distinct_counts: no slot lists (LDS passes off, or no search yet)");
+    const int64_t nblk = ctx->blob_nblk;
+    *nblk_out = nblk;
+    const int64_t m = cap < nblk ? cap : nblk;
+    if (m < 1) return SPHX_OK;
+    int* host = (int*)malloc((size_t)m * BLOB_S * sizeof(int));
+    if (!host) return sphx_set_err(ctx, SPHX_E_NOMEM, "sphx_blob_distinct_counts: out of host memory");
+    HIPCHK(hipSetDevice(ctx->device));
+    hipError_t e = hipMemcpyAsync(host, ctx->uniq.as<int>(), (size_t)m * BLOB_S * sizeof(int), hipMemcpyDeviceToHost, ctx->stream);
+    if (e == hipSuccess) e = hipStreamSynchronize(ctx->stream);
+    if (e != hipSuccess) { free(host); HIPCHK(e); }
+    for (int64_t b = 0; b < m; ++b) {
+        int c = 0;
+        while (c < BLOB_S && host[b * BLOB_S + c] >= 0) ++c;
+        counts[b] = c;
+    }
+    free(host);
+    return SPHX_OK;
+}
+
+template <bool FAST, bool CLIP, int CAP>
+__device__ __forceinline__ void density_batch(DensAcc& a, double (&wout)[NB], const unsigned (&sl)[NB], unsigned cap, const double2* img,
                                               const RecA* __restrict__ rec, const int* __restrict__ nbr,
                                               size_t col0, size_t colstep, double xr, double yr, double zr,
                                               double hi2, double ci, double Ai) {
     Q4 q0b[NB], q1b[NB];
 #pragma unroll
     for (int u = 0; u < NB; ++u) {
-        if (FAST || sl[u] < SLOT_OVER) { q0b[u] = lload4(img, (int)sl[u], 0); q1b[u] = lload4(img, (int)sl[u], 1); }
-        else if (sl[u] == SLOT_OVER) {
+        if (FAST || sl[u] < cap) { q0b[u] = lload4<CAP>(img, (int)sl[u], 0); q1b[u] = lload4<CAP>(img, (int)sl[u], 1); }
+        else if (sl[u] != SLOT_NONE) {
             const double* q = reinterpret_cast<const double*>(&rec[nbr[col0 + u * colstep]]);
             q0b[u] = gload4(q); q1b[u] = gload4(q + 4);
         } else { q0b[u] = Q4{xr, yr, zr, 0.0}; q1b[u] = Q4{0.0, 0.0, 0.0, 0.0}; }
@@ -213,52 +237,48 @@
     }
 }
 
-__global__ __launch_bounds__(PASS_T, PASS_MINW) void blob_density_kernel(int n, int npad, int k, int nblk,
+__global__ __launch_bounds__(PASS_T, PASS_MINW_OF(DENS_WGS)) void blob_density_kernel(int n, int npad, int k, int nblk,
                                                               const int* __restrict__ nbr,
                                                               const u16* __restrict__ slot16,
                                                               const int* __restrict__ uniq,
-                                                              const int* __restrict__ qorder, int clip,
+                                                              const int* __restrict__ qorder, int cap, int clip,
                                                               const int* __restrict__ omap, int n_active,
                                                               const RecA* __restrict__ rec, double* rho_s,
                                                               double* rho, double* rhod, double* nden, double* G,
                                                               double* ha, BlobSel sel) {
     extern __shared__ double2 img[];
-    u16* tile = reinterpret_cast<u16*>(img + 4 * BLOB_S);
     const int t = threadIdx.x / LPP, half = threadIdx.x & (LPP - 1);
+    const unsigned ucap = (unsigned)cap;
     const int nsel = blob_sel_count(sel, nblk);
     for (int bi = blockIdx.x; bi < nsel; bi += gridDim.x) {
         const int b = blob_sel_at(sel, bi, nsel);
         const int p = b * BLOB_P + t;
         const int i = (p < n) ? qorder[p] : 0;
-        stage<0>(img, nullptr, tile, rec, nullptr, 0, nullptr, 0, uniq + (size_t)b * BLOB_S, slot16, npad, k, b);
+        SlotRegs sr;
+        unsigned sl0;
+        load_slot_regs(sr, sl0, slot16, npad, k, p, half, p < n);
+        stage<0, DENS_S>(img, nullptr, rec, nullptr, 0, nullptr, 0, uniq + (size_t)b * BLOB_S, cap);
         const double* self = reinterpret_cast<const double*>(&rec[i]);
         const Q4 s0 = gload4(self), s1 = gload4(self + 4);
         const int o = (p < n) ? (omap ? omap[i] : i) : 0x7FFFFFFF;
         __syncthreads();
         if (o < n_active) {
             double xr = s0.a, yr = s0.b, zr = s0.c;
-            {
-                const unsigned sl0 = tile[t];
-                if (sl0 < SLOT_OVER) { const Q4 r = lload4(img, (int)sl0, 0); xr = r.a; yr = r.b; zr = r.c; }
-                else if (sl0 == SLOT_OVER) { const int j0 = nbr[p]; xr = rec[j0].x; yr = rec[j0].y; zr = rec[j0].z; }
-            }
+            if (sl0 < ucap) { const Q4 r = lload4<DENS_S>(img, (int)sl0, 0); xr = r.a; yr = r.b; zr = r.c; }
+            else if (sl0 != SLOT_NONE) { const int j0 = nbr[p]; xr = rec[j0].x; yr = rec[j0].y; zr = rec[j0].z; }
             const double hi2 = s0.d, ci = -6.0 * s1.a, Ai = s1.c;
             DensAcc a{0.0, 0.0, 0.0, 0.0, 0.0, 0.0};
             const int nm = KPAD(k) / LPP;
-            unsigned sl[NB];
-            load_slots(sl, tile, 0, half, t);
             for (int m0 = 0; m0 < nm; m0 += NB) {
                 unsigned cur[NB];
-#pragma unroll
-                for (int u = 0; u < NB; ++u) cur[u] = sl[u];
-                if (m0 + NB < nm) load_slots(sl, tile, m0 + NB, half, t);
+                next_slots(cur, sr);
                 const size_t col0 = (size_t)(LPP * m0 + half) * npad + p;
-                const bool fast = all_staged(cur);
+                const bool fast = all_staged(cur, ucap);
                 double wo[NB];
-                if (fast && !clip) density_batch<true, false>(a, wo, cur, img, rec, nbr, col0, LPP * (size_t)npad, xr, yr, zr, hi2, ci, Ai);
-                else if (fast) density_batch<true, true>(a, wo, cur, img, rec, nbr, col0, LPP * (size_t)npad, xr, yr, zr, hi2, ci, Ai);
-                else if (!clip) density_batch<false, false>(a, wo, cur, img, rec, nbr, col0, LPP * (size_t)npad, xr, yr, zr, hi2, ci, Ai);
-                else density_batch<false, true>(a, wo, cur, img, rec, nbr, col0, LPP * (size_t)npad, xr, yr, zr, hi2, ci, Ai);
+                if (fast && !clip) density_batch<true, false, DENS_S>(a, wo, cur, ucap, img, rec, nbr, col0, LPP * (size_t)npad, xr, yr, zr, hi2, ci, Ai);
+                else if (fast) density_batch<true, true, DENS_S>(a, wo, cur, ucap, img, rec, nbr, col0, LPP * (size_t)npad, xr, yr, zr, hi2, ci, Ai);
+                else if (!clip) density_batch<false, false, DENS_S>(a, wo, cur, ucap, img, rec, nbr, col0, LPP * (size_t)npad, xr, yr, zr, hi2, ci, Ai);
+                else density_batch<false, true, DENS_S>(a, wo, cur, ucap, img, rec, nbr, col0, LPP * (size_t)npad, xr, yr, zr, hi2, ci, Ai);
             }
             const double s_rho = group_total(a.rho), s_rd = group_total(a.rd), s_n = group_total(a.n);
             const double gx = group_total(a.gx), gy = group_total(a.gy), gz = group_total(a.gz);
@@ -275,8 +295,8 @@
     }
 }
 
-template <bool FAST>
-__device__ __forceinline__ void pi_batch(double& s_pi, double& maxrel, const unsigned (&sl)[NB], const double2* img,
+template <bool FAST, int CAP>
+__device__ __forceinline__ void pi_batch(double& s_pi, double& maxrel, const unsigned (&sl)[NB], unsigned cap, const double2* img,
                                          const double* lrho, const RecB* __restrict__ recb,
                                          const double* __restrict__ rho_s, const int* __restrict__ nbr, size_t col0,
                                          size_t colstep, const Q4& r0, const Q4& rv, double rho_i, double cs_i) {
@@ -284,10 +304,10 @@
     double rhob[NB];
 #pragma unroll
     for (int u = 0; u < NB; ++u) {
-        if (FAST || sl[u] < SLOT_OVER) {
-            q0b[u] = lload4(img, (int)sl[u], 0); qvb[u] = lload4(img, (int)sl[u], 1);
+        if (FAST || sl[u] < cap) {
+            q0b[u] = lload4<CAP>(img, (int)sl[u], 0); qvb[u] = lload4<CAP>(img, (int)sl[u], 1);
             rhob[u] = lrho[sl[u]];
-        } else if (sl[u] == SLOT_OVER) {
+        } else if (sl[u] != SLOT_NONE) {
             const int jj = nbr[col0 + u * colstep];
             const double* qb = reinterpret_cast<const double*>(&recb[jj]);
             q0b[u] = gload4(qb); qvb[u] = gload4(qb + 4);
@@ -304,27 +324,30 @@
     }
 }
 
-__global__ __launch_bounds__(PASS_T, PASS_MINW) void blob_pi_kernel(int n, int npad, int k, int nblk,
+__global__ __launch_bounds__(PASS_T, PASS_MINW_OF(PI_WGS)) void blob_pi_kernel(int n, int npad, int k, int nblk,
                                                          const int* __restrict__ nbr,
                                                          const u16* __restrict__ slot16,
                                                          const int* __restrict__ uniq,
-                                                         const int* __restrict__ qorder,
+                                                         const int* __restrict__ qorder, int cap,
                                                          const int* __restrict__ omap, int n_active,
                                                          const RecB* __restrict__ recb,
                                                          const double* __restrict__ rho_s,
                                                          const RecSelf* __restrict__ selfr, RecBC* bc, double* Pi,
                                                          double* BwOut, u64* ct_bits, BlobSel sel) {
     extern __shared__ double2 img[];
-    double* lrho = reinterpret_cast<double*>(img + 4 * BLOB_S);
-    u16* tile = reinterpret_cast<u16*>(lrho + BLOB_S);
+    double* lrho = reinterpret_cast<double*>(img + 4 * PI_S);
     const int t = threadIdx.x / LPP, half = threadIdx.x & (LPP - 1);
+    const unsigned ucap = (unsigned)cap;
     u64 my_ct = SPHX_CT_NONE;
     const int nsel = blob_sel_count(sel, nblk);
     for (int bi = blockIdx.x; bi < nsel; bi += gridDim.x) {
         const int b = blob_sel_at(sel, bi, nsel);
         const int p = b * BLOB_P + t;
         const int i = (p < n) ? qorder[p] : 0;
-        stage<1>(img, lrho, tile, recb, rho_s, 1, nullptr, 0, uniq + (size_t)b * BLOB_S, slot16, npad, k, b);
+        SlotRegs sr;
+        unsigned sl0;
+        load_slot_regs(sr, sl0, slot16, npad, k, p, half, p < n);
+        stage<1, PI_S>(img, lrho, recb, rho_s, 1, nullptr, 0, uniq + (size_t)b * BLOB_S, cap);
         const RecSelf sf = selfr[i];
         const double rho_i = rho_s[i];
         const double* selfq = reinterpret_cast<const double*>(&recb[i]);
@@ -333,29 +356,22 @@
         __syncthreads();
         if (o < n_active) {
             Q4 r0 = self0, rv = selfv;
-            {
-                const unsigned sl0 = tile[t];
-                if (sl0 < SLOT_OVER) { r0 = lload4(img, (int)sl0, 0); rv = lload4(img, (int)sl0, 1); }
-                else if (sl0 == SLOT_OVER) {
-                    const double* rq = reinterpret_cast<const double*>(&recb[nbr[p]]);
-                    r0 = gload4(rq); rv = gload4(rq + 4);
-                }
+            if (sl0 < ucap) { r0 = lload4<PI_S>(img, (int)sl0, 0); rv = lload4<PI_S>(img, (int)sl0, 1); }
+            else if (sl0 != SLOT_NONE) {
+                const double* rq = reinterpret_cast<const double*>(&recb[nbr[p]]);
+                r0 = gload4(rq); rv = gload4(rq + 4);
             }
             const double cs_i = sf.csi, ms_i = sf.mg, h_i = sf.h;
             double s_pi = 0.0, maxrel = 0.0;
             const int nm = KPAD(k) / LPP;
-            unsigned sl[NB];
-            load_slots(sl, tile, 0, half, t);
             for (int m0 = 0; m0 < nm; m0 += NB) {
                 unsigned cur[NB];
-#pragma unroll
-                for (int u = 0; u < NB; ++u) cur[u] = sl[u];
-                if (m0 + NB < nm) load_slots(sl, tile, m0 + NB, half, t);
+                next_slots(cur, sr);
                 const size_t col0 = (size_t)(LPP * m0 + half) * npad + p;
-                if (all_staged(cur))
-                    pi_batch<true>(s_pi, maxrel, cur, img, lrho, recb, rho_s, nbr, col0, LPP * (size_t)npad, r0, rv, rho_i, cs_i);
+                if (all_staged(cur, ucap))
+                    pi_batch<true, PI_S>(s_pi, maxrel, cur, ucap, img, lrho, recb, rho_s, nbr, col0, LPP * (size_t)npad, r0, rv, rho_i, cs_i);
                 else
-                    pi_batch<false>(s_pi, maxrel, cur, img, lrho, recb, rho_s, nbr, col0, LPP * (size_t)npad, r0, rv, rho_i, cs_i);
+                    pi_batch<false, PI_S>(s_pi, maxrel, cur, ucap, img, lrho, recb, rho_s, nbr, col0, LPP * (size_t)npad, r0, rv, rho_i, cs_i);
             }
             s_pi = group_total(s_pi);
             maxrel = group_max(maxrel);
@@ -375,8 +391,8 @@
     block_min_vote<PASS_T>(my_ct, ct_bits);
 }
 
-template <bool FAST, bool CLIP>
-__device__ __forceinline__ void visc_batch(ViscAcc& a, const unsigned (&sl)[NB], const double2* img,
+template <bool FAST, bool CLIP, int CAP>
+__device__ __forceinline__ void visc_batch(ViscAcc& a, const unsigned (&sl)[NB], unsigned cap, const double2* img,
                                            const double* lc1, const RecB* __restrict__ recb,
                                            const RecBC* __restrict__ bc, const int* __restrict__ nbr, size_t col0,
                                            size_t colstep, const Q4& r0, const Q4& rv, double hi2, double ci,
@@ -385,10 +401,10 @@
     double c1b[NB];
 #pragma unroll
     for (int u = 0; u < NB; ++u) {
-        if (FAST || sl[u] < SLOT_OVER) {
-            q0b[u] = lload4(img, (int)sl[u], 0); qvb[u] = lload4(img, (int)sl[u], 1);
+        if (FAST || sl[u] < cap) {
+            q0b[u] = lload4<CAP>(img, (int)sl[u], 0); qvb[u] = lload4<CAP>(img, (int)sl[u], 1);
             c1b[u] = lc1[sl[u]];
-        } else if (sl[u] == SLOT_OVER) {
+        } else if (sl[u] != SLOT_NONE) {
             const int jj = nbr[col0 + u * colstep];
             const double* qb = reinterpret_cast<const double*>(&recb[jj]);
             q0b[u] = gload4(qb); qvb[u] = gload4(qb + 4);
@@ -404,27 +420,30 @@
     }
 }
 
-__global__ __launch_bounds__(PASS_T, PASS_MINW) void blob_visc_kernel(int n, int npad, int k, int nblk,
+__global__ __launch_bounds__(PASS_T, PASS_MINW_OF(VISC_WGS)) void blob_visc_kernel(int n, int npad, int k, int nblk,
                                                            const int* __restrict__ nbr,
                                                            const u16* __restrict__ slot16,
                                                            const int* __restrict__ uniq,
-                                                           const int* __restrict__ qorder, int clip,
+                                                           const int* __restrict__ qorder, int cap, int clip,
                                                            const int* __restrict__ omap, int n_active,
                                                            const RecB* __restrict__ recb,
                                                            const RecBC* __restrict__ bc,
                                                            const double* __restrict__ m, double* va, double* vh,
                                                            BlobSel sel) {
     extern __shared__ double2 img[];
-    double* lc1 = reinterpret_cast<double*>(img + 4 * BLOB_S);
-    u16* tile = reinterpret_cast<u16*>(lc1 + BLOB_S);
+    double* lc1 = reinterpret_cast<double*>(img + 4 * VISC_S);
     const int t = threadIdx.x / LPP, half = threadIdx.x & (LPP - 1);
+    const unsigned ucap = (unsigned)cap;
     const double* bcd = reinterpret_cast<const double*>(bc);
     const int nsel = blob_sel_count(sel, nblk);
     for (int bi = blockIdx.x; bi < nsel; bi += gridDim.x) {
         const int b = blob_sel_at(sel, bi, nsel);
         const int p = b * BLOB_P + t;
         const int i = (p < n) ? qorder[p] : 0;
-        stage<2>(img, lc1, tile, recb, bcd, 2, bcd + 1, 2, uniq + (size_t)b * BLOB_S, slot16, npad, k, b);
+        SlotRegs sr;
+        unsigned sl0;
+        load_slot_regs(sr, sl0, slot16, npad, k, p, half, p < n);
+        stage<2, VISC_S>(img, lc1, recb, bcd, 2, bcd + 1, 2, uniq + (size_t)b * BLOB_S, cap);
         const double2 bci = *reinterpret_cast<const double2*>(&bc[i]);
         const double* selfq = reinterpret_cast<const double*>(&recb[i]);
         const Q4 self0 = gload4(selfq), selfv = gload4(selfq + 4);
@@ -433,30 +452,23 @@
         __syncthreads();
         if (o < n_active) {
             Q4 r0 = self0, rv = selfv;
-            {
-                const unsigned sl0 = tile[t];
-                if (sl0 < SLOT_OVER) { r0 = lload4(img, (int)sl0, 0); rv = lload4(img, (int)sl0, 1); }
-                else if (sl0 == SLOT_OVER) {
-                    const double* rq = reinterpret_cast<const double*>(&recb[nbr[p]]);
-                    r0 = gload4(rq); rv = gload4(rq + 4);
-                }
+            if (sl0 < ucap) { r0 = lload4<VISC_S>(img, (int)sl0, 0); rv = lload4<VISC_S>(img, (int)sl0, 1); }
+            else if (sl0 != SLOT_NONE) {
+                const double* rq = reinterpret_cast<const double*>(&recb[nbr[p]]);
+                r0 = gload4(rq); rv = gload4(rq + 4);
             }
             const double hi2 = self0.d, ci = -6.0 * bci.y, Bi = bci.x;
             ViscAcc a{0.0, 0.0, 0.0, 0.0};
             const int nm = KPAD(k) / LPP;
-            unsigned sl[NB];
-            load_slots(sl, tile, 0, half, t);
             for (int m0 = 0; m0 < nm; m0 += NB) {
                 unsigned cur[NB];
-#pragma unroll
-                for (int u = 0; u < NB; ++u) cur[u] = sl[u];
-                if (m0 + NB < nm) load_slots(sl, tile, m0 + NB, half, t);
+                next_slots(cur, sr);
                 const size_t col0 = (size_t)(LPP * m0 + half) * npad + p;
-                const bool fast = all_staged(cur);
-                if (fast && !clip) visc_batch<true, false>(a, cur, img, lc1, recb, bc, nbr, col0, LPP * (size_t)npad, r0, rv, hi2, ci, Bi);
-                else if (fast) visc_batch<true, true>(a, cur, img, lc1, recb, bc, nbr, col0, LPP * (size_t)npad, r0, rv, hi2, ci, Bi);
-                else if (!clip) visc_batch<false, false>(a, cur, img, lc1, recb, bc, nbr, col0, LPP * (size_t)npad, r0, rv, hi2, ci, Bi);
-                else visc_batch<false, true>(a, cur, img, lc1, recb, bc, nbr, col0, LPP * (size_t)npad, r0, rv, hi2, ci, Bi);
+                const bool fast = all_staged(cur, ucap);
+                if (fast && !clip) visc_batch<true, false, VISC_S>(a, cur, ucap, img, lc1, recb, bc, nbr, col0, LPP * (size_t)npad, r0, rv, hi2, ci, Bi);
+                else if (fast) visc_batch<true, true, VISC_S>(a, cur, ucap, img, lc1, recb, bc, nbr, col0, LPP * (size_t)npad, r0, rv, hi2, ci, Bi);
+                else if (!clip) visc_batch<false, false, VISC_S>(a, cur, ucap, img, lc1, recb, bc, nbr, col0, LPP * (size_t)npad, r0, rv, hi2, ci, Bi);
+                else visc_batch<false, true, VISC_S>(a, cur, ucap, img, lc1, recb, bc, nbr, col0, LPP * (size_t)npad, r0, rv, hi2, ci, Bi);
             }
             const double ax = group_total(a.x), ay = group_total(a.y), az = group_total(a.z), heat = group_total(a.h);
             if (!half) {
@@ -468,8 +480,8 @@
     }
 }
 
-template <bool FAST, bool CLIP>
-__device__ __forceinline__ void visc_pw_batch(ViscAcc& a, double& maxrel, const unsigned (&sl)[NB], const double2* img,
+template <bool FAST, bool CLIP, int CAP>
+__device__ __forceinline__ void visc_pw_batch(ViscAcc& a, double& maxrel, const unsigned (&sl)[NB], unsigned cap, const double2* img,
                                               const double* lrho, const RecB* __restrict__ recb,
                                               const double* __restrict__ rho_s, const RecBC* __restrict__ bc,
                                               const int* __restrict__ nbr, size_t col0, size_t colstep, const Q4& r0,
@@ -478,11 +490,11 @@
     double rhob[NB], mcb[NB];
 #pragma unroll
     for (int u = 0; u < NB; ++u) {
-        if (FAST || sl[u] < SLOT_OVER) {
-            q0b[u] = lload4(img, (int)sl[u], 0); qvb[u] = lload4(img, (int)sl[u], 1);
+        if (FAST || sl[u] < cap) {
+            q0b[u] = lload4<CAP>(img, (int)sl[u], 0); qvb[u] = lload4<CAP>(img, (int)sl[u], 1);
             rhob[u] = lrho[sl[u]];
             mcb[u] = bc[nbr[col0 + u * colstep]].Bw;
-        } else if (sl[u] == SLOT_OVER) {
+        } else if (sl[u] != SLOT_NONE) {
             const int jj = nbr[col0 + u * colstep];
             const double* qb = reinterpret_cast<const double*>(&recb[jj]);
             q0b[u] = gload4(qb); qvb[u] = gload4(qb + 4);
@@ -501,7 +513,7 @@
                                                               const int* __restrict__ nbr,
                                                               const u16* __restrict__ slot16,
                                                               const int* __restrict__ uniq,
-                                                              const int* __restrict__ qorder, int clip,
+                                                              const int* __restrict__ qorder, int cap, int clip,
                                                               const int* __restrict__ omap, int n_active,
                                                               const RecB* __restrict__ recb,
                                                               const double* __restrict__ rho_s,
@@ -511,15 +523,16 @@
                                                               u64* ct_bits, BlobSel sel) {
     extern __shared__ double2 img[];
     double* lrho = reinterpret_cast<double*>(img + 4 * BLOB_S);
-    u16* tile = reinterpret_cast<u16*>(lrho + BLOB_S);
     const int t = threadIdx.x / LPP, half = threadIdx.x & (LPP - 1);
+    const unsigned ucap = (unsigned)cap;
     u64 my_ct = SPHX_CT_NONE;
     const int nsel = blob_sel_count(sel, nblk);
     for (int bi = blockIdx.x; bi < nsel; bi += gridDim.x) {
         const int b = blob_sel_at(sel, bi, nsel);
         const int p = b * BLOB_P + t;
         const int i = (p < n) ? qorder[p] : 0;
-        stage<1>(img, lrho, tile, recb, rho_s, 1, nullptr, 0, uniq + (size_t)b * BLOB_S, slot16, npad, k, b);
+        const unsigned sl0 = (p < n) ? (unsigned)slot16[(unsigned)p] : SLOT_NONE;
+        stage<1, BLOB_S>(img, lrho, recb, rho_s, 1, nullptr, 0, uniq + (size_t)b * BLOB_S, cap);
         const RecSelf sf = selfr[i];
         const double rho_i = rho_s[i], mci = bc[i].Bw;
         const double* selfq = reinterpret_cast<const double*>(&recb[i]);
@@ -529,31 +542,29 @@
         __syncthreads();
         if (o < n_active) {
             Q4 r0 = self0, rv = selfv;
-            {
-                const unsigned sl0 = tile[t];
-                if (sl0 < SLOT_OVER) { r0 = lload4(img, (int)sl0, 0); rv = lload4(img, (int)sl0, 1); }
-                else if (sl0 == SLOT_OVER) {
-                    const double* rq = reinterpret_cast<const double*>(&recb[nbr[p]]);
-                    r0 = gload4(rq); rv = gload4(rq + 4);
-                }
+            if (sl0 < ucap) { r0 = lload4<BLOB_S>(img, (int)sl0, 0); rv = lload4<BLOB_S>(img, (int)sl0, 1); }
+            else if (sl0 != SLOT_NONE) {
+                const double* rq = reinterpret_cast<const double*>(&recb[nbr[p]]);
+                r0 = gload4(rq); rv = gload4(rq + 4);
             }
             const double cs_i = sf.csi, h_i = sf.h, hi2 = self0.d, ci = -6.0 * mci;
             ViscAcc a{0.0, 0.0, 0.0, 0.0};
             double maxrel = 0.0;
             const int nm = KPAD(k) / LPP;
-            unsigned sl[NB];
-            load_slots(sl, tile, 0, half, t);
+            const unsigned lane = slot_lane(npad, p, half);
+            unsigned nx[NB];
+            load_batch_slots(nx, slot16, npad, k, 0, lane, half, true);
             for (int m0 = 0; m0 < nm; m0 += NB) {
                 unsigned cur[NB];
 #pragma unroll
-                for (int u = 0; u < NB; ++u) cur[u] = sl[u];
-                if (m0 + NB < nm) load_slots(sl, tile, m0 + NB, half, t);
+                for (int u = 0; u < NB; ++u) cur[u] = nx[u];
+                if (m0 + NB < nm) load_batch_slots(nx, slot16, npad, k, m0 + NB, lane, half, true);
                 const size_t col0 = (size_t)(LPP * m0 + half) * npad + p;
-                const bool fast = all_staged(cur);
-                if (fast && !clip) visc_pw_batch<true, false>(a, maxrel, cur, img, lrho, recb, rho_s, bc, nbr, col0, LPP * (size_t)npad, r0, rv, rho_i, cs_i, hi2, ci);
-                else if (fast) visc_pw_batch<true, true>(a, maxrel, cur, img, lrho, recb, rho_s, bc, nbr, col0, LPP * (size_t)npad, r0, rv, rho_i, cs_i, hi2, ci);
-                else if (!clip) visc_pw_batch<false, false>(a, maxrel, cur, img, lrho, recb, rho_s, bc, nbr, col0, LPP * (size_t)npad, r0, rv, rho_i, cs_i, hi2, ci);
-                else visc_pw_batch<false, true>(a, maxrel, cur, img, lrho, recb, rho_s, bc, nbr, col0, LPP * (size_t)npad, r0, rv, rho_i, cs_i, hi2, ci);
+                const bool fast = all_staged(cur, ucap);
+                if (fast && !clip) visc_pw_batch<true, false, BLOB_S>(a, maxrel, cur, ucap, img, lrho, recb, rho_s, bc, nbr, col0, LPP * (size_t)npad, r0, rv, rho_i, cs_i, hi2, ci);
+                else if (fast) visc_pw_batch<true, true, BLOB_S>(a, maxrel, cur, ucap, img, lrho, recb, rho_s, bc, nbr, col0, LPP * (size_t)npad, r0, rv, rho_i, cs_i, hi2, ci);
+                else if (!clip) visc_pw_batch<false, false, BLOB_S>(a, maxrel, cur, ucap, img, lrho, recb, rho_s, bc, nbr, col0, LPP * (size_t)npad, r0, rv, rho_i, cs_i, hi2, ci);
+                else visc_pw_batch<false, true, BLOB_S>(a, maxrel, cur, ucap, img, lrho, recb, rho_s, bc, nbr, col0, LPP * (size_t)npad, r0, rv, rho_i, cs_i, hi2, ci);
             }
             const double ax = group_total(a.x), ay = group_total(a.y), az = group_total(a.z), heat = group_total(a.h);
             maxrel = group_max(maxrel);
@@ -667,7 +678,8 @@
         const bool live = p < n;
         const int i = live ? qorder[p] : 0;
         const int* uq = uniq + (size_t)b * BLOB_S;
-        stage<0>(img, nullptr, tile, rec, nullptr, 0, nullptr, 0, uq, slot16, npad, k, b);
+        stage<0, BLOB_S>(img, nullptr, rec, nullptr, 0, nullptr, 0, uq, BLOB_S);
+        stage_tile(tile, slot16, npad, k, b);
         const double* self = reinterpret_cast<const double*>(&rec[i]);
         const Q4 s0 = gload4(self), s1 = gload4(self + 4);
         __syncthreads();
@@ -689,12 +701,12 @@
                     unsigned cur[NB];
                     load_slots(cur, tile, m0, half, t);
                     const size_t col0 = (size_t)(LPP * m0 + half) * npad + p;
-                    const bool fast = all_staged(cur);
+                    const bool fast = all_staged(cur, SLOT_OVER);
                     double wo[NB];
-                    if (fast && !clip) density_batch<true, false>(a, wo, cur, img, rec, nbr, col0, LPP * (size_t)npad, xr, yr, zr, hi2, ci, Ai);
-                    else if (fast) density_batch<true, true>(a, wo, cur, img, rec, nbr, col0, LPP * (size_t)npad, xr, yr, zr, hi2, ci, Ai);
-                    else if (!clip) density_batch<false, false>(a, wo, cur, img, rec, nbr, col0, LPP * (size_t)npad, xr, yr, zr, hi2, ci, Ai);
-                    else density_batch<false, true>(a, wo, cur, img, rec, nbr, col0, LPP * (size_t)npad, xr, yr, zr, hi2, ci, Ai);
+                    if (fast && !clip) density_batch<true, false, BLOB_S>(a, wo, cur, SLOT_OVER, img, rec, nbr, col0, LPP * (size_t)npad, xr, yr, zr, hi2, ci, Ai);
+                    else if (fast) density_batch<true, true, BLOB_S>(a, wo, cur, SLOT_OVER, img, rec, nbr, col0, LPP * (size_t)npad, xr, yr, zr, hi2, ci, Ai);
+                    else if (!clip) density_batch<false, false, BLOB_S>(a, wo, cur, SLOT_OVER, img, rec, nbr, col0, LPP * (size_t)npad, xr, yr, zr, hi2, ci, Ai);
+                    else density_batch<false, true, BLOB_S>(a, wo, cur, SLOT_OVER, img, rec, nbr, col0, LPP * (size_t)npad, xr, yr, zr, hi2, ci, Ai);
 #pragma unroll
                     for (int u = 0; u < NB; ++u) if (m0 + u < SPEC_MAXM) w[m0 + u] = wo[u];
                 }
@@ -737,7 +749,8 @@
         const bool live = p < n;
         const int i = live ? qorder[p] : 0;
         const int* uq = uniq + (size_t)b * BLOB_S;
-        stage<0>(img, nullptr, tile, rec, nullptr, 0, nullptr, 0, uq, slot16, npad, k, b);
+        stage<0, BLOB_S>(img, nullptr, rec, nullptr, 0, nullptr, 0, uq, BLOB_S);
+        stage_tile(tile, slot16, npad, k, b);
         __syncthreads();
         double w[SPEC_MAXM];
         {
@@ -797,15 +810,10 @@
         const int i = live ? qorder[p] : 0;
         const int* uq = uniq + (size_t)b * BLOB_S;
         if (FILL) {
-            stage<0>(img, nullptr, tile, recb, nullptr, 0, nullptr, 0, uq, slot16, npad, k, b);
+            stage<0, BLOB_S>(img, nullptr, recb, nullptr, 0, nullptr, 0, uq, BLOB_S);
+            stage_tile(tile, slot16, npad, k, b);
         } else {
-            const int pieces = KPAD(k) * (BLOB_P / 8);
-            for (int q = threadIdx.x; q < pieces; q += PASS_T) {
-                const int kk = q / (BLOB_P / 8), c = q % (BLOB_P / 8);
-                uint4 v = make_uint4(0xFFFFFFFFu, 0xFFFFFFFFu, 0xFFFFFFFFu, 0xFFFFFFFFu);
-                if (kk < k) v = *reinterpret_cast<const uint4*>(slot16 + (size_t)kk * npad + (size_t)b * BLOB_P + c * 8);
-                *reinterpret_cast<uint4*>(tile + kk * BLOB_P + c * 8) = v;
-            }
+            stage_tile(tile, slot16, npad, k, b);
         }
         for (int s = threadIdx.x; s < BLOB_S; s += PASS_T) {
             const int j = uq[s];
@@ -889,13 +897,14 @@
     return BlobSel{list, list + (size_t)ctx->blob_split_nblk, part == 0 ? 3 : part};
 }
 
-int sphx_blob_grid(sphx_ctx* ctx, int nblk) {
-    if (ctx->blob_grid <= 0) {
+int sphx_blob_grid(sphx_ctx* ctx, int nblk, int wgs) {
+    if (ctx->blob_cus <= 0) {
         int cus = 256;
         (void)hipDeviceGetAttribute(&cus, hipDeviceAttributeMultiprocessorCount, ctx->device);
-        ctx->blob_grid = ((cus * 2 + 7) / 8) * 8;
-    }
-    return nblk < ctx->blob_grid ? nblk : ctx->blob_grid;
+        ctx->blob_cus = cus;
+    }
+    const int grid = ((ctx->blob_cus * (ctx->blob_wgs > 0 ? ctx->blob_wgs : wgs) + 7) / 8) * 8;
+    return nblk < grid ? nblk : grid;
 }
 
 int sphx_lds_opt_in(sphx_ctx* ctx, const void* kernel, size_t bytes) {
@@ -909,11 +918,11 @@
 }
 
 template <class Kern, class... Rest>
-static int blob_launch(sphx_ctx* ctx, Kern kern, int per_slot, size_t extra, int64_t n, int k, Rest... rest) {
+static int blob_launch(sphx_ctx* ctx, Kern kern, int wgs, size_t lds, size_t lds_max, int64_t n, int k, Rest... rest) {
     const int64_t npad = sphx_pad64(n);
     const int nblk = (int)((npad + BLOB_P - 1) / BLOB_P);
-    SPHX_TRY(sphx_lds_opt_in(ctx, reinterpret_cast<const void*>(kern), IMG_BYTES(per_slot, SPHX_MAX_K) + extra));
-    hipLaunchKernelGGL(kern, dim3(sphx_blob_grid(ctx, nblk)), dim3(PASS_T), IMG_BYTES(per_slot, k) + extra, ctx->stream, (int)n,
+    SPHX_TRY(sphx_lds_opt_in(ctx, reinterpret_cast<const void*>(kern), lds_max));
+    hipLaunchKernelGGL(kern, dim3(sphx_blob_grid(ctx, nblk, wgs)), dim3(PASS_T), lds, ctx->stream, (int)n,
                        (int)npad, k, nblk, ctx->nbr.as<int>(), ctx->slot16.as<u16>(), ctx->uniq.as<int>(), ctx->qorder, rest...);
     HIPCHK(hipGetLastError());
     return SPHX_OK;
@@ -921,26 +930,26 @@
 static int blob_n_active(const sphx_ctx* ctx, int64_t n) { return ctx->map_perm ? ctx->map_nactive : (int)n; }
 
 int sphx_blob_density(sphx_ctx* ctx, int64_t n, int k, bool lean) {
-    return blob_launch(ctx, blob_density_kernel, 64, 0, n, k, ctx->clip_grad, ctx->map_perm, blob_n_active(ctx, n),
+    return blob_launch(ctx, blob_density_kernel, DENS_WGS, IMG_BYTES(DENS_S, 64), IMG_BYTES(DENS_S, 64), n, k, sphx_pass_slots(ctx, DENS_S), ctx->clip_grad, ctx->map_perm, blob_n_active(ctx, n),
                        ctx->rec1.as<RecA>(), ctx->rho_s.as<double>(), ctx->rho.as<double>(), ctx->rhod.as<double>(),
                        ctx->nden.as<double>(), lean ? nullptr : ctx->G.as<double>(), ctx->ha.as<double>(),
                        sphx_blob_sel(ctx, ctx->pass_part));
 }
 
 int sphx_blob_pi(sphx_ctx* ctx, int64_t n, int k, u64* ct_bits) {
-    return blob_launch(ctx, blob_pi_kernel, 72, 0, n, k, ctx->map_perm, blob_n_active(ctx, n), ctx->recv.as<RecB>(),
+    return blob_launch(ctx, blob_pi_kernel, PI_WGS, IMG_BYTES(PI_S, 72), IMG_BYTES(PI_S, 72), n, k, sphx_pass_slots(ctx, PI_S), ctx->map_perm, blob_n_active(ctx, n), ctx->recv.as<RecB>(),
                        ctx->rho_s.as<double>(), ctx->self_s.as<RecSelf>(), ctx->bc_s.as<RecBC>(), ctx->Pi.as<double>(),
                        ctx->map_perm ? ctx->Bw.as<double>() : nullptr, ct_bits, sphx_blob_sel(ctx, ctx->pass_part));
 }
 
 int sphx_blob_visc(sphx_ctx* ctx, int64_t n, int k, const double* m) {
-    return blob_launch(ctx, blob_visc_kernel, 72, 0, n, k, ctx->clip_grad, ctx->map_perm, blob_n_active(ctx, n),
+    return blob_launch(ctx, blob_visc_kernel, VISC_WGS, IMG_BYTES(VISC_S, 72), IMG_BYTES(VISC_S, 72), n, k, sphx_pass_slots(ctx, VISC_S), ctx->clip_grad, ctx->map_perm, blob_n_active(ctx, n),
                        ctx->recv.as<RecB>(), ctx->bc_s.as<RecBC>(), m, ctx->va.as<double>(), ctx->vh.as<double>(),
                        sphx_blob_sel(ctx, ctx->pass_part));
 }
 
 int sphx_blob_visc_pw(sphx_ctx* ctx, int64_t n, int k, const double* m, u64* ct_bits) {
-    return blob_launch(ctx, blob_visc_pw_kernel, 72, 0, n, k, ctx->clip_grad, ctx->map_perm, blob_n_active(ctx, n),
+    return blob_launch(ctx, blob_visc_pw_kernel, 2, IMG_BYTES(BLOB_S, 72), IMG_BYTES(BLOB_S, 72), n, k, sphx_pass_slots(ctx, BLOB_S), ctx->clip_grad, ctx->map_perm, blob_n_active(ctx, n),
                        ctx->recv.as<RecB>(), ctx->rho_s.as<double>(), ctx->bc_s.as<RecBC>(), ctx->self_s.as<RecSelf>(), m,
                        ctx->va.as<double>(), ctx->vh.as<double>(), ct_bits, sphx_blob_sel(ctx, ctx->pass_part));
 }
@@ -948,7 +957,7 @@
 int sphx_blob_density_species(sphx_ctx* ctx, int64_t n, int k, bool lean, int S, const double* fun, const int* row_of,
                               const double* m_sorted, double* F, double* Z, double* agb, int agb_on) {
     const auto kern = (KPAD(k) / LPP <= 10) ? blob_density_species_kernel<10> : blob_density_species_kernel<16>;
-    return blob_launch(ctx, kern, 64, 0, n, k, ctx->clip_grad, ctx->rec1.as<RecA>(), ctx->rho_s.as<double>(), ctx->rho.as<double>(),
+    return blob_launch(ctx, kern, 2, IMG_BYTES(BLOB_S, 64) + TILE_BYTES(k), IMG_BYTES(BLOB_S, 64) + TILE_BYTES(SPHX_MAX_K), n, k, ctx->clip_grad, ctx->rec1.as<RecA>(), ctx->rho_s.as<double>(), ctx->rho.as<double>(),
                        ctx->rhod.as<double>(), ctx->nden.as<double>(), lean ? nullptr : ctx->G.as<double>(),
                        ctx->ha.as<double>(), S, fun, row_of, m_sorted, ctx->agb, agb_on, F, Z, agb);
 }
@@ -956,12 +965,12 @@
 int sphx_blob_species(sphx_ctx* ctx, int64_t n, int k, int S, const double* fun, const int* row_of, const double* m_sorted, double* F,
                       double* Z, double* agb, int agb_on) {
     const auto kern = (KPAD(k) / LPP <= 10) ? blob_species_kernel<10> : blob_species_kernel<16>;
-    return blob_launch(ctx, kern, 64, 0, n, k, S, ctx->rec1.as<RecA>(), fun, row_of, m_sorted, ctx->agb, agb_on, F, Z, agb);
+    return blob_launch(ctx, kern, 2, IMG_BYTES(BLOB_S, 64) + TILE_BYTES(k), IMG_BYTES(BLOB_S, 64) + TILE_BYTES(SPHX_MAX_K), n, k, S, ctx->rec1.as<RecA>(), fun, row_of, m_sorted, ctx->agb, agb_on, F, Z, agb);
 }
 
 int sphx_blob_drag(sphx_ctx* ctx, int64_t n, int k, bool count_only, const double* m, const double* ptype, const double* mgm,
                    const double* mcs, const int* id, double* onto, const DragScatter& sc) {
     if (count_only)
-        return blob_launch(ctx, blob_drag_kernel<false>, 0, DRAG_XLDS, n, k, nullptr, m, ptype, mgm, mcs, id, onto, sc);
-    return blob_launch(ctx, blob_drag_kernel<true>, 64, DRAG_XLDS, n, k, ctx->recv.as<RecB>(), m, ptype, mgm, mcs, id, onto, sc);
-}
+        return blob_launch(ctx, blob_drag_kernel<false>, 2, TILE_BYTES(k) + DRAG_XLDS, TILE_BYTES(SPHX_MAX_K) + DRAG_XLDS, n, k, nullptr, m, ptype, mgm, mcs, id, onto, sc);
+    return blob_launch(ctx, blob_drag_kernel<true>, 2, IMG_BYTES(BLOB_S, 64) + TILE_BYTES(k) + DRAG_XLDS, IMG_BYTES(BLOB_S, 64) + TILE_BYTES(SPHX_MAX_K) + DRAG_XLDS, n, k, ctx->recv.as<RecB>(), m, ptype, mgm, mcs, id, onto, sc);
+}
diff --git a/sph-code_amd/csrc/sphx_internal.h b/sph-code_amd/csrc/sphx_internal.h
--- a/sph-code_amd/csrc/sphx_internal.h
+++ b/sph-code_amd/csrc/sphx_internal.h
@@ -134,8 +134,10 @@
     bool blob_split_on = true;
     bool species_lds = true;
     bool species_fused = true;
-    int blob_grid = 0;
+    int blob_cus = 0;
+    int blob_wgs = 0;
     int blob_slots = 1 << 20;
+    int blob_pass_slots = 1 << 20;
     int olev_mode = 2;
     int distrust_mode = 0;
     bool cell_feedback = true;
@@ -252,6 +254,7 @@
     DevBuf cell_rank;
     DevBuf tie_list;
     DevBuf slot16, uniq;
+    int blob_nblk = 0;
     DevBuf blob_class, blob_split;
     DevBuf rho, rhod, nden, G, Pi, Bw, va, vh, ha, F;
     DevBuf scal;
diff --git a/sph-code_amd/csrc/sphx_loopforms.hip b/sph-code_amd/csrc/sphx_loopforms.hip
--- a/sph-code_amd/csrc/sphx_loopforms.hip
+++ b/sph-code_amd/csrc/sphx_loopforms.hip
@@ -513,21 +513,21 @@
                                                                           const int* __restrict__ nbr,
                                                                           const u16* __restrict__ slot16,
                                                                           const int* __restrict__ uniq,
-                                                                          const int* __restrict__ qorder,
+                                                                          const int* __restrict__ qorder, int cap,
                                                                           const RecP1* __restrict__ p1,
                                                                           const double* __restrict__ side, double* rho,
                                                                           double* rhod, double* nden, double* G,
                                                                           RecP2* p2, BlobSel sel) {
     extern __shared__ double2 img[];
     double* lgam = reinterpret_cast<double*>(img + 4 * BLOB_S);
-    u16* tile = reinterpret_cast<u16*>(lgam + BLOB_S);
     const int t = threadIdx.x / LPP, part = threadIdx.x & (LPP - 1);
+    const unsigned ucap = (unsigned)cap;
     const int nsel = blob_sel_count(sel, nblk);
     for (int bi = blockIdx.x; bi < nsel; bi += gridDim.x) {
         const int b = blob_sel_at(sel, bi, nsel);
         const int p = b * BLOB_P + t;
         const int i = (p < n) ? qorder[p] : 0;
-        stage<1>(img, lgam, tile, p1, side, 1, nullptr, 0, uniq + (size_t)b * BLOB_S, slot16, npad, k, b);
+        stage<1, BLOB_S>(img, lgam, p1, side, 1, nullptr, 0, uniq + (size_t)b * BLOB_S, cap);
         const double* sp = reinterpret_cast<const double*>(&p1[i]);
         const Q4 s0 = gload4(sp), s1 = gload4(sp + 4);
         __syncthreads();
@@ -535,13 +535,18 @@
             const bool gas_i = s1.c > 0.0;
             L1Acc a{0.0, 0.0, 0.0, 0.0, 0.0, 0.0};
             const int nm = KPAD(k) / LPP;
+            const unsigned lane = slot_lane(npad, p, part);
+            unsigned nx[NB];
+            load_batch_slots(nx, slot16, npad, k, 0, lane, part, true);
             for (int m0 = 0; m0 < nm; m0 += NB) {
                 unsigned sl[NB];
-                load_slots(sl, tile, m0, part, t);
+#pragma unroll
+                for (int u = 0; u < NB; ++u) sl[u] = nx[u];
+                if (m0 + NB < nm) load_batch_slots(nx, slot16, npad, k, m0 + NB, lane, part, true);
                 Q4 q0b[NB], q1b[NB];
                 double gb[NB];
                 int jb[NB];
-                if (all_staged(sl)) {
+                if (all_staged(sl, ucap)) {
 #pragma unroll
                     for (int u = 0; u < NB; ++u) {
                         q0b[u] = lload4(img, (int)sl[u], 0); q1b[u] = lload4(img, (int)sl[u], 1); gb[u] = lgam[sl[u]];
@@ -551,9 +556,9 @@
 #pragma unroll
                     for (int u = 0; u < NB; ++u) {
                         jb[u] = -1;
-                        if (sl[u] < SLOT_OVER) {
+                        if (sl[u] < ucap) {
                             q0b[u] = lload4(img, (int)sl[u], 0); q1b[u] = lload4(img, (int)sl[u], 1); gb[u] = lgam[sl[u]];
-                        } else if (sl[u] == SLOT_OVER) {
+                        } else if (sl[u] != SLOT_NONE) {
                             jb[u] = nbr[(size_t)(LPP * (m0 + u) + part) * npad + p];
                             const double* q = reinterpret_cast<const double*>(&p1[jb[u]]);
                             q0b[u] = gload4(q); q1b[u] = gload4(q + 4); gb[u] = side[jb[u]];
@@ -584,7 +589,7 @@
                                                                           const int* __restrict__ nbr,
                                                                           const u16* __restrict__ slot16,
                                                                           const int* __restrict__ uniq,
-                                                                          const int* __restrict__ qorder,
+                                                                          const int* __restrict__ qorder, int cap,
                                                                           const RecP1* __restrict__ p1,
                                                                           const RecP2* __restrict__ p2,
                                                                           const double* __restrict__ m,
@@ -592,15 +597,15 @@
                                                                           double* vh, u64* ct_bits, BlobSel sel) {
     extern __shared__ double2 img[];
     double* lm = reinterpret_cast<double*>(img + 4 * BLOB_S);
-    u16* tile = reinterpret_cast<u16*>(lm + BLOB_S);
     const int t = threadIdx.x / LPP, part = threadIdx.x & (LPP - 1);
+    const unsigned ucap = (unsigned)cap;
     u64 mine = SPHX_CT_NONE;
     const int nsel = blob_sel_count(sel, nblk);
     for (int bi = blockIdx.x; bi < nsel; bi += gridDim.x) {
         const int b = blob_sel_at(sel, bi, nsel);
         const int p = b * BLOB_P + t;
         const int i = (p < n) ? qorder[p] : 0;
-        stage<1>(img, lm, tile, p2, m, 1, nullptr, 0, uniq + (size_t)b * BLOB_S, slot16, npad, k, b);
+        stage<1, BLOB_S>(img, lm, p2, m, 1, nullptr, 0, uniq + (size_t)b * BLOB_S, cap);
         const double* sp = reinterpret_cast<const double*>(&p2[i]);
         const Q4 s0 = gload4(sp), sv = gload4(sp + 4);
         const double hq_i = p1[i].hq, g1_i = p1[i].g1, m_i = m[i], h_i = h[i];
@@ -610,12 +615,17 @@
             double mx = 0.0;
             if (s0.d >= 0.0) {
                 const int nm = KPAD(k) / LPP;
+                const unsigned lane = slot_lane(npad, p, part);
+                unsigned nx[NB];
+                load_batch_slots(nx, slot16, npad, k, 0, lane, part, true);
                 for (int m0 = 0; m0 < nm; m0 += NB) {
                     unsigned sl[NB];
-                    load_slots(sl, tile, m0, part, t);
+#pragma unroll
+                    for (int u = 0; u < NB; ++u) sl[u] = nx[u];
+                    if (m0 + NB < nm) load_batch_slots(nx, slot16, npad, k, m0 + NB, lane, part, true);
                     Q4 q0b[NB], qvb[NB];
                     double mb[NB];
-                    if (all_staged(sl)) {
+                    if (all_staged(sl, ucap)) {
 #pragma unroll
                         for (int u = 0; u < NB; ++u) {
                             q0b[u] = lload4(img, (int)sl[u], 0); qvb[u] = lload4(img, (int)sl[u], 1); mb[u] = lm[sl[u]];
@@ -623,9 +633,9 @@
                     } else {
 #pragma unroll
                         for (int u = 0; u < NB; ++u) {
-                            if (sl[u] < SLOT_OVER) {
+                            if (sl[u] < ucap) {
                                 q0b[u] = lload4(img, (int)sl[u], 0); qvb[u] = lload4(img, (int)sl[u], 1); mb[u] = lm[sl[u]];
-                            } else if (sl[u] == SLOT_OVER) {
+                            } else if (sl[u] != SLOT_NONE) {
                                 const int j = nbr[(size_t)(LPP * (m0 + u) + part) * npad + p];
                                 const double* q = reinterpret_cast<const double*>(&p2[j]);
                                 q0b[u] = gload4(q); qvb[u] = gload4(q + 4); mb[u] = m[j];
@@ -690,14 +700,14 @@
     const int npad = (int)sphx_pad64(n);
     RecP1* p1 = ctx->lrec_a.as<RecP1>(); RecP2* p2 = ctx->lrec_v.as<RecP2>();
     if (ctx->qorder && ctx->blob_lists) {
-        SPHX_TRY(sphx_lds_opt_in(ctx, reinterpret_cast<const void*>(blob_loop1_kernel), IMG_BYTES(72, SPHX_MAX_K)));
+        SPHX_TRY(sphx_lds_opt_in(ctx, reinterpret_cast<const void*>(blob_loop1_kernel), IMG_BYTES(BLOB_S, 72)));
         const int nblk = (npad + BLOB_P - 1) / BLOB_P;
-        const int g = sphx_blob_grid(ctx, nblk);
+        const int g = sphx_blob_grid(ctx, nblk, 2);
         SPHX_TRY(sphx_ensure(ctx, ctx->loop_side, (size_t)n * sizeof(double)));
         hipLaunchKernelGGL(loop_dust_side_kernel, dim3((unsigned)((n + 255) / 256)), dim3(256), 0, ctx->stream, (int)n,
                            st.ptype.as<double>(), st.m.as<double>(), h, st.gam.as<double>(), p1, ctx->loop_side.as<double>());
-        hipLaunchKernelGGL(blob_loop1_kernel, dim3(g), dim3(PASS_T), IMG_BYTES(72, k), ctx->stream, (int)n, npad, k, nblk,
-                           d9, ctx->nbr.as<int>(), ctx->slot16.as<u16>(), ctx->uniq.as<int>(), ctx->qorder, p1,
+        hipLaunchKernelGGL(blob_loop1_kernel, dim3(g), dim3(PASS_T), IMG_BYTES(BLOB_S, 72), ctx->stream, (int)n, npad, k, nblk,
+                           d9, ctx->nbr.as<int>(), ctx->slot16.as<u16>(), ctx->uniq.as<int>(), ctx->qorder, sphx_pass_slots(ctx, BLOB_S), p1,
                            ctx->loop_side.as<double>(),
                            ctx->rho.as<double>(), ctx->rhod.as<double>(), ctx->nden.as<double>(), ctx->G.as<double>(), p2,
                            sphx_blob_sel(ctx, 0));
@@ -714,11 +724,11 @@
     const int npad = (int)sphx_pad64(n);
     RecP1* p1 = ctx->lrec_a.as<RecP1>(); RecP2* p2 = ctx->lrec_v.as<RecP2>();
     if (ctx->qorder && ctx->blob_lists) {
-        SPHX_TRY(sphx_lds_opt_in(ctx, reinterpret_cast<const void*>(blob_loop2_kernel), IMG_BYTES(72, SPHX_MAX_K)));
+        SPHX_TRY(sphx_lds_opt_in(ctx, reinterpret_cast<const void*>(blob_loop2_kernel), IMG_BYTES(BLOB_S, 72)));
         const int nblk = (npad + BLOB_P - 1) / BLOB_P;
-        const int g = sphx_blob_grid(ctx, nblk);
-        hipLaunchKernelGGL(blob_loop2_kernel, dim3(g), dim3(PASS_T), IMG_BYTES(72, k), ctx->stream, (int)n, npad, k, nblk,
-                           ctx->nbr.as<int>(), ctx->slot16.as<u16>(), ctx->uniq.as<int>(), ctx->qorder, p1, p2,
+        const int g = sphx_blob_grid(ctx, nblk, 2);
+        hipLaunchKernelGGL(blob_loop2_kernel, dim3(g), dim3(PASS_T), IMG_BYTES(BLOB_S, 72), ctx->stream, (int)n, npad, k, nblk,
+                           ctx->nbr.as<int>(), ctx->slot16.as<u16>(), ctx->uniq.as<int>(), ctx->qorder, sphx_pass_slots(ctx, BLOB_S), p1, p2,
                            st.m.as<double>(), h, ctx->va.as<double>(), ctx->vh.as<double>(), ct, sphx_blob_sel(ctx, part));
     } else {
         hipLaunchKernelGGL(loop_pass2_kernel, dim3((unsigned)((n + 255) / 256)), dim3(256), 0, ctx->stream, (int)n, npad, k,
```

New measurement: 779.3 million. 0.954x the previous value.
